# roahmlab/armour

Measured on NVIDIA B200. Metric: planning iters/s (eval_g + eval_jac_g pairs on built reach sets; Kinova 7-DOF, 128 steps, 10 obstacles), higher is better.
Workload: dtype f64

## Files before the change

### armour_b200/_lib.py

```python
from __future__ import annotations

import ctypes as C
import os

_HERE = os.path.dirname(os.path.abspath(__file__))
LIB_PATH = os.environ.get("ARMOUR_B200_LIB") or os.path.join(_HERE, "libarmour_b200.so")
NF = 7

OK, ERR_ARG, ERR_CUDA, ERR_OBSTACLES, ERR_CAPACITY, ERR_STATE, ERR_NOMEM = 0, -1, -2, -3, -4, -5, -6


class ArmourError(RuntimeError):
    def __init__(self, code, msg):
        super().__init__(f"armour_b200 error {code}: {msg}")
        self.code = code


class Config(C.Structure):
    _fields_ = [
        ("struct_size", C.c_int), ("device", C.c_int), ("robot_model", C.c_int), ("num_time_steps", C.c_int),
        ("max_obstacles", C.c_int), ("max_problems", C.c_int), ("cap_link_monomials", C.c_int),
        ("cap_torque_monomials", C.c_int), ("cap_work_monomials", C.c_int), ("simplify_threshold", C.c_double),
        ("k_range", C.c_double * NF), ("mass_uncertainty", C.c_double), ("inertia_uncertainty", C.c_double),
    ]


dp = C.POINTER(C.c_double)
ip = C.POINTER(C.c_int)
up = C.POINTER(C.c_ulonglong)


class ReachsetTables(C.Structure):
    _fields_ = [
        ("cap_link", C.c_int), ("cap_u", C.c_int), ("link_n", ip), ("link_center", dp), ("link_key", up),
        ("link_coeff", dp), ("u_n", ip), ("u_center", dp), ("u_key", up), ("u_coeff", dp), ("u_radius", dp),
        ("torque_radius", dp), ("link_gens", dp),
    ]


SIGNATURES = {
    "armour_config_default": (C.c_int, [C.POINTER(Config)]),
    "armour_ctx_create": (C.c_int, [C.POINTER(Config), C.POINTER(C.c_void_p)]),
    "armour_ctx_destroy": (C.c_int, [C.c_void_p]),
    "armour_ctx_reserve": (C.c_int, [C.c_void_p, C.c_int, C.c_int]),
    "armour_ctx_set_stream": (C.c_int, [C.c_void_p, C.c_void_p]),
    "armour_ctx_synchronize": (C.c_int, [C.c_void_p]),
    "armour_status_string": (C.c_char_p, [C.c_int]),
    "armour_last_error": (C.c_char_p, [C.c_void_p]),
    "armour_abi_version": (C.c_int, []),
    "armour_kernel_launches": (C.c_longlong, [C.c_void_p]),
    "armour_num_joints": (C.c_int, [C.c_void_p]),
    "armour_num_time_steps": (C.c_int, [C.c_void_p]),
    "armour_num_constraints": (C.c_int, [C.c_void_p, C.c_int]),
    "armour_reachsets_build": (C.c_int, [C.c_void_p, dp, dp, dp, dp, C.c_int]),
    "armour_get_torque_radius": (C.c_int, [C.c_void_p, dp]),
    "armour_get_link_independent_generators": (C.c_int, [C.c_void_p, dp]),
    "armour_get_bounds": (C.c_int, [C.c_void_p, dp, dp]),
    "armour_eval_g": (C.c_int, [C.c_void_p, dp, dp]),
    "armour_eval_jac_g": (C.c_int, [C.c_void_p, dp, dp]),
    "armour_eval_g_jac": (C.c_int, [C.c_void_p, dp, dp, dp]),
    "armour_get_link_sliced_center": (C.c_int, [C.c_void_p, dp]),
    "armour_verdict": (C.c_int, [C.c_void_p, dp, ip, ip]),
    "armour_cost": (C.c_int, [C.c_void_p, dp, dp, dp, dp]),
    "armour_batch_reachsets_build": (C.c_int, [C.c_void_p, C.c_int, dp, dp, dp, dp, C.c_int]),
    "armour_batch_eval": (C.c_int, [C.c_void_p, C.c_int, dp, dp, dp]),
    "armour_batch_eval_device": (C.c_int, [C.c_void_p, C.c_int, C.c_void_p, C.c_void_p, C.c_void_p]),
    "armour_batch_reachsets_build_device": (C.c_int, [C.c_void_p, C.c_int, C.c_void_p, C.c_void_p, C.c_void_p,
                                                      C.c_void_p, C.c_int]),
    "armour_batch_verdict_device": (C.c_int, [C.c_void_p, C.c_int, C.c_void_p, C.c_void_p, C.c_void_p]),
    "armour_batch_get_torque_radius": (C.c_int, [C.c_void_p, C.c_int, dp]),
    "armour_batch_get_link_independent_generators": (C.c_int, [C.c_void_p, C.c_int, dp]),
    "armour_batch_get_bounds": (C.c_int, [C.c_void_p, C.c_int, dp, dp]),
    "armour_batch_get_build_status": (C.c_int, [C.c_void_p, C.c_int, ip]),
    "armour_batch_get_monomial_counts": (C.c_int, [C.c_void_p, C.c_int, ip, ip]),
    "armour_batch_get_candidate_counts": (C.c_int, [C.c_void_p, C.c_int, C.c_void_p]),
    "armour_chunk_intervals": (C.c_int, []),
    "armour_jacobian_nnz": (C.c_longlong, [C.c_void_p, C.c_int]),
    "armour_jacobian_structure": (C.c_int, [C.c_void_p, C.c_int, ip, ip]),
    "armour_eval_jac_g_structured": (C.c_int, [C.c_void_p, dp, dp]),
    "armour_batch_eval_structured": (C.c_int, [C.c_void_p, C.c_int, dp, dp, dp]),
    "armour_batch_eval_structured_device": (C.c_int, [C.c_void_p, C.c_int, C.c_void_p, C.c_void_p, C.c_void_p]),
    "armour_measure_fp64_peak": (C.c_int, [C.c_void_p, dp]),
    "armour_solver_options_default": (None, [C.c_void_p]),
    "armour_batch_solve_device": (C.c_int, [C.c_void_p, C.c_int, C.c_void_p, C.c_void_p, C.c_void_p, C.c_void_p,
                                            C.c_void_p, C.c_void_p]),
    "armour_batch_solve": (C.c_int, [C.c_void_p, C.c_int, dp, C.c_void_p, dp, ip, ip, ip]),
    "armour_export_reachsets": (C.c_int, [C.c_void_p, C.c_int, C.POINTER(ReachsetTables)]),
    "armour_import_reachsets": (C.c_int, [C.c_void_p, C.c_int, C.c_int, C.POINTER(ReachsetTables), dp, dp, dp, dp,
                                          C.c_int]),
}


class ControllerGains(C.Structure):
    _fields_ = [("Kr", dp), ("alpha", C.c_double), ("V_max", C.c_double), ("r_norm_threshold", C.c_double),
                ("apply_friction", C.c_int)]


_gp = C.POINTER(ControllerGains)
SIGNATURES.update({
    "armour_controller_create": (C.c_int, [C.c_char_p, C.c_double, C.c_int, C.POINTER(C.c_void_p)]),
    "armour_controller_create_error": (C.c_char_p, []),
    "armour_controller_destroy": (None, [C.c_void_p]),
    "armour_controller_num_joints": (C.c_int, [C.c_void_p]),
    "armour_controller_last_error": (C.c_char_p, [C.c_void_p]),
    "armour_controller_kernel_launches": (C.c_longlong, [C.c_void_p]),
    "armour_controller_set_stream": (C.c_int, [C.c_void_p, C.c_void_p]),
    "armour_controller_synchronize": (C.c_int, [C.c_void_p]),
    "armour_controller_get_interval_model": (C.c_int, [C.c_void_p, dp]),
    "armour_controller_rnea": (C.c_int, [C.c_void_p, C.c_int, dp, dp, dp, dp, C.c_int, C.c_int, dp, dp, dp]),
    "armour_controller_rnea_device": (C.c_int, [C.c_void_p, C.c_int] + [C.c_void_p] * 5 + [C.c_int, C.c_int] + [C.c_void_p] * 3),
    "armour_controller_update": (C.c_int, [C.c_void_p, C.c_int, _gp, dp, dp, dp, dp, dp, dp, dp, dp, ip]),
    "armour_controller_update_device": (C.c_int, [C.c_void_p, C.c_int, _gp] + [C.c_void_p] * 10),
})

SIGNATURES.update({
    "armour_armtd_ctx_create": (C.c_int, [C.POINTER(Config), C.POINTER(C.c_void_p)]),
    "armour_armtd_build": (C.c_int, [C.c_void_p, dp, dp, dp, dp, dp, C.c_int]),
    "armour_armtd_num_constraints": (C.c_int, [C.c_void_p]),
    "armour_armtd_eval": (C.c_int, [C.c_void_p, dp, dp, dp]),
    "armour_armtd_get_bounds": (C.c_int, [C.c_void_p, dp, dp]),
    "armour_armtd_verdict": (C.c_int, [C.c_void_p, dp, ip, ip]),
    "armour_armtd_cost": (C.c_int, [C.c_void_p, dp, dp, dp, dp]),
    "armour_armtd_get_link_sliced_center": (C.c_int, [C.c_void_p, dp]),
    "armour_armtd_get_link_independent_generators": (C.c_int, [C.c_void_p, dp]),
    "armour_armtd_batch_ctx_create": (C.c_int, [C.POINTER(Config), C.POINTER(C.c_void_p)]),
    "armour_armtd_batch_build": (C.c_int, [C.c_void_p, C.c_int, dp, dp, dp, dp, dp, C.c_int]),
    "armour_armtd_batch_build_device": (C.c_int, [C.c_void_p, C.c_int] + [C.c_void_p] * 5 + [C.c_int, C.c_void_p]),
    "armour_armtd_batch_eval": (C.c_int, [C.c_void_p, C.c_int, dp, dp, dp]),
    "armour_armtd_batch_eval_device": (C.c_int, [C.c_void_p, C.c_int, C.c_void_p, C.c_void_p, C.c_void_p]),
    "armour_armtd_batch_verdict_device": (C.c_int, [C.c_void_p, C.c_int, C.c_void_p, C.c_void_p, C.c_void_p]),
    "armour_armtd_batch_cost": (C.c_int, [C.c_void_p, C.c_int, dp, dp, dp, dp]),
    "armour_armtd_batch_get_link_independent_generators": (C.c_int, [C.c_void_p, C.c_int, dp]),
    "armour_armtd_batch_solve": (C.c_int, [C.c_void_p, C.c_int, dp, C.c_void_p, dp, ip, ip, ip]),
    "armour_armtd_batch_solve_device": (C.c_int, [C.c_void_p, C.c_int] + [C.c_void_p] * 6),
})


class SolverOptions(C.Structure):
    _fields_ = [("max_iter", C.c_int), ("tol", C.c_double), ("torque_tol", C.c_double), ("collision_tol", C.c_double),
                ("qp_sweeps", C.c_int), ("qp_update_budget", C.c_int)]


class RolloutOptions(C.Structure):
    _fields_ = [("struct_size", C.c_int), ("max_replans", C.c_int), ("lookahead", C.c_double), ("goal_radius", C.c_double),
                ("audit_samples", C.c_int), ("solver", SolverOptions)]


class RolloutOut(C.Structure):
    _fields_ = [("outcome", ip), ("replans", ip), ("infeasible", ip), ("final_state", dp), ("min_clearance", dp),
                ("log_state", dp), ("log_q_des", dp), ("log_k", dp), ("log_int", ip), ("log_clearance", dp)]


ROLLOUT_BUDGET, ROLLOUT_ARRIVED, ROLLOUT_COLLISION, ROLLOUT_LIMIT = 0, 1, 2, 3

SIGNATURES.update({
    "armour_rollout_options_default": (None, [C.POINTER(RolloutOptions)]),
    "armour_batch_rollout_device": (C.c_int, [C.c_void_p, C.c_int, C.c_void_p, C.c_void_p, C.c_void_p, C.c_int,
                                              C.POINTER(RolloutOptions), C.POINTER(RolloutOut)]),
    "armour_batch_rollout": (C.c_int, [C.c_void_p, C.c_int, dp, dp, dp, C.c_int, C.POINTER(RolloutOptions),
                                       C.POINTER(RolloutOut)]),
    "armour_batch_clearance_device": (C.c_int, [C.c_void_p, C.c_int] + [C.c_void_p] * 3 + [C.c_int, C.c_void_p, C.c_void_p]),
    "armour_batch_clearance": (C.c_int, [C.c_void_p, C.c_int, dp, ip, dp, C.c_int, dp, ip]),
})


_LIB = None


def load():
    global _LIB
    if _LIB is None:
        if not os.path.exists(LIB_PATH):
            raise ImportError(
                f"{LIB_PATH} is missing: build the CUDA extension first (python -c 'import __graft_entry__ as g; "
                "g.build()' or make -C armour_b200/csrc). armour_b200 has no CPU fallback.")
        lib = C.CDLL(LIB_PATH)
        for name, (res, args) in SIGNATURES.items():
            fn = getattr(lib, name)
            fn.restype = res
            fn.argtypes = args
        _LIB = lib
    return _LIB
```

### armour_b200/csrc/armour_capi.cu

```cuda
#include <cuda_runtime.h>

#include <algorithm>
#include <cmath>
#include <cstdio>
#include <cstdlib>
#include <cstring>
#include <mutex>
#include <new>
#include <string>
#include <vector>

#include "../../include/armour_b200.h"
#include "bezier.cuh"
#include "device_constants.cuh"
#ifdef K1_PROFILE
constexpr int K1_PROF_SITES = 512;
__device__ long long g_k1prof[128 * K1_PROF_SITES * 2];
__device__ int g_k1spill[8];
#endif
#ifndef K1LAT_NT
#define K1LAT_NT 128
#endif
#ifndef K1LAT_CTAS
#define K1LAT_CTAS 1
#endif
#ifndef K1LAT_GROUPS
#define K1LAT_GROUPS 3
#endif
#ifndef K1LAT_MG
#define K1LAT_MG 1
#endif
#ifndef K1LAT_TAB_16THS
#define K1LAT_TAB_16THS 11
#endif
#define K1_TAB_16THS K1LAT_TAB_16THS
#ifndef K1LAT_DYN_CAP
#define K1LAT_DYN_CAP -1
#endif
#define K1_DYN_CAP K1LAT_DYN_CAP
#define K1_NS k1lat
#define K1_NT K1LAT_NT
#define K1_CTAS K1LAT_CTAS
#define K1_GROUPS K1LAT_GROUPS
#define K1_MG K1LAT_MG
#include "k1_reachsets.cuh"
#undef K1_NS
#undef K1_NT
#undef K1_CTAS
#undef K1_GROUPS
#undef K1_MG
#undef K1_TAB_16THS
#define K1_MG 0
#ifndef K1THR_NT
#define K1THR_NT 64
#endif
#ifndef K1THR_GROUPS
#define K1THR_GROUPS 8
#endif
#ifndef K1THR_CTAS
#define K1THR_CTAS 2
#endif
#ifndef K1THR_TAB_EIGHTHS
#define K1THR_TAB_EIGHTHS 4
#endif
#ifndef K1THR_DYN_CAP
#define K1THR_DYN_CAP 0
#endif
#ifndef K1THR_JRS_GLOBAL
#define K1THR_JRS_GLOBAL 1
#endif
#undef K1_JRS_GLOBAL
#define K1_JRS_GLOBAL K1THR_JRS_GLOBAL
#undef K1_DYN_CAP
#define K1_DYN_CAP K1THR_DYN_CAP
#undef K1_TAB_EIGHTHS
#define K1_TAB_EIGHTHS K1THR_TAB_EIGHTHS
#define K1_TAB_16THS (2 * K1THR_TAB_EIGHTHS)
#define K1_NS k1thr
#define K1_NT K1THR_NT
#define K1_CTAS K1THR_CTAS
#define K1_GROUPS K1THR_GROUPS
#include "k1_reachsets.cuh"
#undef K1_NS
#undef K1_NT
#undef K1_CTAS
#undef K1_GROUPS
#include "k3_constraints.cuh"
#include "k4_solver.cuh"
#include "armtd.cuh"
#include "rollout.cuh"
#include "layout.h"

using namespace armour;

struct armour_ctx {
    armour_config cfg;
    RobotConstants rc;
    cudaStream_t stream = nullptr;
    cudaStream_t own_stream = nullptr;
    Batch B;
    int built_nprob = 0;
    size_t hp_capacity = 0;
    int hp_nprob = 0;
    int* d_unit_flag = nullptr;
    size_t obs_capacity = 0;
    double* d_in = nullptr;
    double* d_obs = nullptr;
    double* d_k = nullptr;
    double* d_g = nullptr;
    double* d_jac = nullptr;
    size_t g_capacity = 0, jac_capacity = 0;
    double* d_jnz = nullptr;
    size_t jnz_capacity = 0;
    int* d_verdict = nullptr;
    double* d_solver = nullptr;
    int* d_solver_i = nullptr;
    double* d_solver_io = nullptr;
    size_t solver_doubles = 0, solver_ints = 0;
    k1lat::K1Scratch k1_lat;
    k1thr::K1Scratch k1_thr;
    bool k1_thr_ready = false;
    long long launches = 0;
    std::string last_error;
    std::vector<double> h_torque_radius;
    bool h_torque_valid = false;
    std::vector<double> h_q0, h_qd0, h_qdd0;
    bool armtd = false;
    double* d_jrs = nullptr;
    double* d_armtd_in = nullptr;
    double* d_krange = nullptr;
    double* d_zero = nullptr;
    double* d_cs = nullptr;
    double* d_jrs_raw = nullptr;
    double* d_ga = nullptr;
    double* d_ja = nullptr;
    size_t ga_capacity = 0, ja_capacity = 0;
    std::vector<double> h_krange;
    double* d_roll = nullptr;
    int* d_roll_i = nullptr;
    size_t roll_doubles = 0, roll_ints = 0;
    char* d_stage = nullptr;
    size_t stage_bytes = 0;
};

namespace {

__global__ void __launch_bounds__(256) k_fp64_peak(double* out, int iters, double a) {
    double x[8];
#pragma unroll
    for (int i = 0; i < 8; i++) x[i] = double(threadIdx.x + i);
    for (int it = 0; it < iters; it++) {
#pragma unroll
        for (int i = 0; i < 8; i++) x[i] = __fma_rn(x[i], a, 0.5);
    }
    double s = 0;
#pragma unroll
    for (int i = 0; i < 8; i++) s += x[i];
    if (s == 12345.678) out[0] = s;
}

int fail(armour_ctx* c, int code, const std::string& msg) {
    if (c) c->last_error = msg;
    return code;
}
#define CU(expr)                                                                                     \
    do {                                                                                             \
        cudaError_t e__ = (expr);                                                                    \
        if (e__ != cudaSuccess)                                                                      \
            return fail(ctx, ARMOUR_ERR_CUDA, std::string(#expr) + ": " + cudaGetErrorString(e__)); \
    } while (0)

template <class T>
cudaError_t dalloc(T** p, size_t n) {
    return cudaMalloc(reinterpret_cast<void**>(p), std::max<size_t>(n, 1) * sizeof(T));
}

int ensure_eval_buffers(armour_ctx* ctx, int nprob, bool need_g, bool need_jac) {
    const size_t m = size_t(ctx->B.m());
    if (need_g && ctx->g_capacity < nprob * m) {
        if (ctx->d_g) cudaFree(ctx->d_g);
        ctx->d_g = nullptr;
        CU(dalloc(&ctx->d_g, nprob * m));
        ctx->g_capacity = nprob * m;
    }
    if (need_jac && ctx->jac_capacity < nprob * m * NF) {
        if (ctx->d_jac) cudaFree(ctx->d_jac);
        ctx->d_jac = nullptr;
        CU(dalloc(&ctx->d_jac, nprob * m * NF));
        ctx->jac_capacity = nprob * m * NF;
    }
    return ARMOUR_OK;
}

int ensure_obstacle_buffers(armour_ctx* ctx, int nprob, int nobs) {
    const size_t need_obs = size_t(nprob) * nobs * 12;
    if (ctx->obs_capacity < need_obs) {
        if (ctx->d_obs) cudaFree(ctx->d_obs);
        ctx->d_obs = nullptr;
        CU(dalloc(&ctx->d_obs, need_obs));
        ctx->obs_capacity = need_obs;
    }
    Batch& B = ctx->B;
    B.O = nobs;
    B.nprob = nprob;
    const size_t need_hp = size_t(nprob) * (B.T / TB) * B.hp_chunk();
    if (ctx->hp_capacity < need_hp || ctx->hp_nprob < nprob) {
        if (B.hp_cand) cudaFree(B.hp_cand);
        if (B.hp_cnt) cudaFree(B.hp_cnt);
        if (B.hp_slow) cudaFree(B.hp_slow);
        B.hp_cand = nullptr;
        B.hp_cnt = nullptr;
        B.hp_slow = nullptr;
        ctx->hp_capacity = 0;
        ctx->hp_nprob = 0;
        ctx->built_nprob = 0;
        const size_t np = std::max(nprob, ctx->hp_nprob);
        CU(dalloc(&B.hp_cand, need_hp));
        CU(dalloc(&B.hp_cnt, need_hp / (HP_CAP * 4)));
        CU(dalloc(&B.hp_slow, np));
        CU(cudaMemsetAsync(B.hp_slow, 0, np * sizeof(int), ctx->stream));
        ctx->hp_capacity = need_hp;
        ctx->hp_nprob = nprob;
    }
    B.obstacles = ctx->d_obs;
    return ARMOUR_OK;
}

int launch_build(armour_ctx* ctx, const Batch& B, int* nl, bool* latency) {
    const long long nunits = (long long)B.nprob * B.T;
    const bool thr = ctx->cfg.max_problems > 1 && nunits > 2LL * ctx->k1_lat.grid;
    *latency = !thr;
    if (thr) {
        if (!ctx->k1_thr_ready) {
            CU(k1thr::k1_scratch_create(&ctx->k1_thr, ctx->cfg, ctx->rc, ctx->stream));
            ctx->k1_thr_ready = true;
        }
        CU(k1thr::launch_reachsets(B, ctx->k1_thr, ctx->stream, nl));
    } else {
        CU(k1lat::launch_reachsets(B, ctx->k1_lat, ctx->stream, nl, ctx->d_unit_flag));
    }
    return ARMOUR_OK;
}

std::mutex g_const_mutex;
struct ConstOwner {
    bool valid = false;
    RobotConstants rc;
};
ConstOwner g_const_owner[64];

int ensure_constants(armour_ctx* ctx) {
    const int dev = ctx->cfg.device;
    if (dev < 0 || dev >= 64) return fail(ctx, ARMOUR_ERR_ARG, "device ordinal");
    std::lock_guard<std::mutex> lock(g_const_mutex);
    ConstOwner& o = g_const_owner[dev];
    if (o.valid && std::memcmp(&o.rc, &ctx->rc, sizeof(RobotConstants)) == 0) return ARMOUR_OK;
    CU(cudaDeviceSynchronize());
    CU(upload_constants(ctx->rc, ctx->stream));
    o.rc = ctx->rc;
    o.valid = true;
    return ARMOUR_OK;
}

int check_batch(armour_ctx* ctx, int nprob, int nobs) {
    if (!ctx) return ARMOUR_ERR_ARG;
    if (nprob < 1 || nprob > ctx->cfg.max_problems)
        return fail(ctx, ARMOUR_ERR_STATE, "nprob outside [1, max_problems]");
    if (nobs < 0) return fail(ctx, ARMOUR_ERR_ARG, "negative obstacle count");
    if (nobs > ctx->cfg.max_obstacles)
        return fail(ctx, ARMOUR_ERR_OBSTACLES, "number of obstacles larger than max_obstacles");
    return ARMOUR_OK;
}

int fetch_torque_radius(armour_ctx* ctx) {
    if (ctx->h_torque_valid) return ARMOUR_OK;
    const size_t n = size_t(ctx->built_nprob) * NF * ctx->B.T;
    ctx->h_torque_radius.resize(n);
    CU(cudaMemcpyAsync(ctx->h_torque_radius.data(), ctx->B.torque_radius, n * sizeof(double), cudaMemcpyDeviceToHost,
                       ctx->stream));
    CU(cudaStreamSynchronize(ctx->stream));
    ctx->h_torque_valid = true;
    return ARMOUR_OK;
}

}

extern "C" {

int armour_abi_version(void) { return ARMOUR_ABI_VERSION; }

const char* armour_status_string(int s) {
    switch (s) {
        case ARMOUR_OK: return "ok";
        case ARMOUR_ERR_ARG: return "invalid argument";
        case ARMOUR_ERR_CUDA: return "CUDA error";
        case ARMOUR_ERR_OBSTACLES: return "too many obstacles";
        case ARMOUR_ERR_CAPACITY: return "monomial table capacity exceeded";
        case ARMOUR_ERR_STATE: return "invalid call order or batch size";
        case ARMOUR_ERR_NOMEM: return "out of memory";
        default: return "unknown status";
    }
}

int armour_config_default(armour_config* cfg) {
    if (!cfg) return ARMOUR_ERR_ARG;
    std::memset(cfg, 0, sizeof(*cfg));
    cfg->struct_size = int(sizeof(armour_config));
    cfg->device = 0;
    cfg->robot_model = 0;
    cfg->num_time_steps = 128;
    cfg->max_obstacles = 40;
    cfg->max_problems = 1;
    cfg->cap_link_monomials = 32;
    cfg->cap_torque_monomials = 64;
    cfg->cap_work_monomials = 768;
    cfg->simplify_threshold = 5e-4;
    for (int i = 0; i < NF; i++) cfg->k_range[i] = M_PI / 48;
    cfg->mass_uncertainty = -1;
    cfg->inertia_uncertainty = -1;
    return ARMOUR_OK;
}

int armour_ctx_create(const armour_config* cfg, armour_ctx** out) {
    if (!cfg || !out) return ARMOUR_ERR_ARG;
    *out = nullptr;
    if (cfg->struct_size != int(sizeof(armour_config))) return ARMOUR_ERR_ARG;
    if (cfg->num_time_steps < TB || cfg->num_time_steps > 128 || cfg->num_time_steps % TB != 0) return ARMOUR_ERR_ARG;
    if (cfg->max_problems < 1 || cfg->max_obstacles < 0) return ARMOUR_ERR_ARG;
    if (cfg->robot_model < 0 || cfg->robot_model > 1) return ARMOUR_ERR_ARG;
    if (cfg->cap_link_monomials < 1 || cfg->cap_torque_monomials < 1 || cfg->cap_work_monomials < 64)
        return ARMOUR_ERR_ARG;
    if (cfg->cap_link_monomials % 8 != 0 || cfg->cap_torque_monomials % 8 != 0) return ARMOUR_ERR_ARG;
    if (cfg->max_problems > 65535) return ARMOUR_ERR_ARG;
    int ndev = 0;
    if (cudaGetDeviceCount(&ndev) != cudaSuccess || ndev == 0 || cfg->device >= ndev) return ARMOUR_ERR_CUDA;
    armour_ctx* ctx = new (std::nothrow) armour_ctx();
    if (!ctx) return ARMOUR_ERR_NOMEM;
    ctx->cfg = *cfg;
    ctx->rc = make_robot_constants(cfg->robot_model);
    ctx->rc.num_time_steps = cfg->num_time_steps;
    ctx->rc.simplify_threshold = cfg->simplify_threshold;
    for (int i = 0; i < NF; i++) ctx->rc.k_range[i] = cfg->k_range[i];
    if (cfg->mass_uncertainty >= 0) ctx->rc.mass_uncertainty = cfg->mass_uncertainty;
    if (cfg->inertia_uncertainty >= 0) ctx->rc.inertia_uncertainty = cfg->inertia_uncertainty;

    auto bail = [&](const char* what, cudaError_t e) {
        std::fprintf(stderr, "armour_ctx_create: %s: %s\n", what, cudaGetErrorString(e));
        armour_ctx_destroy(ctx);
        return ARMOUR_ERR_CUDA;
    };
    cudaError_t e;
    if ((e = cudaSetDevice(cfg->device)) != cudaSuccess) return bail("cudaSetDevice", e);
    if ((e = cudaStreamCreateWithFlags(&ctx->own_stream, cudaStreamNonBlocking)) != cudaSuccess)
        return bail("cudaStreamCreate", e);
    ctx->stream = ctx->own_stream;
    if (ensure_constants(ctx) != ARMOUR_OK) return bail("upload_constants", cudaGetLastError());

    Batch& B = ctx->B;
    std::memset(&B, 0, sizeof(B));
    B.T = cfg->num_time_steps;
    B.NJ = ctx->rc.num_joints;
    B.capL = cfg->cap_link_monomials;
    B.capU = cfg->cap_torque_monomials;
    const size_t P = size_t(cfg->max_problems), T = size_t(B.T), NJ = size_t(B.NJ);
#define ALLOC(ptr, n) \
    if ((e = dalloc(&ptr, (n))) != cudaSuccess) return bail(#ptr, e)
    ALLOC(ctx->d_in, 3 * P * NF);
    ALLOC(B.link_n, P * T * NJ);
    ALLOC(B.link_c, P * T * NJ * 3);
    ALLOC(B.link_key, P * T * NJ * B.capL);
    ALLOC(B.link_g, P * T * NJ * B.capL * 3);
    ALLOC(B.u_n, P * T * NF);
    ALLOC(B.u_c, P * T * NF);
    ALLOC(B.u_r, P * T * NF);
    ALLOC(B.u_key, P * T * NF * B.capU);
    ALLOC(B.u_g, P * T * NF * B.capU);
    ALLOC(B.torque_radius, P * NF * T);
    ALLOC(B.link_gens, P * T * NJ * 18);
    ALLOC(B.link_r, P * T * NJ * 3);
    ALLOC(B.link_sliced, P * T * NJ * 3);
    ALLOC(B.status, P);
    ALLOC(ctx->d_unit_flag, P * T);
    ALLOC(ctx->d_k, P * NF);
    ALLOC(ctx->d_verdict, 2 * P);
#undef ALLOC
    B.q0 = ctx->d_in;
    B.qd0 = ctx->d_in + P * NF;
    B.qdd0 = ctx->d_in + 2 * P * NF;
    if ((e = cudaMemsetAsync(B.status, 0, P * sizeof(int), ctx->stream)) != cudaSuccess) return bail("memset", e);
    if ((e = cudaMemsetAsync(ctx->d_unit_flag, 0, P * T * sizeof(int), ctx->stream)) != cudaSuccess) return bail("memset", e);
    if ((e = cudaMemsetAsync(B.link_n, 0, P * T * NJ * sizeof(int), ctx->stream)) != cudaSuccess) return bail("memset", e);
    if ((e = cudaMemsetAsync(B.u_n, 0, P * T * NF * sizeof(int), ctx->stream)) != cudaSuccess) return bail("memset", e);
    if ((e = k1lat::k1_scratch_create(&ctx->k1_lat, ctx->cfg, ctx->rc, ctx->stream)) != cudaSuccess) return bail("k1 scratch", e);
    if ((long long)cfg->max_problems * B.T > 2LL * ctx->k1_lat.grid) {
        if ((e = k1thr::k1_scratch_create(&ctx->k1_thr, ctx->cfg, ctx->rc, ctx->stream)) != cudaSuccess) return bail("k1 throughput scratch", e);
        ctx->k1_thr_ready = true;
        cudaFuncAttributes fa2;
        if ((e = cudaFuncGetAttributes(&fa2, k1thr::k_reachsets)) != cudaSuccess) return bail("load k_reachsets (throughput)", e);
    }
    {
        cudaFuncAttributes fa;
        if ((e = cudaFuncGetAttributes(&fa, k1lat::k_reachsets)) != cudaSuccess) return bail("load k_reachsets", e);
        if ((e = cudaFuncGetAttributes(&fa, k_hyperplanes)) != cudaSuccess) return bail("load k_hyperplanes", e);
        if ((e = cudaFuncGetAttributes(&fa, k_constraints)) != cudaSuccess) return bail("load k_constraints", e);
        if ((e = cudaFuncSetAttribute(k_constraints, cudaFuncAttributeMaxDynamicSharedMemorySize,
                                      TB * (MAXJ * K3_LTAB_BYTES + NF * K3_UTAB_BYTES) + K3_CAND_ARENA)) != cudaSuccess)
            return bail("k_constraints shared memory", e);
        if ((e = cudaFuncGetAttributes(&fa, k_constraints_slow)) != cudaSuccess) return bail("load k_constraints_slow", e);
        if ((e = cudaFuncGetAttributes(&fa, k_verdict)) != cudaSuccess) return bail("load k_verdict", e);
    }
    if ((e = cudaStreamSynchronize(ctx->stream)) != cudaSuccess) return bail("sync", e);
    *out = ctx;
    return ARMOUR_OK;
}

int armour_ctx_destroy(armour_ctx* ctx) {
    if (!ctx) return ARMOUR_OK;
    cudaSetDevice(ctx->cfg.device);
    Batch& B = ctx->B;
    void* ptrs[] = {ctx->d_roll, ctx->d_roll_i, ctx->d_stage, ctx->d_solver, ctx->d_solver_i, ctx->d_solver_io, ctx->d_unit_flag, ctx->d_jnz, ctx->d_jrs, ctx->d_armtd_in, ctx->d_ga, ctx->d_ja,
                    ctx->d_in, ctx->d_obs, ctx->d_k, ctx->d_g, ctx->d_jac, ctx->d_verdict, B.link_n, B.link_c,
                    B.link_key, B.link_g, B.u_n, B.u_c, B.u_r, B.u_key, B.u_g, B.torque_radius, B.link_gens, B.link_r, B.hp_cand, B.hp_cnt, B.hp_slow,
                    B.link_sliced, B.status};
    for (void* p : ptrs)
        if (p) cudaFree(p);
    k1lat::k1_scratch_destroy(&ctx->k1_lat);
    k1thr::k1_scratch_destroy(&ctx->k1_thr);
    if (ctx->own_stream) cudaStreamDestroy(ctx->own_stream);
    delete ctx;
    return ARMOUR_OK;
}

int armour_ctx_set_stream(armour_ctx* ctx, void* s) {
    if (!ctx) return ARMOUR_ERR_ARG;
    ctx->stream = s ? static_cast<cudaStream_t>(s) : ctx->own_stream;
    return ARMOUR_OK;
}
int armour_ctx_synchronize(armour_ctx* ctx) {
    if (!ctx) return ARMOUR_ERR_ARG;
    CU(cudaStreamSynchronize(ctx->stream));
    return ARMOUR_OK;
}
const char* armour_last_error(const armour_ctx* ctx) { return ctx ? ctx->last_error.c_str() : "null context"; }
long long armour_kernel_launches(const armour_ctx* ctx) { return ctx ? ctx->launches : 0; }
int armour_num_joints(const armour_ctx* ctx) { return ctx ? ctx->B.NJ : ARMOUR_ERR_ARG; }
int armour_num_time_steps(const armour_ctx* ctx) { return ctx ? ctx->B.T : ARMOUR_ERR_ARG; }
int armour_num_constraints(const armour_ctx* ctx, int nobs) {
    if (!ctx || nobs < 0) return ARMOUR_ERR_ARG;
    return NF * ctx->B.T + ctx->B.NJ * ctx->B.T * nobs + 4 * NF;
}

int armour_ctx_reserve(armour_ctx* ctx, int nprob, int nobs) {
    int rc = check_batch(ctx, nprob, nobs);
    if (rc) return rc;
    CU(cudaSetDevice(ctx->cfg.device));
    { int rc_c = ensure_constants(ctx); if (rc_c) return rc_c; }
    const int O = ctx->B.O, np = ctx->B.nprob;
    rc = ensure_obstacle_buffers(ctx, nprob, nobs);
    ctx->B.O = O;
    ctx->B.nprob = np;
    if (rc) return rc;
    ctx->B.O = nobs;
    rc = ensure_eval_buffers(ctx, nprob, true, true);
    ctx->B.O = O;
    return rc;
}

int armour_batch_reachsets_build_device(armour_ctx* ctx, int nprob, const double* d_q0, const double* d_qd0,
                                        const double* d_qdd0, const double* d_obstacles, int nobs) {
    int rc = check_batch(ctx, nprob, nobs);
    if (rc) return rc;
    if (!d_q0 || !d_qd0 || !d_qdd0 || (nobs > 0 && !d_obstacles)) return fail(ctx, ARMOUR_ERR_ARG, "null input");
    CU(cudaSetDevice(ctx->cfg.device));
    { int rc_c = ensure_constants(ctx); if (rc_c) return rc_c; }
    rc = ensure_obstacle_buffers(ctx, nprob, nobs);
    if (rc) return rc;
    const size_t P = size_t(ctx->cfg.max_problems);
    ctx->B.epoch++;
    int nl = 0;
    bool latency = false;
    if (nobs > 0) {
        Batch Bb = ctx->B;
        Bb.q0 = d_q0;
        Bb.qd0 = d_qd0;
        Bb.qdd0 = d_qdd0;
        Bb.obstacles = d_obstacles;
        { int rc2 = launch_build(ctx, Bb, &nl, &latency); if (rc2) return rc2; }
        HpStage stage{ctx->d_in, ctx->d_in + P * NF, ctx->d_in + 2 * P * NF, ctx->d_obs};
        CU(launch_hyperplanes(Bb, ctx->stream, latency ? ctx->d_unit_flag : nullptr, stage));
        nl++;
    } else {
        const size_t nb = size_t(nprob) * NF * sizeof(double);
        CU(cudaMemcpyAsync(ctx->d_in, d_q0, nb, cudaMemcpyDeviceToDevice, ctx->stream));
        CU(cudaMemcpyAsync(ctx->d_in + P * NF, d_qd0, nb, cudaMemcpyDeviceToDevice, ctx->stream));
        CU(cudaMemcpyAsync(ctx->d_in + 2 * P * NF, d_qdd0, nb, cudaMemcpyDeviceToDevice, ctx->stream));
        { int rc2 = launch_build(ctx, ctx->B, &nl, &latency); if (rc2) return rc2; }
    }
    ctx->launches += nl;
    ctx->built_nprob = nprob;
    ctx->h_torque_valid = false;
    ctx->h_q0.clear();
    return ARMOUR_OK;
}

int armour_batch_reachsets_build(armour_ctx* ctx, int nprob, const double* q0, const double* qd0, const double* qdd0,
                                 const double* obstacles, int nobs) {
    int rc = check_batch(ctx, nprob, nobs);
    if (rc) return rc;
    if (!q0 || !qd0 || !qdd0 || (nobs > 0 && !obstacles)) return fail(ctx, ARMOUR_ERR_ARG, "null input");
    CU(cudaSetDevice(ctx->cfg.device));
    { int rc_c = ensure_constants(ctx); if (rc_c) return rc_c; }
    rc = ensure_obstacle_buffers(ctx, nprob, nobs);
    if (rc) return rc;
    const size_t P = size_t(ctx->cfg.max_problems);
    const size_t nb = size_t(nprob) * NF * sizeof(double);
    CU(cudaMemcpyAsync(ctx->d_in, q0, nb, cudaMemcpyHostToDevice, ctx->stream));
    CU(cudaMemcpyAsync(ctx->d_in + P * NF, qd0, nb, cudaMemcpyHostToDevice, ctx->stream));
    CU(cudaMemcpyAsync(ctx->d_in + 2 * P * NF, qdd0, nb, cudaMemcpyHostToDevice, ctx->stream));
    if (nobs > 0)
        CU(cudaMemcpyAsync(ctx->d_obs, obstacles, size_t(nprob) * nobs * 12 * sizeof(double), cudaMemcpyHostToDevice,
                           ctx->stream));
    ctx->B.epoch++;
    int nl = 0;
    bool latency = false;
    { int rc2 = launch_build(ctx, ctx->B, &nl, &latency); if (rc2) return rc2; }
    ctx->launches += nl;
    CU(launch_hyperplanes(ctx->B, ctx->stream, (latency && nobs > 0) ? ctx->d_unit_flag : nullptr));
    ctx->launches += (nobs > 0);
    ctx->built_nprob = nprob;
    ctx->h_torque_valid = false;
    ctx->h_q0.assign(q0, q0 + size_t(nprob) * NF);
    ctx->h_qd0.assign(qd0, qd0 + size_t(nprob) * NF);
    ctx->h_qdd0.assign(qdd0, qdd0 + size_t(nprob) * NF);
    std::vector<int> st(nprob);
    CU(cudaMemcpyAsync(st.data(), ctx->B.status, nprob * sizeof(int), cudaMemcpyDeviceToHost, ctx->stream));
    CU(cudaStreamSynchronize(ctx->stream));
    for (int p = 0; p < nprob; p++)
        if ((st[p] >> 3) == ctx->B.epoch && (st[p] & 7) != 0) {
            int site[3] = {0, 0, 0};
            const int* dstats = latency ? ctx->k1_lat.stats : ctx->k1_thr.stats;
            std::string where;
            if (dstats && cudaMemcpy(site, dstats + 4, sizeof(site), cudaMemcpyDeviceToHost) == cudaSuccess && site[2] == ctx->B.epoch) {
                const int line = site[0] >> 3;
                where = "; first failing check: code " + std::to_string(site[0] & 7) + " at " +
                        (line >= 10000 ? "k1_reachsets.cuh:" + std::to_string(line - 10000) : "k1_pz.cuh:" + std::to_string(line)) +
                        ", problem " + std::to_string(site[1] / ctx->B.T) + " interval " + std::to_string(site[1] % ctx->B.T);
            }
            return fail(ctx, ARMOUR_ERR_CAPACITY,
                        "reach-set build overflowed a monomial table (problem " + std::to_string(p) + ", code " +
                            std::to_string(st[p] & 7) + ")" + where);
        }
    return ARMOUR_OK;
}

int armour_reachsets_build(armour_ctx* ctx, const double* q0, const double* qd0, const double* qdd0,
                           const double* obstacles, int nobs) {
    return armour_batch_reachsets_build(ctx, 1, q0, qd0, qdd0, obstacles, nobs);
}

int armour_batch_get_build_status(armour_ctx* ctx, int nprob, int* out) {
    if (!ctx || !out || nprob < 1 || nprob > ctx->built_nprob) return ARMOUR_ERR_ARG;
    CU(cudaMemcpyAsync(out, ctx->B.status, nprob * sizeof(int), cudaMemcpyDeviceToHost, ctx->stream));
    CU(cudaStreamSynchronize(ctx->stream));
    for (int p = 0; p < nprob; p++)
        out[p] = ((out[p] >> 3) == ctx->B.epoch && (out[p] & 7) != 0) ? ARMOUR_ERR_CAPACITY : ARMOUR_OK;
    return ARMOUR_OK;
}

int armour_batch_get_monomial_counts(armour_ctx* ctx, int nprob, int* link_n, int* u_n) {
    if (!ctx || nprob < 1 || nprob > ctx->built_nprob) return ARMOUR_ERR_ARG;
    const size_t T = ctx->B.T, NJ = ctx->B.NJ;
    if (link_n)
        CU(cudaMemcpyAsync(link_n, ctx->B.link_n, nprob * T * NJ * sizeof(int), cudaMemcpyDeviceToHost, ctx->stream));
    if (u_n) CU(cudaMemcpyAsync(u_n, ctx->B.u_n, nprob * T * NF * sizeof(int), cudaMemcpyDeviceToHost, ctx->stream));
    CU(cudaStreamSynchronize(ctx->stream));
    return ARMOUR_OK;
}

int armour_batch_get_candidate_counts(armour_ctx* ctx, int nprob, unsigned char* out) {
    if (!ctx || !out || nprob < 1 || nprob > ctx->built_nprob) return ARMOUR_ERR_ARG;
    const size_t rows = size_t(ctx->B.NJ) * ctx->B.T * ctx->B.O;
    if (rows) CU(cudaMemcpyAsync(out, ctx->B.hp_cnt, nprob * rows, cudaMemcpyDeviceToHost, ctx->stream));
    CU(cudaStreamSynchronize(ctx->stream));
    return ARMOUR_OK;
}

int armour_chunk_intervals(void) { return TB; }

#ifdef K1_PROFILE
extern "C" int armour_debug_k1_profile(long long* out, int reset) {
    cudaDeviceSynchronize();
    if (out) {
        int sp[8];
        if (cudaMemcpyFromSymbol(sp, g_k1spill, sizeof(sp)) == cudaSuccess)
            std::printf("k1 profile: %d of %d arena blocks in global memory, %d scratch pools in global memory, %d cross products on "
                        "the table path (largest term count %d)\n", sp[0], sp[1], sp[2], sp[3], sp[4]);
    }
    if (out && cudaMemcpyFromSymbol(out, g_k1prof, sizeof(long long) * 128 * K1_PROF_SITES * 2) != cudaSuccess) return ARMOUR_ERR_CUDA;
    if (reset) {
        void* p = nullptr;
        if (cudaGetSymbolAddress(&p, g_k1prof) != cudaSuccess) return ARMOUR_ERR_CUDA;
        if (cudaMemset(p, 0, sizeof(long long) * 128 * K1_PROF_SITES * 2) != cudaSuccess) return ARMOUR_ERR_CUDA;
    }
    return ARMOUR_OK;
}
#endif

int armour_measure_fp64_peak(armour_ctx* ctx, double* tflops) {
    if (!ctx || !tflops) return ARMOUR_ERR_ARG;
    CU(cudaSetDevice(ctx->cfg.device));
    { int rc_c = ensure_constants(ctx); if (rc_c) return rc_c; }
    int sms = 0;
    CU(cudaDeviceGetAttribute(&sms, cudaDevAttrMultiProcessorCount, ctx->cfg.device));
    double* d_out = nullptr;
    CU(dalloc(&d_out, 1));
    cudaEvent_t e0, e1;
    CU(cudaEventCreate(&e0));
    CU(cudaEventCreate(&e1));
    const int iters = 4096, grid = sms * 8, block = 256;
    double best = 0.0;
    for (int rep = 0; rep < 4; rep++) {
        CU(cudaEventRecord(e0, ctx->stream));
        k_fp64_peak<<<grid, block, 0, ctx->stream>>>(d_out, iters, 1.0000001);
        CU(cudaEventRecord(e1, ctx->stream));
        CU(cudaEventSynchronize(e1));
        float ms = 0;
        CU(cudaEventElapsedTime(&ms, e0, e1));
        const double fl = 2.0 * 8 * double(iters) * double(grid) * block;
        if (rep > 0) best = std::max(best, fl / (ms * 1e-3) / 1e12);
    }
    ctx->launches += 4;
    cudaEventDestroy(e0);
    cudaEventDestroy(e1);
    cudaFree(d_out);
    *tflops = best;
    return ARMOUR_OK;
}

int armour_batch_eval_device(armour_ctx* ctx, int nprob, const double* d_k, double* d_g, double* d_values) {
    if (!ctx || !d_k) return ARMOUR_ERR_ARG;
    if (nprob < 1 || nprob > ctx->built_nprob) return fail(ctx, ARMOUR_ERR_STATE, "evaluate before build");
    CU(cudaSetDevice(ctx->cfg.device));
    { int rc_c = ensure_constants(ctx); if (rc_c) return rc_c; }
    Batch B = ctx->B;
    B.nprob = nprob;
    CU(launch_constraints(B, d_k, d_g, d_values, ctx->stream));
    ctx->launches += 1 + (B.O > 0);
    return ARMOUR_OK;
}

int armour_batch_eval(armour_ctx* ctx, int nprob, const double* k, double* g, double* values) {
    if (!ctx || !k) return ARMOUR_ERR_ARG;
    if (nprob < 1 || nprob > ctx->built_nprob) return fail(ctx, ARMOUR_ERR_STATE, "evaluate before build");
    CU(cudaSetDevice(ctx->cfg.device));
    { int rc_c = ensure_constants(ctx); if (rc_c) return rc_c; }
    int rc = ensure_eval_buffers(ctx, nprob, g != nullptr, values != nullptr);
    if (rc) return rc;
    const size_t m = size_t(ctx->B.m());
    CU(cudaMemcpyAsync(ctx->d_k, k, size_t(nprob) * NF * sizeof(double), cudaMemcpyHostToDevice, ctx->stream));
    rc = armour_batch_eval_device(ctx, nprob, ctx->d_k, g ? ctx->d_g : nullptr, values ? ctx->d_jac : nullptr);
    if (rc) return rc;
    if (g) CU(cudaMemcpyAsync(g, ctx->d_g, nprob * m * sizeof(double), cudaMemcpyDeviceToHost, ctx->stream));
    if (values)
        CU(cudaMemcpyAsync(values, ctx->d_jac, nprob * m * NF * sizeof(double), cudaMemcpyDeviceToHost, ctx->stream));
    CU(cudaStreamSynchronize(ctx->stream));
    return ARMOUR_OK;
}

long long armour_jacobian_nnz(const armour_ctx* ctx, int nobs) {
    if (!ctx || nobs < 0) return ARMOUR_ERR_ARG;
    return jac_nnz(ctx->B.T, ctx->B.NJ, nobs);
}

int armour_jacobian_structure(const armour_ctx* ctx, int nobs, int* iRow, int* jCol) {
    if (!ctx || nobs < 0 || !iRow || !jCol) return ARMOUR_ERR_ARG;
    const int T = ctx->B.T, NJ = ctx->B.NJ;
    size_t n = 0;
    for (int r = 0; r < NF * T; r++)
        for (int c = 0; c < NF; c++, n++) {
            iRow[n] = r;
            jCol[n] = c;
        }
    for (int l = 0; l < NJ; l++)
        for (int r = 0; r < T * nobs; r++)
            for (int c = 0; c < jac_link_width(l); c++, n++) {
                iRow[n] = NF * T + l * T * nobs + r;
                jCol[n] = c;
            }
    for (int r = 0; r < 4 * NF; r++, n++) {
        iRow[n] = NF * T + NJ * T * nobs + r;
        jCol[n] = r % NF;
    }
    return ARMOUR_OK;
}

int armour_batch_eval_structured_device(armour_ctx* ctx, int nprob, const double* d_k, double* d_g, double* d_values_nnz) {
    if (!ctx || !d_k || !d_values_nnz) return ARMOUR_ERR_ARG;
    if (nprob < 1 || nprob > ctx->built_nprob) return fail(ctx, ARMOUR_ERR_STATE, "evaluate before build");
    CU(cudaSetDevice(ctx->cfg.device));
    int rc = ensure_eval_buffers(ctx, nprob, false, true);
    if (rc) return rc;
    rc = armour_batch_eval_device(ctx, nprob, d_k, d_g, ctx->d_jac);
    if (rc) return rc;
    Batch B = ctx->B;
    B.nprob = nprob;
    CU(launch_pack_jacobian(B, ctx->d_jac, d_values_nnz, ctx->stream));
    ctx->launches += 1;
    return ARMOUR_OK;
}

int armour_batch_eval_structured(armour_ctx* ctx, int nprob, const double* k, double* g, double* values_nnz) {
    if (!ctx || !k || !values_nnz) return ARMOUR_ERR_ARG;
    if (nprob < 1 || nprob > ctx->built_nprob) return fail(ctx, ARMOUR_ERR_STATE, "evaluate before build");
    CU(cudaSetDevice(ctx->cfg.device));
    int rc = ensure_eval_buffers(ctx, nprob, g != nullptr, true);
    if (rc) return rc;
    const size_t m = size_t(ctx->B.m());
    const size_t nnz = size_t(jac_nnz(ctx->B.T, ctx->B.NJ, ctx->B.O));
    if (ctx->jnz_capacity < nprob * nnz) {
        if (ctx->d_jnz) cudaFree(ctx->d_jnz);
        ctx->d_jnz = nullptr;
        ctx->jnz_capacity = 0;
        CU(dalloc(&ctx->d_jnz, nprob * nnz));
        ctx->jnz_capacity = nprob * nnz;
    }
    CU(cudaMemcpyAsync(ctx->d_k, k, size_t(nprob) * NF * sizeof(double), cudaMemcpyHostToDevice, ctx->stream));
    rc = armour_batch_eval_structured_device(ctx, nprob, ctx->d_k, g ? ctx->d_g : nullptr, ctx->d_jnz);
    if (rc) return rc;
    if (g) CU(cudaMemcpyAsync(g, ctx->d_g, nprob * m * sizeof(double), cudaMemcpyDeviceToHost, ctx->stream));
    CU(cudaMemcpyAsync(values_nnz, ctx->d_jnz, nprob * nnz * sizeof(double), cudaMemcpyDeviceToHost, ctx->stream));
    CU(cudaStreamSynchronize(ctx->stream));
    return ARMOUR_OK;
}

int armour_eval_jac_g_structured(armour_ctx* ctx, const double* k, double* values_nnz) {
    return armour_batch_eval_structured(ctx, 1, k, nullptr, values_nnz);
}

int armour_eval_g(armour_ctx* ctx, const double* k, double* g) { return armour_batch_eval(ctx, 1, k, g, nullptr); }
int armour_eval_jac_g(armour_ctx* ctx, const double* k, double* values) {
    return armour_batch_eval(ctx, 1, k, nullptr, values);
}
int armour_eval_g_jac(armour_ctx* ctx, const double* k, double* g, double* values) {
    return armour_batch_eval(ctx, 1, k, g, values);
}

int armour_batch_verdict_device(armour_ctx* ctx, int nprob, const double* d_g, int* d_feasible, int* d_first) {
    if (!ctx || !d_g || !d_feasible || !d_first) return ARMOUR_ERR_ARG;
    if (nprob < 1 || nprob > ctx->built_nprob) return fail(ctx, ARMOUR_ERR_STATE, "verdict before build");
    CU(cudaSetDevice(ctx->cfg.device));
    { int rc_c = ensure_constants(ctx); if (rc_c) return rc_c; }
    Batch B = ctx->B;
    B.nprob = nprob;
    CU(launch_verdict(B, d_g, d_feasible, d_first, ctx->stream));
    ctx->launches += 1;
    return ARMOUR_OK;
}

void armour_solver_options_default(armour_solver_options* opt) {
    if (!opt) return;
    opt->max_iter = 60;
    opt->tol = 1e-4;
    opt->torque_tol = 1e-2;
    opt->collision_tol = 1e-4;
    opt->qp_sweeps = 200;
    opt->qp_update_budget = 16384;
}

}

namespace {

template <class Nlp, class Eval, class Verdict>
int run_solver(armour_ctx* ctx, int nprob, const double* d_q_des, const armour_solver_options& opt, const Nlp& nlp, int m_rows,
               double* g_x, double* jac_x, const Eval& eval, int n_eval, const Verdict& verdict, double* d_k_opt, int* d_feasible,
               int* d_first, int* d_iters) {
    if (opt.max_iter < 1 || !(opt.tol > 0) || opt.qp_sweeps < 1) return fail(ctx, ARMOUR_ERR_ARG, "solver options");
    Batch B = ctx->B;
    B.nprob = nprob;
    const size_t m = size_t(m_rows);
    const size_t P = size_t(nprob);
    const size_t need_d = P * (3 * NF + 4) + P * m + P * SOLVER_ROWCAP * SOLVER_ROWW;
    const size_t need_i = 8 * P + 1;
    if (ctx->solver_doubles < need_d) {
        if (ctx->d_solver) cudaFree(ctx->d_solver);
        ctx->d_solver = nullptr;
        ctx->solver_doubles = 0;
        CU(dalloc(&ctx->d_solver, need_d));
        ctx->solver_doubles = need_d;
    }
    if (ctx->solver_ints < need_i) {
        if (ctx->d_solver_i) cudaFree(ctx->d_solver_i);
        ctx->d_solver_i = nullptr;
        ctx->solver_ints = 0;
        CU(dalloc(&ctx->d_solver_i, need_i));
        ctx->solver_ints = need_i;
    }
    SolverState S;
    double* w = ctx->d_solver;
    S.x = w; w += P * NF;
    S.xt = w; w += P * NF;
    S.best = w; w += P * NF;
    S.f = w; w += P;
    S.viol = w; w += P;
    S.fbest = w; w += P;
    S.delta = w; w += P;
    double* d_gt = w; w += P * m;
    S.rows = w;
    S.have_best = ctx->d_solver_i;
    S.status = S.have_best + P;
    S.iters = S.status + P;
    S.evals = S.iters + P;
    S.dbg = S.evals + P;
    int* d_running = S.dbg + 3 * P;
    int* d_list = d_running + 1;
    S.q_des = d_q_des;
    S.tol = opt.tol;
    S.torque_tol = opt.torque_tol;
    S.collision_tol = opt.collision_tol;
    S.max_iter = opt.max_iter;
    S.qp_sweeps = opt.qp_sweeps;
    S.qp_update_budget = opt.qp_update_budget;
    cudaStream_t st = ctx->stream;
    const size_t step_smem = solver_step_smem(m_rows);
    if (step_smem > 200 * 1024) return fail(ctx, ARMOUR_ERR_ARG, "too many constraint rows for the batched solver");
    if (step_smem > 40 * 1024)
        CU(cudaFuncSetAttribute(k_solver_step<Nlp>, cudaFuncAttributeMaxDynamicSharedMemorySize, int(step_smem)));
    CU(cudaMemsetAsync(S.x, 0, size_t(nprob) * NF * sizeof(double), st));
    CU(cudaMemsetAsync(S.xt, 0, size_t(nprob) * NF * sizeof(double), st));
    { int rc = eval(B, S.x, g_x, nullptr); if (rc) return rc; }
    k_solver_start<<<nprob, SOLVER_THREADS, 0, st>>>(B, nlp, S, g_x);
    CU(cudaGetLastError());
    ctx->launches += 1 + n_eval;
    static const int compact_every = [] {
        const char* v = std::getenv("ARMOUR_SOLVER_COMPACT_EVERY");
        const int n = v ? std::atoi(v) : 0;
        return n >= 1 ? n : 4;
    }();
    Batch Ba = B;
    int nactive = nprob;
    for (int it = 0; it < opt.max_iter && nactive > 0; it++) {
        Ba.nprob = nactive;
        { int rc = eval(Ba, S.x, g_x, jac_x); if (rc) return rc; }
        k_solver_step<<<nactive, SOLVER_THREADS, step_smem, st>>>(Ba, nlp, S, g_x, jac_x, it);
        { int rc = eval(Ba, S.xt, d_gt, nullptr); if (rc) return rc; }
        k_solver_accept<<<nactive, SOLVER_THREADS, 0, st>>>(Ba, nlp, S, d_gt, it == opt.max_iter - 1 ? 1 : 0);
        CU(cudaGetLastError());
        ctx->launches += 2 + 2 * n_eval;
        if ((it + 1) % compact_every == 0 && it + 1 < opt.max_iter) {
            CU(cudaMemsetAsync(d_running, 0, sizeof(int), st));
            k_solver_compact<<<(nprob + 255) / 256, 256, 0, st>>>(S, nprob, d_running, d_list);
            CU(cudaMemcpyAsync(&nactive, d_running, sizeof(int), cudaMemcpyDeviceToHost, st));
            CU(cudaStreamSynchronize(st));
            ctx->launches += 1;
            Ba.plist = d_list;
        }
    }
    k_solver_final<<<(nprob + 255) / 256, 256, 0, st>>>(S, nprob, d_k_opt, nullptr);
    { int rc = eval(B, d_k_opt, g_x, nullptr); if (rc) return rc; }
    { int rc = verdict(g_x, d_feasible, d_first); if (rc) return rc; }
    if (d_iters) CU(cudaMemcpyAsync(d_iters, S.iters, size_t(nprob) * sizeof(int), cudaMemcpyDeviceToDevice, st));
    if (std::getenv("ARMOUR_SOLVER_DEBUG")) {
        std::vector<int> dbg(size_t(nprob) * 3);
        CU(cudaMemcpyAsync(dbg.data(), S.dbg, dbg.size() * sizeof(int), cudaMemcpyDeviceToHost, st));
        CU(cudaStreamSynchronize(st));
        long long r = 0, sw = 0, mv = 0;
        int rmax = 0, mvmax = 0;
        for (int p = 0; p < nprob; p++) {
            r += dbg[p * 3];
            sw += dbg[p * 3 + 1];
            mv += dbg[p * 3 + 2];
            rmax = std::max(rmax, dbg[p * 3]);
            mvmax = std::max(mvmax, dbg[p * 3 + 2]);
        }
        std::printf("solver debug: last step per problem: rows mean %.0f max %d, active-set iterations mean %.1f, dropped rows mean %.1f max %d\n",
                    double(r) / nprob, rmax, double(sw) / nprob, double(mv) / nprob, mvmax);
    }
    ctx->launches += 2 + n_eval;
    CU(cudaGetLastError());
    return ARMOUR_OK;
}

using SolveDeviceFn = int (*)(armour_ctx*, int, const double*, const armour_solver_options*, double*, int*, int*, int*);
int solve_from_host(armour_ctx* ctx, int nprob, const double* q_des, const armour_solver_options* opt, double* k_opt, int* feasible,
                    int* first_violation, int* iterations, SolveDeviceFn solve_device) {
    CU(cudaSetDevice(ctx->cfg.device));
    { int rc_c = ensure_constants(ctx); if (rc_c) return rc_c; }
    if (!ctx->d_solver_io) CU(dalloc(&ctx->d_solver_io, size_t(ctx->cfg.max_problems) * (2 * NF + 2)));
    const size_t P = size_t(ctx->cfg.max_problems);
    double* d_q = ctx->d_solver_io;
// ... 205 lines not shown
    for (int i = 0; i < 13; i++) {
        off[i] = total;
        total += (sz[i] + 255) / 256 * 256;
    }
    rc = ensure_buffer(ctx, &ctx->d_stage, &ctx->stage_bytes, total);
    if (rc) return rc;
    char* base = ctx->d_stage;
    auto at = [&](int i) -> void* { return sz[i] ? base + off[i] : nullptr; };
    cudaStream_t st = ctx->stream;
    CU(cudaMemcpyAsync(at(0), start, sz[0], cudaMemcpyHostToDevice, st));
    CU(cudaMemcpyAsync(at(1), goal, sz[1], cudaMemcpyHostToDevice, st));
    if (nobs > 0) CU(cudaMemcpyAsync(at(2), obstacles, sz[2], cudaMemcpyHostToDevice, st));
    armour_rollout_out d_out;
    d_out.outcome = static_cast<int*>(at(3));
    d_out.replans = static_cast<int*>(at(4));
    d_out.infeasible = static_cast<int*>(at(5));
    d_out.final_state = static_cast<double*>(at(6));
    d_out.min_clearance = static_cast<double*>(at(7));
    d_out.log_state = static_cast<double*>(at(8));
    d_out.log_q_des = static_cast<double*>(at(9));
    d_out.log_k = static_cast<double*>(at(10));
    d_out.log_int = static_cast<int*>(at(11));
    d_out.log_clearance = static_cast<double*>(at(12));
    rc = rollout_run(ctx, nworlds, static_cast<const double*>(at(0)), static_cast<const double*>(at(1)),
                     nobs > 0 ? static_cast<const double*>(at(2)) : nullptr, nobs, *opt, d_out);
    if (rc) return rc;
    void* host[13] = {nullptr, nullptr, nullptr, out->outcome, out->replans, out->infeasible, out->final_state, out->min_clearance,
                      out->log_state, out->log_q_des, out->log_k, out->log_int, out->log_clearance};
    for (int i = 3; i < 13; i++)
        if (sz[i]) CU(cudaMemcpyAsync(host[i], at(i), sz[i], cudaMemcpyDeviceToHost, st));
    CU(cudaStreamSynchronize(st));
    return ARMOUR_OK;
}

int armour_batch_clearance_device(armour_ctx* ctx, int nconf, const double* d_q, const int* d_world, const double* d_obstacles,
                                  int nobs, double* d_clearance, int* d_which) {
    int rc = check_clearance(ctx, nconf, nobs);
    if (rc) return rc;
    if (!d_q || !d_clearance || (nobs > 0 && !d_obstacles)) return fail(ctx, ARMOUR_ERR_ARG, "null input");
    CU(cudaSetDevice(ctx->cfg.device));
    { int rc_c = ensure_constants(ctx); if (rc_c) return rc_c; }
    k_clearance<<<nconf, CLEAR_THREADS, 0, ctx->stream>>>(d_q, 1, d_world, d_obstacles, nobs, d_clearance, d_which);
    CU(cudaGetLastError());
    ctx->launches += 1;
    return ARMOUR_OK;
}

int armour_batch_clearance(armour_ctx* ctx, int nconf, const double* q, const int* world, const double* obstacles, int nobs,
                           double* clearance, int* which) {
    int rc = check_clearance(ctx, nconf, nobs);
    if (rc) return rc;
    if (!q || !clearance || (nobs > 0 && !obstacles)) return fail(ctx, ARMOUR_ERR_ARG, "null input");
    int nsets = 1;
    if (world)
        for (int i = 0; i < nconf; i++) {
            if (world[i] < 0) return fail(ctx, ARMOUR_ERR_ARG, "negative obstacle-set index");
            nsets = std::max(nsets, world[i] + 1);
        }
    CU(cudaSetDevice(ctx->cfg.device));
    const size_t nq = size_t(nconf) * NF * 8, nw = world ? size_t(nconf) * 4 : 0, nb = size_t(nsets) * nobs * 12 * 8,
                 nc = size_t(nconf) * 8, nh = which ? size_t(nconf) * 4 : 0;
    const size_t oq = 0, ow = oq + (nq + 255) / 256 * 256, ob = ow + (nw + 255) / 256 * 256, oc = ob + (nb + 255) / 256 * 256,
                 oh = oc + (nc + 255) / 256 * 256;
    rc = ensure_buffer(ctx, &ctx->d_stage, &ctx->stage_bytes, oh + nh);
    if (rc) return rc;
    char* base = ctx->d_stage;
    cudaStream_t st = ctx->stream;
    CU(cudaMemcpyAsync(base + oq, q, nq, cudaMemcpyHostToDevice, st));
    if (world) CU(cudaMemcpyAsync(base + ow, world, nw, cudaMemcpyHostToDevice, st));
    if (nobs > 0) CU(cudaMemcpyAsync(base + ob, obstacles, nb, cudaMemcpyHostToDevice, st));
    rc = armour_batch_clearance_device(ctx, nconf, reinterpret_cast<const double*>(base + oq),
                                       world ? reinterpret_cast<const int*>(base + ow) : nullptr,
                                       nobs > 0 ? reinterpret_cast<const double*>(base + ob) : nullptr, nobs,
                                       reinterpret_cast<double*>(base + oc), which ? reinterpret_cast<int*>(base + oh) : nullptr);
    if (rc) return rc;
    CU(cudaMemcpyAsync(clearance, base + oc, nc, cudaMemcpyDeviceToHost, st));
    if (which) CU(cudaMemcpyAsync(which, base + oh, nh, cudaMemcpyDeviceToHost, st));
    CU(cudaStreamSynchronize(st));
    return ARMOUR_OK;
}

int armour_batch_get_torque_radius(armour_ctx* ctx, int nprob, double* out) {
    if (!ctx || !out || nprob < 1 || nprob > ctx->built_nprob) return ARMOUR_ERR_ARG;
    int rc = fetch_torque_radius(ctx);
    if (rc) return rc;
    std::memcpy(out, ctx->h_torque_radius.data(), size_t(nprob) * NF * ctx->B.T * sizeof(double));
    return ARMOUR_OK;
}
int armour_get_torque_radius(armour_ctx* ctx, double* out) { return armour_batch_get_torque_radius(ctx, 1, out); }

int armour_batch_get_link_independent_generators(armour_ctx* ctx, int nprob, double* out) {
    if (!ctx || !out || nprob < 1 || nprob > ctx->built_nprob) return ARMOUR_ERR_ARG;
    CU(cudaMemcpyAsync(out, ctx->B.link_gens, size_t(nprob) * ctx->B.T * ctx->B.NJ * 18 * sizeof(double),
                       cudaMemcpyDeviceToHost, ctx->stream));
    CU(cudaStreamSynchronize(ctx->stream));
    return ARMOUR_OK;
}
int armour_get_link_independent_generators(armour_ctx* ctx, double* out) {
    return armour_batch_get_link_independent_generators(ctx, 1, out);
}

int armour_get_link_sliced_center(armour_ctx* ctx, double* out) {
    if (!ctx || !out || ctx->built_nprob < 1) return ARMOUR_ERR_ARG;
    CU(cudaMemcpyAsync(out, ctx->B.link_sliced, size_t(ctx->B.T) * ctx->B.NJ * 3 * sizeof(double),
                       cudaMemcpyDeviceToHost, ctx->stream));
    CU(cudaStreamSynchronize(ctx->stream));
    return ARMOUR_OK;
}

int armour_batch_get_bounds(armour_ctx* ctx, int nprob, double* g_l, double* g_u) {
    if (!ctx || !g_l || !g_u || nprob < 1 || nprob > ctx->built_nprob) return ARMOUR_ERR_ARG;
    int rc = fetch_torque_radius(ctx);
    if (rc) return rc;
    const RobotConstants& R = ctx->rc;
    const int T = ctx->B.T, NJ = ctx->B.NJ, O = ctx->B.O, m = ctx->B.m();
    for (int p = 0; p < nprob; p++) {
        double* gl = g_l + size_t(p) * m;
        double* gu = g_u + size_t(p) * m;
        const double* tr = ctx->h_torque_radius.data() + size_t(p) * NF * T;
        for (int t = 0; t < T; t++)
            for (int j = 0; j < NF; j++) {
                gl[t * NF + j] = -R.torque_limits[j] + tr[j * T + t];
                gu[t * NF + j] = R.torque_limits[j] - tr[j * T + t];
            }
        int off = NF * T;
        for (int i = off; i < off + T * NJ * O; i++) {
            gl[i] = -1e19;
            gu[i] = 0;
        }
        off += T * NJ * O;
        for (int rep = 0; rep < 2; rep++, off += NF)
            for (int i = 0; i < NF; i++) {
                gl[off + i] = R.state_limits_lb[i] + R.qe;
                gu[off + i] = R.state_limits_ub[i] - R.qe;
            }
        for (int rep = 0; rep < 2; rep++, off += NF)
            for (int i = 0; i < NF; i++) {
                gl[off + i] = -R.speed_limits[i] + R.qde;
                gu[off + i] = R.speed_limits[i] - R.qde;
            }
    }
    return ARMOUR_OK;
}
int armour_get_bounds(armour_ctx* ctx, double* g_l, double* g_u) { return armour_batch_get_bounds(ctx, 1, g_l, g_u); }

int armour_verdict(armour_ctx* ctx, const double* g, int* feasible, int* first_violation) {
    if (!ctx || !g || !feasible || ctx->built_nprob < 1) return ARMOUR_ERR_ARG;
    int rc = fetch_torque_radius(ctx);
    if (rc) return rc;
    const RobotConstants& R = ctx->rc;
    const int T = ctx->B.T, NJ = ctx->B.NJ, O = ctx->B.O;
    const double* tr = ctx->h_torque_radius.data();
    auto done = [&](int ok, int row) {
        *feasible = ok;
        if (first_violation) *first_violation = row;
        return ARMOUR_OK;
    };
    for (int t = 0; t < T; t++)
        for (int j = 0; j < NF; j++) {
            const double v = g[t * NF + j];
            if (v < -R.torque_limits[j] + tr[j * T + t] - R.torque_violation_threshold ||
                v > R.torque_limits[j] - tr[j * T + t] + R.torque_violation_threshold)
                return done(0, t * NF + j);
        }
    int off = NF * T;
    for (int i = 0; i < NJ * T * O; i++)
        if (g[off + i] > R.collision_violation_threshold) return done(0, off + i);
    off += NJ * T * O;
    for (int rep = 0; rep < 2; rep++, off += NF)
        for (int i = 0; i < NF; i++)
            if (g[off + i] < R.state_limits_lb[i] + R.qe || g[off + i] > R.state_limits_ub[i] - R.qe)
                return done(0, off + i);
    for (int rep = 0; rep < 2; rep++, off += NF)
        for (int i = 0; i < NF; i++)
            if (g[off + i] < -R.speed_limits[i] + R.qde || g[off + i] > R.speed_limits[i] - R.qde)
                return done(0, off + i);
    return done(1, -1);
}

int armour_cost(armour_ctx* ctx, const double* q_des, const double* k, double* obj, double* grad) {
    if (!ctx || !q_des || !k || ctx->built_nprob < 1 || ctx->h_q0.empty()) return ARMOUR_ERR_ARG;
    const RobotConstants& R = ctx->rc;
    auto wrap = [](double a) {
        while (a < -M_PI) a += 2 * M_PI;
        while (a > M_PI) a -= 2 * M_PI;
        return a;
    };
    const double tp = R.t_plan, D = R.duration;
    double qp[NF];
    for (int i = 0; i < NF; i++)
        qp[i] = bez_q(ctx->h_q0[i], ctx->h_qd0[i] * D, ctx->h_qdd0[i] * D * D, R.k_range[i] * k[i], tp);
    if (obj) {
        double v = pw2(wrap(q_des[0] - qp[0])) + pw2(wrap(q_des[2] - qp[2])) + pw2(wrap(q_des[4] - qp[4])) +
                   pw2(wrap(q_des[6] - qp[6])) + pw2(q_des[1] - qp[1]) + pw2(q_des[3] - qp[3]) + pw2(q_des[5] - qp[5]);
        *obj = v * R.cost_scale;
    }
    if (grad) {
        for (int i = 0; i < NF; i++) {
            const double dk = pw3(tp) * (6 * pw2(tp) - 15 * tp + 10) * R.k_range[i];
            grad[i] = (i % 2 == 0) ? (2 * wrap(qp[i] - q_des[i]) * dk) : (2 * (qp[i] - q_des[i]) * dk);
            grad[i] *= R.cost_scale;
        }
    }
    return ARMOUR_OK;
}

int armour_export_reachsets(armour_ctx* ctx, int prob, armour_reachset_tables* out) {
    if (!ctx || !out || prob < 0 || prob >= ctx->built_nprob) return ARMOUR_ERR_ARG;
    const Batch& B = ctx->B;
    const size_t T = B.T, NJ = B.NJ;
    if (out->cap_link < B.capL || out->cap_u < B.capU) return fail(ctx, ARMOUR_ERR_ARG, "export caps too small");
    std::vector<uint16_t> lk(T * NJ * B.capL), uk(T * NF * B.capU);
    std::vector<double> lg(T * NJ * B.capL * 3), ug(T * NF * B.capU);
    cudaStream_t st = ctx->stream;
#define D2H(dst, src, n) CU(cudaMemcpyAsync(dst, src, (n), cudaMemcpyDeviceToHost, st))
    D2H(out->link_n, B.link_n + prob * T * NJ, T * NJ * sizeof(int));
    D2H(out->link_center, B.link_c + prob * T * NJ * 3, T * NJ * 3 * sizeof(double));
    D2H(lk.data(), B.link_key + prob * T * NJ * B.capL, lk.size() * sizeof(uint16_t));
    D2H(lg.data(), B.link_g + prob * T * NJ * B.capL * 3, lg.size() * sizeof(double));
    D2H(out->u_n, B.u_n + prob * T * NF, T * NF * sizeof(int));
    D2H(out->u_center, B.u_c + prob * T * NF, T * NF * sizeof(double));
    D2H(uk.data(), B.u_key + prob * T * NF * B.capU, uk.size() * sizeof(uint16_t));
    D2H(ug.data(), B.u_g + prob * T * NF * B.capU, ug.size() * sizeof(double));
    if (out->u_radius) D2H(out->u_radius, B.u_r + prob * T * NF, T * NF * sizeof(double));
    if (out->torque_radius) D2H(out->torque_radius, B.torque_radius + prob * NF * T, NF * T * sizeof(double));
    if (out->link_gens) D2H(out->link_gens, B.link_gens + prob * T * NJ * 18, T * NJ * 18 * sizeof(double));
#undef D2H
    CU(cudaStreamSynchronize(st));
    for (size_t i = 0; i < T * NJ; i++)
        for (int mI = 0; mI < out->cap_link; mI++) {
            const bool valid = mI < out->link_n[i] && mI < B.capL;
            out->link_key[i * out->cap_link + mI] = valid ? lk[i * B.capL + mI] : 0;
            for (int e = 0; e < 3; e++)
                out->link_coeff[(i * out->cap_link + mI) * 3 + e] = valid ? lg[(i * B.capL + mI) * 3 + e] : 0.0;
        }
    for (size_t i = 0; i < T * NF; i++)
        for (int mI = 0; mI < out->cap_u; mI++) {
            const bool valid = mI < out->u_n[i] && mI < B.capU;
            out->u_key[i * out->cap_u + mI] = valid ? uk[i * B.capU + mI] : 0;
            out->u_coeff[i * out->cap_u + mI] = valid ? ug[i * B.capU + mI] : 0.0;
        }
    return ARMOUR_OK;
}

int armour_import_reachsets(armour_ctx* ctx, int prob, int nprob_total, const armour_reachset_tables* in,
                            const double* q0, const double* qd0, const double* qdd0, const double* obstacles, int nobs) {
    int rc = check_batch(ctx, nprob_total, nobs);
    if (rc) return rc;
    if (!in || !in->u_radius || !in->torque_radius || !in->link_gens || !q0 || !qd0 || !qdd0 || prob < 0 ||
        prob >= nprob_total)
        return ARMOUR_ERR_ARG;
    CU(cudaSetDevice(ctx->cfg.device));
    { int rc_c = ensure_constants(ctx); if (rc_c) return rc_c; }
    if (prob == 0 || ctx->B.O != nobs || ctx->B.nprob != nprob_total) {
        rc = ensure_obstacle_buffers(ctx, nprob_total, nobs);
        if (rc) return rc;
    }
    if (prob == 0) ctx->B.epoch++;
    const Batch& B = ctx->B;
    const size_t T = B.T, NJ = B.NJ, P = size_t(ctx->cfg.max_problems);
    std::vector<uint16_t> lk(T * NJ * B.capL, 0), uk(T * NF * B.capU, 0);
    std::vector<double> lg(T * NJ * B.capL * 3, 0.0), ug(T * NF * B.capU, 0.0);
    for (size_t i = 0; i < T * NJ; i++) {
        if (in->link_n[i] > B.capL) return fail(ctx, ARMOUR_ERR_CAPACITY, "imported link table exceeds cap_link_monomials");
        for (int mI = 0; mI < in->link_n[i]; mI++) {
            lk[i * B.capL + mI] = uint16_t(in->link_key[i * in->cap_link + mI]);
            for (int e = 0; e < 3; e++) lg[(i * B.capL + mI) * 3 + e] = in->link_coeff[(i * in->cap_link + mI) * 3 + e];
        }
    }
    for (size_t i = 0; i < T * NF; i++) {
        if (in->u_n[i] > B.capU) return fail(ctx, ARMOUR_ERR_CAPACITY, "imported torque table exceeds cap_torque_monomials");
        for (int mI = 0; mI < in->u_n[i]; mI++) {
            uk[i * B.capU + mI] = uint16_t(in->u_key[i * in->cap_u + mI]);
            ug[i * B.capU + mI] = in->u_coeff[i * in->cap_u + mI];
        }
    }
    cudaStream_t st = ctx->stream;
#define H2D(dst, src, n) CU(cudaMemcpyAsync(dst, src, (n), cudaMemcpyHostToDevice, st))
    H2D(B.link_n + prob * T * NJ, in->link_n, T * NJ * sizeof(int));
    H2D(B.link_c + prob * T * NJ * 3, in->link_center, T * NJ * 3 * sizeof(double));
    H2D(B.link_key + prob * T * NJ * B.capL, lk.data(), lk.size() * sizeof(uint16_t));
    H2D(B.link_g + prob * T * NJ * B.capL * 3, lg.data(), lg.size() * sizeof(double));
    H2D(B.u_n + prob * T * NF, in->u_n, T * NF * sizeof(int));
    H2D(B.u_c + prob * T * NF, in->u_center, T * NF * sizeof(double));
    H2D(B.u_key + prob * T * NF * B.capU, uk.data(), uk.size() * sizeof(uint16_t));
    H2D(B.u_g + prob * T * NF * B.capU, ug.data(), ug.size() * sizeof(double));
    H2D(B.torque_radius + prob * NF * T, in->torque_radius, NF * T * sizeof(double));
    H2D(B.link_gens + prob * T * NJ * 18, in->link_gens, T * NJ * 18 * sizeof(double));
    std::vector<double> lr(T * NJ * 3);
    for (size_t i = 0; i < T * NJ; i++)
        for (int e = 0; e < 3; e++) lr[i * 3 + e] = in->link_gens[i * 18 + e + (3 + e) * 3];
    H2D(B.link_r + prob * T * NJ * 3, lr.data(), lr.size() * sizeof(double));
    H2D(B.u_r + prob * T * NF, in->u_radius, T * NF * sizeof(double));
    H2D(ctx->d_in + prob * NF, q0, NF * sizeof(double));
    H2D(ctx->d_in + P * NF + prob * NF, qd0, NF * sizeof(double));
    H2D(ctx->d_in + 2 * P * NF + prob * NF, qdd0, NF * sizeof(double));
    if (nobs > 0) H2D(ctx->d_obs + size_t(prob) * nobs * 12, obstacles, size_t(nobs) * 12 * sizeof(double));
#undef H2D
    CU(cudaStreamSynchronize(st));
    if (prob == nprob_total - 1) {
        if (nobs > 0) CU(cudaMemsetAsync(ctx->B.hp_slow, 0, size_t(nprob_total) * sizeof(int), ctx->stream));
        CU(launch_hyperplanes(ctx->B, ctx->stream));
        ctx->launches += (nobs > 0);
        ctx->built_nprob = nprob_total;
        ctx->h_torque_valid = false;
    }
    if (prob == 0) {
        ctx->h_q0.assign(q0, q0 + NF);
        ctx->h_qd0.assign(qd0, qd0 + NF);
        ctx->h_qdd0.assign(qdd0, qdd0 + NF);
    }
    return ARMOUR_OK;
}


}

namespace {

int armtd_ctx_create(const armour_config* cfg_in, bool batch, armour_ctx** out) {
    if (!out) return ARMOUR_ERR_ARG;
    armour_config cfg;
    if (cfg_in) {
        cfg = *cfg_in;
    } else {
        int rc = armour_config_default(&cfg);
        if (rc) return rc;
    }
    cfg.num_time_steps = ARMTD_T_PADDED;
    if (!batch) cfg.max_problems = 1;
    cfg.robot_model = 0;
    armour_ctx* ctx = nullptr;
    int rc = armour_ctx_create(&cfg, &ctx);
    if (rc) return rc;
    const size_t P = size_t(ctx->cfg.max_problems);
    if (dalloc(&ctx->d_jrs, P * ARMTD_T_PADDED * NF * 6) != cudaSuccess ||
        dalloc(&ctx->d_armtd_in, P * NF * 4 + P * 6 * NF * ARMTD_T) != cudaSuccess ||
        cudaMemsetAsync(ctx->d_armtd_in, 0, P * NF * 2 * sizeof(double), ctx->stream) != cudaSuccess ||
        cudaStreamSynchronize(ctx->stream) != cudaSuccess) {
        armour_ctx_destroy(ctx);
        return ARMOUR_ERR_NOMEM;
    }
    ctx->d_krange = ctx->d_armtd_in;
    ctx->d_zero = ctx->d_krange + P * NF;
    ctx->d_cs = ctx->d_zero + P * NF;
    ctx->d_jrs_raw = ctx->d_cs + P * NF * 2;
    ctx->armtd = true;
    ctx->B.jrs_ext = ctx->d_jrs;
    *out = ctx;
    return ARMOUR_OK;
}

int check_armtd_batch(armour_ctx* ctx, int nprob, int nobs) {
    if (!ctx) return ARMOUR_ERR_ARG;
    if (!ctx->armtd) return fail(ctx, ARMOUR_ERR_STATE, "not an ARMTD context (armour_armtd_ctx_create / armour_armtd_batch_ctx_create)");
    return check_batch(ctx, nprob, nobs);
}

int check_armtd_built(armour_ctx* ctx, int nprob, const char* what) {
    if (!ctx->armtd) return fail(ctx, ARMOUR_ERR_STATE, "not an ARMTD context (armour_armtd_ctx_create / armour_armtd_batch_ctx_create)");
    if (nprob < 1 || nprob > ctx->built_nprob) return fail(ctx, ARMOUR_ERR_STATE, std::string(what) + " before armour_armtd_build");
    return ARMOUR_OK;
}

int ensure_armtd_buffers(armour_ctx* ctx, int nprob, bool need_jac) {
    const size_t ma = size_t(nprob) * armtd_m(ctx->B.NJ, ctx->B.O);
    if (ctx->ga_capacity < ma) {
        if (ctx->d_ga) cudaFree(ctx->d_ga);
        ctx->d_ga = nullptr;
        ctx->ga_capacity = 0;
        CU(dalloc(&ctx->d_ga, ma));
        ctx->ga_capacity = ma;
    }
    if (need_jac && ctx->ja_capacity < ma * NF) {
        if (ctx->d_ja) cudaFree(ctx->d_ja);
        ctx->d_ja = nullptr;
        ctx->ja_capacity = 0;
        CU(dalloc(&ctx->d_ja, ma * NF));
        ctx->ja_capacity = ma * NF;
    }
    return ARMOUR_OK;
}

int armtd_eval_launch(armour_ctx* ctx, const Batch& Bb, const double* d_k, double* d_g, double* d_jac) {
    CU(launch_constraints(Bb, d_k, ctx->d_g, d_jac ? ctx->d_jac : nullptr, ctx->stream));
    CU(launch_armtd_assemble(Bb, ctx->d_krange, d_k, ctx->d_g, ctx->d_jac, d_g, d_jac, ctx->stream));
    return ARMOUR_OK;
}

int fetch_armtd_inputs(armour_ctx* ctx) {
    const size_t n = size_t(ctx->built_nprob) * NF, P = size_t(ctx->cfg.max_problems);
    if (ctx->h_q0.size() >= n && ctx->h_qd0.size() >= n && ctx->h_krange.size() >= n) return ARMOUR_OK;
    ctx->h_q0.resize(n);
    ctx->h_qd0.resize(n);
    ctx->h_qdd0.assign(n, 0.0);
    ctx->h_krange.resize(n);
    CU(cudaMemcpyAsync(ctx->h_q0.data(), ctx->d_in, n * sizeof(double), cudaMemcpyDeviceToHost, ctx->stream));
    CU(cudaMemcpyAsync(ctx->h_qd0.data(), ctx->d_in + P * NF, n * sizeof(double), cudaMemcpyDeviceToHost, ctx->stream));
    CU(cudaMemcpyAsync(ctx->h_krange.data(), ctx->d_krange, n * sizeof(double), cudaMemcpyDeviceToHost, ctx->stream));
    CU(cudaStreamSynchronize(ctx->stream));
    return ARMOUR_OK;
}

}

extern "C" {

int armour_armtd_ctx_create(const armour_config* cfg, armour_ctx** out) { return armtd_ctx_create(cfg, false, out); }
int armour_armtd_batch_ctx_create(const armour_config* cfg, armour_ctx** out) { return armtd_ctx_create(cfg, true, out); }

int armour_armtd_num_constraints(const armour_ctx* ctx) {
    if (!ctx || !ctx->armtd) return ARMOUR_ERR_ARG;
    return armtd_m(ctx->B.NJ, ctx->B.O);
}

int armour_armtd_batch_build_device(armour_ctx* ctx, int nprob, const double* d_q0, const double* d_qd0, const double* d_jrs,
                                    const double* d_k_range, const double* d_obstacles, int nobs, const double* d_sincos) {
    int rc = check_armtd_batch(ctx, nprob, nobs);
    if (rc) return rc;
    if (!d_q0 || !d_qd0 || !d_jrs || !d_k_range || (nobs > 0 && !d_obstacles)) return fail(ctx, ARMOUR_ERR_ARG, "null input");
    CU(cudaSetDevice(ctx->cfg.device));
    { int rc_c = ensure_constants(ctx); if (rc_c) return rc_c; }
    const int n = nprob * ARMTD_T_PADDED * NF;
    k_armtd_jrs<<<(n + 255) / 256, 256, 0, ctx->stream>>>(nprob, d_q0, d_sincos, d_jrs, ctx->d_jrs);
    CU(cudaGetLastError());
    ctx->launches++;
    CU(cudaMemcpyAsync(ctx->d_krange, d_k_range, size_t(nprob) * NF * sizeof(double), cudaMemcpyDeviceToDevice, ctx->stream));
    ctx->h_krange.clear();
    return armour_batch_reachsets_build_device(ctx, nprob, d_q0, d_qd0, ctx->d_zero, d_obstacles, nobs);
}

int armour_armtd_batch_build(armour_ctx* ctx, int nprob, const double* q0, const double* qd0, const double* jrs,
                             const double* k_range, const double* obstacles, int nobs) {
    int rc = check_armtd_batch(ctx, nprob, nobs);
    if (rc) return rc;
    if (!q0 || !qd0 || !jrs || !k_range || (nobs > 0 && !obstacles)) return fail(ctx, ARMOUR_ERR_ARG, "null input");
    CU(cudaSetDevice(ctx->cfg.device));
    { int rc_c = ensure_constants(ctx); if (rc_c) return rc_c; }
    const size_t n = size_t(nprob) * NF;
    std::vector<double> cs(2 * n);
    for (size_t x = 0; x < n; x++) {
        cs[2 * x] = std::cos(q0[x]);
        cs[2 * x + 1] = std::sin(q0[x]);
    }
    cudaStream_t st = ctx->stream;
    CU(cudaMemcpyAsync(ctx->d_cs, cs.data(), cs.size() * sizeof(double), cudaMemcpyHostToDevice, st));
    CU(cudaMemcpyAsync(ctx->d_jrs_raw, jrs, n * 6 * ARMTD_T * sizeof(double), cudaMemcpyHostToDevice, st));
    CU(cudaMemcpyAsync(ctx->d_krange, k_range, n * sizeof(double), cudaMemcpyHostToDevice, st));
    const int nt = nprob * ARMTD_T_PADDED * NF;
    k_armtd_jrs<<<(nt + 255) / 256, 256, 0, st>>>(nprob, nullptr, ctx->d_cs, ctx->d_jrs_raw, ctx->d_jrs);
    CU(cudaGetLastError());
    ctx->launches++;
    ctx->h_krange.assign(k_range, k_range + n);
    const std::vector<double> zero(n, 0.0);
    rc = armour_batch_reachsets_build(ctx, nprob, q0, qd0, zero.data(), obstacles, nobs);
    if (rc != ARMOUR_OK && rc != ARMOUR_ERR_CAPACITY) cudaStreamSynchronize(st);
    return rc;
}

int armour_armtd_build(armour_ctx* ctx, const double* q0, const double* qd0, const double* jrs, const double* k_range,
                       const double* obstacles, int nobs) {
    if (!ctx || !q0 || !qd0 || !jrs || !k_range) return ARMOUR_ERR_ARG;
    return armour_armtd_batch_build(ctx, 1, q0, qd0, jrs, k_range, obstacles, nobs);
}

int armour_armtd_batch_eval_device(armour_ctx* ctx, int nprob, const double* d_k, double* d_g, double* d_values) {
    if (!ctx || !d_k || (!d_g && !d_values)) return ARMOUR_ERR_ARG;
    int rc = check_armtd_built(ctx, nprob, "evaluate");
    if (rc) return rc;
    CU(cudaSetDevice(ctx->cfg.device));
    { int rc_c = ensure_constants(ctx); if (rc_c) return rc_c; }
    rc = ensure_eval_buffers(ctx, nprob, true, d_values != nullptr);
    if (rc) return rc;
    Batch B = ctx->B;
    B.nprob = nprob;
    rc = armtd_eval_launch(ctx, B, d_k, d_g, d_values);
    ctx->launches += 2 + (B.O > 0);
    return rc;
}

int armour_armtd_batch_eval(armour_ctx* ctx, int nprob, const double* k, double* g, double* values) {
    if (!ctx || !k || (!g && !values)) return ARMOUR_ERR_ARG;
    int rc = check_armtd_built(ctx, nprob, "evaluate");
    if (rc) return rc;
    CU(cudaSetDevice(ctx->cfg.device));
    rc = ensure_armtd_buffers(ctx, nprob, values != nullptr);
    if (rc) return rc;
    const size_t ma = size_t(nprob) * armtd_m(ctx->B.NJ, ctx->B.O);
    cudaStream_t st = ctx->stream;
    CU(cudaMemcpyAsync(ctx->d_k, k, size_t(nprob) * NF * sizeof(double), cudaMemcpyHostToDevice, st));
    rc = armour_armtd_batch_eval_device(ctx, nprob, ctx->d_k, g ? ctx->d_ga : nullptr, values ? ctx->d_ja : nullptr);
    if (rc) return rc;
    if (g) CU(cudaMemcpyAsync(g, ctx->d_ga, ma * sizeof(double), cudaMemcpyDeviceToHost, st));
    if (values) CU(cudaMemcpyAsync(values, ctx->d_ja, ma * NF * sizeof(double), cudaMemcpyDeviceToHost, st));
    CU(cudaStreamSynchronize(st));
    return ARMOUR_OK;
}

int armour_armtd_eval(armour_ctx* ctx, const double* k, double* g, double* values) {
    return armour_armtd_batch_eval(ctx, 1, k, g, values);
}

int armour_armtd_get_bounds(armour_ctx* ctx, double* g_l, double* g_u) {
    if (!ctx || !g_l || !g_u || !ctx->armtd || ctx->built_nprob < 1) return ARMOUR_ERR_ARG;
    const RobotConstants& R = ctx->rc;
    int off = ctx->B.NJ * ARMTD_T * ctx->B.O;
    for (int i = 0; i < off; i++) {
        g_l[i] = -1e19;
        g_u[i] = 0;
    }
    for (int rep = 0; rep < 2; rep++, off += NF)
        for (int i = 0; i < NF; i++) {
            g_l[off + i] = R.state_limits_lb[i] + R.qe;
            g_u[off + i] = R.state_limits_ub[i] - R.qe;
        }
    for (int rep = 0; rep < 2; rep++, off += NF)
        for (int i = 0; i < NF; i++) {
            g_l[off + i] = -R.speed_limits[i] + R.qde;
            g_u[off + i] = R.speed_limits[i] - R.qde;
        }
    return ARMOUR_OK;
}

int armour_armtd_batch_verdict_device(armour_ctx* ctx, int nprob, const double* d_g, int* d_feasible, int* d_first) {
    if (!ctx || !d_g || !d_feasible || !d_first) return ARMOUR_ERR_ARG;
    int rc = check_armtd_built(ctx, nprob, "verdict");
    if (rc) return rc;
    CU(cudaSetDevice(ctx->cfg.device));
    { int rc_c = ensure_constants(ctx); if (rc_c) return rc_c; }
    k_armtd_verdict<<<nprob, 256, 0, ctx->stream>>>(ctx->B.NJ, ctx->B.O, d_g, d_feasible, d_first);
    CU(cudaGetLastError());
    ctx->launches++;
    return ARMOUR_OK;
}

int armour_armtd_verdict(armour_ctx* ctx, const double* g, int* feasible, int* first_violation) {
    if (!ctx || !g || !feasible || !ctx->armtd || ctx->built_nprob < 1) return ARMOUR_ERR_ARG;
    CU(cudaSetDevice(ctx->cfg.device));
    int rc = ensure_armtd_buffers(ctx, 1, false);
    if (rc) return rc;
    cudaStream_t st = ctx->stream;
    CU(cudaMemcpyAsync(ctx->d_ga, g, size_t(armtd_m(ctx->B.NJ, ctx->B.O)) * sizeof(double), cudaMemcpyHostToDevice, st));
    rc = armour_armtd_batch_verdict_device(ctx, 1, ctx->d_ga, ctx->d_verdict, ctx->d_verdict + 1);
    if (rc) return rc;
    int v[2];
    CU(cudaMemcpyAsync(v, ctx->d_verdict, sizeof(v), cudaMemcpyDeviceToHost, st));
    CU(cudaStreamSynchronize(st));
    *feasible = v[0];
    if (first_violation) *first_violation = v[1];
    return ARMOUR_OK;
}

int armour_armtd_batch_cost(armour_ctx* ctx, int nprob, const double* q_des, const double* k, double* obj, double* grad) {
    if (!ctx || !q_des || !k || !ctx->armtd || nprob < 1 || nprob > ctx->built_nprob) return ARMOUR_ERR_ARG;
    int rc = fetch_armtd_inputs(ctx);
    if (rc) return rc;
    for (int p = 0; p < nprob; p++) {
        const size_t o = size_t(p) * NF;
        const double f = armtd_cost(ctx->h_q0.data() + o, ctx->h_qd0.data() + o, ctx->h_krange.data() + o, q_des + o, k + o,
                                    ctx->rc.cost_scale, grad ? grad + o : nullptr);
        if (obj) obj[p] = f;
    }
    return ARMOUR_OK;
}

int armour_armtd_cost(armour_ctx* ctx, const double* q_des, const double* k, double* obj, double* grad) {
    return armour_armtd_batch_cost(ctx, 1, q_des, k, obj, grad);
}

int armour_armtd_batch_solve_device(armour_ctx* ctx, int nprob, const double* d_q_des, const armour_solver_options* opt_in,
                                    double* d_k_opt, int* d_feasible, int* d_first, int* d_iters) {
    if (!ctx || !d_q_des || !d_k_opt || !d_feasible || !d_first) return ARMOUR_ERR_ARG;
    int rc = check_armtd_built(ctx, nprob, "solve");
    if (rc) return rc;
    armour_solver_options opt;
    armour_solver_options_default(&opt);
    opt.tol = 1e-7;
    if (opt_in) opt = *opt_in;
    if (opt.max_iter < 1 || !(opt.tol > 0) || opt.qp_sweeps < 1) return fail(ctx, ARMOUR_ERR_ARG, "solver options");
    CU(cudaSetDevice(ctx->cfg.device));
    { int rc_c = ensure_constants(ctx); if (rc_c) return rc_c; }
    rc = ensure_eval_buffers(ctx, nprob, true, true);
    if (rc) return rc;
    rc = ensure_armtd_buffers(ctx, nprob, true);
    if (rc) return rc;
    auto eval = [ctx](const Batch& Bb, const double* x, double* g, double* jac) { return armtd_eval_launch(ctx, Bb, x, g, jac); };
    auto verdict = [ctx, nprob](const double* g, int* feasible, int* first) {
        k_armtd_verdict<<<nprob, 256, 0, ctx->stream>>>(ctx->B.NJ, ctx->B.O, g, feasible, first);
        CU(cudaGetLastError());
        return int(ARMOUR_OK);
    };
    return run_solver(ctx, nprob, d_q_des, opt, ArmtdNlp{ctx->d_krange}, armtd_m(ctx->B.NJ, ctx->B.O), ctx->d_ga, ctx->d_ja, eval,
                      2 + (ctx->B.O > 0), verdict, d_k_opt, d_feasible, d_first, d_iters);
}

int armour_armtd_batch_solve(armour_ctx* ctx, int nprob, const double* q_des, const armour_solver_options* opt, double* k_opt,
                             int* feasible, int* first_violation, int* iterations) {
    if (!ctx || !q_des || !k_opt || !feasible) return ARMOUR_ERR_ARG;
    int rc = check_armtd_built(ctx, nprob, "solve");
    if (rc) return rc;
    return solve_from_host(ctx, nprob, q_des, opt, k_opt, feasible, first_violation, iterations, armour_armtd_batch_solve_device);
}

int armour_armtd_get_link_sliced_center(armour_ctx* ctx, double* out) {
    if (!ctx || !out || !ctx->armtd || ctx->built_nprob < 1) return ARMOUR_ERR_ARG;
    CU(cudaMemcpyAsync(out, ctx->B.link_sliced, size_t(ARMTD_T) * ctx->B.NJ * 3 * sizeof(double), cudaMemcpyDeviceToHost, ctx->stream));
// ... 17 lines not shown
```

### armour_b200/csrc/k3_constraints.cuh

```cuda
#pragma once
#include <cuda_runtime.h>

#include "bezier.cuh"
#include "device_constants.cuh"
#include "layout.h"

namespace armour {

#ifndef K3_CH
#define K3_CH 2
#endif
#ifndef K3_CQ
#define K3_CQ 2
#endif
#ifndef K3_MINB
#define K3_MINB 4
#endif

template <class F>
__device__ __forceinline__ void for_each_plane(const double (&G)[9][3], const double (&oc)[3], F f) {
    int i = 0;
#pragma unroll
    for (int a = 0; a < 8; a++) {
#pragma unroll
        for (int b = a + 1; b < 9; b++) {
            const double cx = G[a][1] * G[b][2] - G[a][2] * G[b][1];
            const double cy = G[a][2] * G[b][0] - G[a][0] * G[b][2];
            const double cz = G[a][0] * G[b][1] - G[a][1] * G[b][0];
            const double nrm = sqrt(cx * cx + cy * cy + cz * cz);
            double C0 = 0, C1 = 0, C2 = 0;
            if (nrm > 0) {
                C0 = cx / nrm;
                C1 = cy / nrm;
                C2 = cz / nrm;
            }
            const double d = C0 * oc[0] + C1 * oc[1] + C2 * oc[2];
            double delta = 0.0;
#pragma unroll
            for (int gI = 0; gI < 9; gI++) delta += fabs(C0 * G[gI][0] + C1 * G[gI][1] + C2 * G[gI][2]);
            const bool nz = sqrt(C0 * C0 + C1 * C1 + C2 * C2) > 0;
            f(i, C0, C1, C2, d, delta, nz);
            i++;
        }
    }
}

__device__ __forceinline__ void load_row_generators(const double* __restrict__ ob, const double* __restrict__ LG,
                                                    double (&G)[9][3], double (&oc)[3]) {
#pragma unroll
    for (int e = 0; e < 3; e++) {
        oc[e] = ob[e];
#pragma unroll
        for (int gI = 0; gI < 3; gI++) G[gI][e] = ob[(gI + 1) * 3 + e];
#pragma unroll
        for (int gI = 0; gI < 6; gI++) G[gI + 3][e] = LG[e + gI * 3];
    }
}

constexpr int HP_ROWS = 8;
constexpr int HP_STAGE = 24;
constexpr int HP_THREADS = HP_ROWS * NCOMB;
struct HpStage {
    double* q0;
    double* qd0;
    double* qdd0;
    double* obstacles;
};
__global__ void __launch_bounds__(HP_THREADS) k_hyperplanes(Batch B, const int* __restrict__ unit_flag, HpStage stage) {
    const int p = blockIdx.y;
    if (stage.q0 && blockIdx.x == 0) {
        for (int i = threadIdx.x; i < NF; i += HP_THREADS) {
            stage.q0[size_t(p) * NF + i] = B.q0[size_t(p) * NF + i];
            stage.qd0[size_t(p) * NF + i] = B.qd0[size_t(p) * NF + i];
            stage.qdd0[size_t(p) * NF + i] = B.qdd0[size_t(p) * NF + i];
        }
        for (int i = threadIdx.x; i < B.O * 12; i += HP_THREADS)
            stage.obstacles[size_t(p) * B.O * 12 + i] = B.obstacles[size_t(p) * B.O * 12 + i];
    }
    if (unit_flag) {
        if (threadIdx.x == 0) {
            const int per = B.NJ * TB * B.O, total = per * (B.T / TB);
            int r0 = blockIdx.x * HP_ROWS, r1 = r0 + HP_ROWS - 1;
            if (r1 >= total) r1 = total - 1;
            int t_seen = -1;
            for (int r = r0; r <= r1; r++) {
                const int t = (r / per) * TB + ((r % per) / B.O) % TB;
                if (t == t_seen) continue;
                t_seen = t;
                const int* f = unit_flag + size_t(p) * B.T + t;
                int v;
                for (;;) {
                    asm volatile("ld.acquire.gpu.global.s32 %0, [%1];" : "=r"(v) : "l"(f) : "memory");
                    if (v == B.epoch) break;
                    __nanosleep(200);
                }
            }
        }
        __syncthreads();
    }
    const int NJ = B.NJ, O = B.O, T = B.T;
    const int per_pair = NJ * TB * O;
    const int rows_total = per_pair * (T / TB);
    const int lr = threadIdx.x / NCOMB, pi = threadIdx.x % NCOMB;
    const int r = blockIdx.x * HP_ROWS + lr;
    __shared__ double s_G[HP_ROWS][9][3], s_oc[HP_ROWS][3], s_c[HP_ROWS][3];
    __shared__ double s_A[HP_ROWS][NCOMB][3], s_b[HP_ROWS][2 * NCOMB], s_up[HP_ROWS][2 * NCOMB], s_lo[HP_ROWS][NCOMB];
    __shared__ double s_lomax[HP_ROWS];
    __shared__ double s_vc[HP_ROWS][2 * NCOMB];
    __shared__ double s_gm[HP_ROWS][HP_STAGE][3];
    __shared__ int s_best[HP_ROWS];
    __shared__ unsigned char s_flag[HP_ROWS][2 * NCOMB], s_list[HP_ROWS][2 * NCOMB];
    __shared__ int s_nlist[HP_ROWS];
    const bool live = r < rows_total;
    int tb = 0, x = 0;
    size_t idx = 0;
    if (live) {
        tb = r / per_pair;
        x = r - tb * per_pair;
        const int o = x % O, ltt = x / O, tt = ltt % TB, l = ltt / TB;
        idx = (size_t(p) * T + size_t(tb) * TB + tt) * NJ + l;
        if (pi < 27) {
            const int gI = pi / 3, e = pi % 3;
            s_G[lr][gI][e] = (gI < 3) ? B.obstacles[(size_t(p) * O + o) * 12 + (gI + 1) * 3 + e] : B.link_gens[idx * 18 + e + (gI - 3) * 3];
        } else if (pi < 30) {
            s_oc[lr][pi - 27] = B.obstacles[(size_t(p) * O + o) * 12 + (pi - 27)];
        } else if (pi < 33) {
            s_c[lr][pi - 30] = B.link_c[idx * 3 + (pi - 30)];
        } else if (pi == 33) {
            s_nlist[lr] = 0;
        }
        const int n = B.link_n[idx];
        const int ns = n < HP_STAGE ? n : HP_STAGE;
        for (int q = pi; q < ns * 3; q += NCOMB) s_gm[lr][q / 3][q % 3] = B.link_g[idx * B.capL * 3 + q];
    }
    __syncthreads();
    bool nz = false;
    if (live) {
        const int a = c_combA[pi], b = c_combB[pi];
        const double(*G)[3] = s_G[lr];
        const double cx = G[a][1] * G[b][2] - G[a][2] * G[b][1];
        const double cy = G[a][2] * G[b][0] - G[a][0] * G[b][2];
        const double cz = G[a][0] * G[b][1] - G[a][1] * G[b][0];
        const double nrm = sqrt(cx * cx + cy * cy + cz * cz);
        double C0 = 0, C1 = 0, C2 = 0;
        if (nrm > 0) {
            C0 = cx / nrm;
            C1 = cy / nrm;
            C2 = cz / nrm;
        }
        const double d = C0 * s_oc[lr][0] + C1 * s_oc[lr][1] + C2 * s_oc[lr][2];
        double delta = 0.0;
#pragma unroll 1
        for (int gI = 0; gI < 9; gI++) delta += fabs(C0 * G[gI][0] + C1 * G[gI][1] + C2 * G[gI][2]);
        nz = sqrt(C0 * C0 + C1 * C1 + C2 * C2) > 0;
        const double dot = C0 * s_c[lr][0] + C1 * s_c[lr][1] + C2 * s_c[lr][2];
        const double vpos = dot - (d + delta);
        const double vneg = -dot - (-d + delta);
        const int n = B.link_n[idx];
        const int ns = n < HP_STAGE ? n : HP_STAGE;
        const double* __restrict__ lg = B.link_g + idx * B.capL * 3;
        double rr = 0.0;
#pragma unroll 1
        for (int mI = 0; mI < ns; mI++) rr += fabs(C0 * s_gm[lr][mI][0] + C1 * s_gm[lr][mI][1] + C2 * s_gm[lr][mI][2]);
#pragma unroll 1
        for (int mI = ns; mI < n; mI++) rr += fabs(C0 * lg[mI * 3 + 0] + C1 * lg[mI * 3 + 1] + C2 * lg[mI * 3 + 2]);
        const double rho = rr * HP_RHO_SCALE + (1e-10 + 1e-12 * (fabs(dot) + fabs(d) + delta));
        s_A[lr][pi][0] = C0;
        s_A[lr][pi][1] = C1;
        s_A[lr][pi][2] = C2;
        s_b[lr][2 * pi] = d + delta;
        s_b[lr][2 * pi + 1] = -d + delta;
        s_up[lr][2 * pi] = nz ? vpos + rho : -1e300;
        s_up[lr][2 * pi + 1] = nz ? vneg + rho : -1e300;
        s_lo[lr][pi] = nz ? fmax(vpos, vneg) - rho : -1e300;
        s_vc[lr][2 * pi] = vpos;
        s_vc[lr][2 * pi + 1] = vneg;
    }
    __syncthreads();
    if (live && pi == 0) {
        double lo_max = -100000000;
        int best = -1;
#pragma unroll 1
        for (int i = 0; i < NCOMB; i++) {
            if (s_lo[lr][i] > lo_max) {
                lo_max = s_lo[lr][i];
                best = 2 * i + (s_vc[lr][2 * i + 1] > s_vc[lr][2 * i] ? 1 : 0);
            }
        }
        s_lomax[lr] = lo_max;
        s_best[lr] = best;
    }
    __syncthreads();
    bool drop[2] = {false, false};
    if (live && nz && s_best[lr] >= 0) {
        const int jb = s_best[lr];
        const double sj = (jb & 1) ? -1.0 : 1.0;
        const double J0 = sj * s_A[lr][jb >> 1][0], J1 = sj * s_A[lr][jb >> 1][1], J2 = sj * s_A[lr][jb >> 1][2];
        const double vj = s_vc[lr][jb];
        const int n = B.link_n[idx];
        const int ns = n < HP_STAGE ? n : HP_STAGE;
        const double* __restrict__ lg = B.link_g + idx * B.capL * 3;
#pragma unroll 1
        for (int sgn = 0; sgn < 2; sgn++) {
            const int sI = 2 * pi + sgn;
            if (sI == jb || !(s_up[lr][sI] >= s_lomax[lr])) continue;
            const double sg = sgn ? -1.0 : 1.0;
            const double D0 = J0 - sg * s_A[lr][pi][0], D1 = J1 - sg * s_A[lr][pi][1], D2 = J2 - sg * s_A[lr][pi][2];
            double rd = 0.0;
#pragma unroll 1
            for (int mI = 0; mI < ns; mI++) rd += fabs(D0 * s_gm[lr][mI][0] + D1 * s_gm[lr][mI][1] + D2 * s_gm[lr][mI][2]);
#pragma unroll 1
            for (int mI = ns; mI < n; mI++) rd += fabs(D0 * lg[mI * 3 + 0] + D1 * lg[mI * 3 + 1] + D2 * lg[mI * 3 + 2]);
            const double vi = s_vc[lr][sI];
            const double margin = rd * HP_RHO_SCALE + (1e-10 + 1e-12 * (fabs(vi) + fabs(vj) + fabs(s_b[lr][sI]) + fabs(s_b[lr][jb])));
            drop[sgn] = (vj - vi) > margin;
        }
    }
    __syncthreads();
    if (live) {
        if (drop[0]) s_up[lr][2 * pi] = -1e300;
        if (drop[1]) s_up[lr][2 * pi + 1] = -1e300;
    }
    __syncthreads();
    if (live) {
        const double lo_max = s_lomax[lr];
#pragma unroll 1
        for (int sgn = 0; sgn < 2; sgn++) {
            const int sI = 2 * pi + sgn;
            if (nz && s_up[lr][sI] >= lo_max) s_list[lr][atomicAdd(&s_nlist[lr], 1)] = (unsigned char)sI;
        }
    }
    __syncthreads();
    bool keep[2] = {false, false};
    if (live) {
        const double lo_max = s_lomax[lr];
        const int nl = s_nlist[lr];
#pragma unroll 1
        for (int sgn = 0; sgn < 2; sgn++) {
            const int sI = 2 * pi + sgn;
            bool k = nz && s_up[lr][sI] >= lo_max;
            if (k) {
                const double sg = sgn ? -1.0 : 1.0;
                const double A0 = sg * s_A[lr][pi][0], A1 = sg * s_A[lr][pi][1], A2 = sg * s_A[lr][pi][2], bb = s_b[lr][sI];
#pragma unroll 1
                for (int c = 0; c < nl && k; c++) {
                    const int q = s_list[lr][c];
                    if (q >= sI) continue;
                    const double sq = (q & 1) ? -1.0 : 1.0;
                    const int qi = q >> 1;
                    if (sq * s_A[lr][qi][0] == A0 && sq * s_A[lr][qi][1] == A1 && sq * s_A[lr][qi][2] == A2 && s_b[lr][q] <= bb)
                        k = false;
                }
            }
            keep[sgn] = k;
            s_flag[lr][sI] = k ? 1 : 0;
        }
    }
    __syncthreads();
    if (live) {
        const size_t chunk = size_t(p) * (T / TB) + tb;
        double* row = B.hp_cand + chunk * B.hp_chunk() + size_t(x) * 4;
        const size_t cstride = size_t(per_pair) * 4;
        const int nl = s_nlist[lr];
        if (keep[0] || keep[1] || pi == 0) {
            int count = 0, before[2] = {0, 0};
#pragma unroll 1
            for (int c = 0; c < nl; c++) {
                const int q = s_list[lr][c];
                if (s_flag[lr][q]) {
                    count++;
                    before[0] += (q < 2 * pi);
                    before[1] += (q < 2 * pi + 1);
                }
            }
            if (count <= HP_CAP) {
#pragma unroll 1
                for (int sgn = 0; sgn < 2; sgn++) {
                    if (keep[sgn]) {
                        const double sg = sgn ? -1.0 : 1.0;
                        double* e = row + size_t(before[sgn]) * cstride;
                        e[0] = sg * s_A[lr][pi][0];
                        e[1] = sg * s_A[lr][pi][1];
                        e[2] = sg * s_A[lr][pi][2];
                        e[3] = s_b[lr][2 * pi + sgn];
                    }
                }
            }
            if (pi == 0) B.hp_cnt[chunk * per_pair + x] = (count > HP_CAP) ? (unsigned char)HP_OVERFLOW : (unsigned char)count;
            if (pi == 0 && count > HP_CAP) atomicAdd(&B.hp_slow[p], 1);
        }
    }
}

__device__ __noinline__ void row_from_generators(const double* __restrict__ ob, const double* __restrict__ LG,
                                                 double c0, double c1, double c2, double* max_out, double* A0o,
                                                 double* A1o, double* A2o) {
    double G[9][3], oc[3];
    load_row_generators(ob, LG, G, oc);
    double max_elt = -100000000, A0 = 0, A1 = 0, A2 = 0;
    for_each_plane(G, oc, [&](int, double a0, double a1, double a2, double d, double dl, bool nz) {
        if (!nz) return;
        const double dot = a0 * c0 + a1 * c1 + a2 * c2;
        const double pos = dot - (d + dl);
        const double neg = -dot - (-d + dl);
        if (pos > max_elt) {
            max_elt = pos;
            A0 = -a0; A1 = -a1; A2 = -a2;
        }
        if (neg > max_elt) {
            max_elt = neg;
            A0 = a0; A1 = a1; A2 = a2;
        }
    });
    *max_out = max_elt;
    *A0o = A0;
    *A1o = A1;
    *A2o = A2;
}

__device__ __forceinline__ void slice_component(const uint16_t* __restrict__ keys, const double* __restrict__ coef,
                                                int n, int kstride, int cstride, const double2 (*kpd)[4], double& value,
                                                double (&grad)[NF]) {
    constexpr int CH = K3_CH;
    for (int m0 = 0; m0 < n; m0 += CH) {
        unsigned kk[CH];
        double cc[CH];
#pragma unroll
        for (int i = 0; i < CH; i++) {
            const bool on = m0 + i < n;
            kk[i] = on ? keys[(m0 + i) * kstride] : 0u;
            cc[i] = on ? coef[(m0 + i) * cstride] : 0.0;
        }
#pragma unroll 1
        for (int i = 0; i < CH; i++) {
            if (m0 + i >= n) break;
            const unsigned key = kk[0];
            double val = cc[0];
#pragma unroll
            for (int q = 0; q + 1 < CH; q++) {
                kk[q] = kk[q + 1];
                cc[q] = cc[q + 1];
            }
            double D[NF];
#pragma unroll
            for (int j = 0; j < NF; j++) {
                const double2 fd = kpd[j][(key >> (2 * j)) & 3];
                D[j] = val * fd.y;
#pragma unroll
                for (int v = 0; v < j; v++) D[v] *= fd.x;
                val *= fd.x;
            }
            value += val;
#pragma unroll
            for (int v = 0; v < NF; v++) grad[v] += D[v];
        }
    }
}

__device__ __forceinline__ unsigned smem_u32(const void* p) { return (unsigned)__cvta_generic_to_shared(p); }
__device__ __forceinline__ void mbar_init(unsigned long long* bar, unsigned count) {
    asm volatile("mbarrier.init.shared::cta.b64 [%0], %1;" ::"r"(smem_u32(bar)), "r"(count) : "memory");
}
__device__ __forceinline__ void mbar_arrive_expect_tx(unsigned long long* bar, unsigned bytes) {
    asm volatile("mbarrier.arrive.expect_tx.shared::cta.b64 _, [%0], %1;" ::"r"(smem_u32(bar)), "r"(bytes) : "memory");
}
__device__ __forceinline__ void bulk_g2s(void* dst, const void* src, unsigned bytes, unsigned long long* bar) {
    asm volatile("cp.async.bulk.shared::cluster.global.mbarrier::complete_tx::bytes [%0], [%1], %2, [%3];" ::"r"(smem_u32(dst)),
                 "l"(src), "r"(bytes), "r"(smem_u32(bar))
                 : "memory");
}
__device__ __forceinline__ void mbar_wait(unsigned long long* bar, unsigned parity) {
    unsigned ok;
    do {
        asm volatile("{\n\t.reg .pred p;\n\tmbarrier.try_wait.parity.shared::cta.b64 p, [%1], %2;\n\tselp.u32 %0, 1, 0, p;\n\t}"
                     : "=r"(ok)
                     : "r"(smem_u32(bar)), "r"(parity)
                     : "memory");
    } while (!ok);
}
#ifndef K3_STAGE_CAND
#define K3_STAGE_CAND 0
#endif
constexpr int K3_CAND_ARENA = 36864;
#ifndef K3_STAGE_TABLES
#define K3_STAGE_TABLES 0
#endif
#ifndef K3_DIRECT_J
#define K3_DIRECT_J 1
#endif
constexpr int K3_LSLOT = 12;
constexpr int K3_USLOT = 32;
constexpr int K3_LTAB_BYTES = 32 + K3_LSLOT * 24;
constexpr int K3_UTAB_BYTES = K3_USLOT * 2 + K3_USLOT * 8;
__device__ __forceinline__ void cp_async16(void* dst, const void* src) {
    asm volatile("cp.async.ca.shared.global [%0], [%1], 16;" ::"r"((unsigned)__cvta_generic_to_shared(dst)), "l"(src) : "memory");
}
#ifndef K3_SKIP_ZERO_DK
#define K3_SKIP_ZERO_DK 0
#endif
#ifndef K3_STREAM_STORES
#define K3_STREAM_STORES 0
#endif
#if K3_STREAM_STORES
#define K3_ST2(p, a, b) __stcs(reinterpret_cast<double2*>(p), make_double2(a, b))
#define K3_ST1(p, a) __stcs(p, a)
#else
#define K3_ST2(p, a, b) (*reinterpret_cast<double2*>(p) = make_double2(a, b))
#define K3_ST1(p, a) (*(p) = (a))
#endif
#ifndef K3_LD_NOALLOC
#define K3_LD_NOALLOC 0
#endif
#ifndef K3_LD256
#define K3_LD256 1
#endif
#ifndef K3_POWER_TABLES
#define K3_POWER_TABLES 1
#endif
constexpr int PT_LO = 64, PT_LO_STRIDE = 4;
constexpr int PT_HI = 256, PT_HI_STRIDE = 6;
__device__ __forceinline__ void power_and_slope(double k, int d, double& f, double& fp) {
    f = d == 0 ? 1.0 : d == 1 ? k : d == 2 ? k * k : k * k * k;
    fp = d == 0 ? 0.0 : d == 1 ? 1.0 : d == 2 ? 2.0 * k : 3.0 * (k * k);
}
template <int NV>
__device__ __forceinline__ void power_table_entry(const double* __restrict__ k, int v0, int e, double* out) {
    double f[NV], fp[NV];
#pragma unroll
    for (int i = 0; i < NV; i++) power_and_slope(k[v0 + i], (e >> (2 * i)) & 3, f[i], fp[i]);
    double M = f[0];
#pragma unroll
    for (int i = 1; i < NV; i++) M *= f[i];
    out[0] = M;
#pragma unroll
    for (int i = 0; i < NV; i++) {
        double G = fp[i];
#pragma unroll
        for (int u = 0; u < NV; u++)
            if (u != i) G *= f[u];
        out[1 + i] = G;
    }
}
__device__ __forceinline__ void slice_component_pt(const uint16_t* __restrict__ keys, const double* __restrict__ coef, int n,
                                                   int kstride, int cstride, const double* __restrict__ pt_lo,
                                                   const double* __restrict__ pt_hi, double& value, double (&grad)[NF]) {
    constexpr int CH = K3_CH;
    for (int m0 = 0; m0 < n; m0 += CH) {
        unsigned kk[CH];
        double cc[CH];
#pragma unroll
        for (int i = 0; i < CH; i++) {
            const bool on = m0 + i < n;
            kk[i] = on ? keys[(m0 + i) * kstride] : 0u;
            cc[i] = on ? coef[(m0 + i) * cstride] : 0.0;
        }
#pragma unroll
        for (int i = 0; i < CH; i++) {
            const double2* L = reinterpret_cast<const double2*>(pt_lo + (kk[i] & (PT_LO - 1)) * PT_LO_STRIDE);
            const double2* H = reinterpret_cast<const double2*>(pt_hi + ((kk[i] >> 6) & (PT_HI - 1)) * PT_HI_STRIDE);
            const double2 l0 = L[0], l1 = L[1], h0 = H[0], h1 = H[1], h2 = H[2];
            const double cl = cc[i] * l0.x, ch = cc[i] * h0.x;
            value = fma(cl, h0.x, value);
            grad[0] = fma(ch, l0.y, grad[0]);
            grad[1] = fma(ch, l1.x, grad[1]);
            grad[2] = fma(ch, l1.y, grad[2]);
            grad[3] = fma(cl, h0.y, grad[3]);
            grad[4] = fma(cl, h1.x, grad[4]);
            grad[5] = fma(cl, h1.y, grad[5]);
            grad[6] = fma(cl, h2.x, grad[6]);
        }
    }
}
constexpr int K3_LINK_THREADS = ((TB * 3 * MAXJ + 31) / 32) * 32;
#ifndef K3_TORQUE_LANES_N
#define K3_TORQUE_LANES_N 2
#endif
constexpr int K3_TORQUE_LANES = K3_TORQUE_LANES_N;
constexpr int K3_THREADS = K3_LINK_THREADS + ((TB * NF * K3_TORQUE_LANES + 31) / 32) * 32;
constexpr int K3_CNT_SMEM = 2048;
constexpr int K3_WARPS = K3_THREADS / 32;
constexpr int K3_TORQUE_T0 = K3_LINK_THREADS;
static_assert(TB * 3 * MAXJ <= K3_LINK_THREADS && K3_TORQUE_T0 + TB * NF * K3_TORQUE_LANES <= K3_THREADS,
              "thread map of the slice phase");

#if K3_POWER_TABLES
#define K3_SLICE slice_component_pt
#define K3_SLICE_TABLES pt_lo, pt_hi
#else
#define K3_SLICE slice_component
#define K3_SLICE_TABLES kpd
#endif
__global__ void __launch_bounds__(K3_THREADS, K3_MINB)
k_constraints(Batch B, const double* __restrict__ kin, double* __restrict__ g, double* __restrict__ jac) {
    const int tb = blockIdx.x, p = B.plist ? B.plist[blockIdx.y] : int(blockIdx.y);
    const int NJ = B.NJ, O = B.O, T = B.T;
    const int m = B.m();
    const int tid = threadIdx.x, lane = tid & 31, warp = tid >> 5;
#if K3_POWER_TABLES
    __shared__ __align__(16) double pt_lo[PT_LO * PT_LO_STRIDE];
    __shared__ __align__(16) double pt_hi[PT_HI * PT_HI_STRIDE];
#else
    __shared__ double2 kpd[NF][4];
#endif
    __shared__ __align__(4) unsigned char s_cnt[K3_CNT_SMEM];
    __shared__ double s_lc[TB][MAXJ][3];
    __shared__ double s_dlc[TB][MAXJ][NF][3];
#if !K3_DIRECT_J
    __shared__ double s_stage[K3_WARPS][32 * NF];
#endif
    __shared__ double s_tj[TB * NF * NF];
    extern __shared__ __align__(16) unsigned char k3_tab[];
    __shared__ unsigned long long s_bar;
    __shared__ int s_in_domain;
    __shared__ int s_next;

    if (B.failed(p) != 0) {
        double* gp0 = g ? g + size_t(p) * m : nullptr;
        double* jp0 = jac ? jac + size_t(p) * m * NF : nullptr;
        for (int i = tid; i < TB * NF; i += K3_THREADS) {
            if (gp0) gp0[size_t(tb) * TB * NF + i] = 1e300;
            if (jp0)
                for (int v = 0; v < NF; v++) jp0[(size_t(tb) * TB * NF + i) * NF + v] = 0.0;
        }
        for (int x = tid; x < NJ * TB * O; x += K3_THREADS) {
            const int o = x % O, ltt = x / O, tt = ltt % TB, l = ltt / TB;
            const size_t r = size_t(NF) * T + (size_t(l) * T + tb * TB + tt) * O + o;
            if (gp0) gp0[r] = 1e300;
            if (jp0)
                for (int v = 0; v < NF; v++) jp0[r * NF + v] = 0.0;
        }
        if (tb == 0 && tid < 4 * NF) {
            const size_t r = size_t(NF) * T + size_t(NJ) * T * O + tid;
            if (gp0) gp0[r] = 0.0;
            if (jp0)
                for (int v = 0; v < NF; v++) jp0[r * NF + v] = 0.0;
        }
        return;
    }
#if K3_STAGE_CAND
    const int rows_all = NJ * TB * O;
    const int rows_staged = rows_all < K3_CAND_ARENA / 64 ? rows_all : K3_CAND_ARENA / 64;
    double* const s_rec = reinterpret_cast<double*>(k3_tab + (K3_STAGE_TABLES ? TB * (NJ * K3_LTAB_BYTES + NF * K3_UTAB_BYTES) : 0));
    if (tid == 0) {
        mbar_init(&s_bar, 1);
        asm volatile("fence.mbarrier_init.release.cluster;" ::: "memory");
        const double* src = B.hp_cand + (size_t(p) * (T / TB) + tb) * B.hp_chunk();
        const unsigned bytes = unsigned(rows_staged) * 32u;
        mbar_arrive_expect_tx(&s_bar, rows_staged > 0 ? 2 * bytes : 0);
        if (rows_staged > 0) {
            bulk_g2s(s_rec, src, bytes, &s_bar);
            bulk_g2s(s_rec + size_t(rows_staged) * 4, src + size_t(rows_all) * 4, bytes, &s_bar);
        }
    }
#endif
#ifndef K3_PREFETCH_L2
#define K3_PREFETCH_L2 0
#endif
#if K3_PREFETCH_L2
    {
        const char* c0p = reinterpret_cast<const char*>(B.hp_cand + (size_t(p) * (T / TB) + tb) * B.hp_chunk());
        const int lines = (NJ * TB * O * 32 * 2 + 127) / 128;
        for (int i = tid; i < lines; i += K3_THREADS) asm volatile("prefetch.global.L2 [%0];" ::"l"(c0p + size_t(i) * 128));
    }
#endif
    if (tid == 32) {
        bool in = true;
        for (int j = 0; j < NF; j++) in = in && (fabs(kin[size_t(p) * NF + j]) <= K_DOMAIN);
        s_in_domain = in ? 1 : 0;
        s_next = 0;
    }
#if K3_POWER_TABLES
    for (int q = tid; q < PT_HI + PT_LO; q += K3_THREADS) {
        if (q < PT_HI) {
            power_table_entry<4>(kin + size_t(p) * NF, 3, q, pt_hi + q * PT_HI_STRIDE);
            pt_hi[q * PT_HI_STRIDE + 5] = 0.0;
        } else {
            power_table_entry<3>(kin + size_t(p) * NF, 0, q - PT_HI, pt_lo + (q - PT_HI) * PT_LO_STRIDE);
        }
    }
#else
    if (tid < NF) {
        const double k = kin[size_t(p) * NF + tid];
        kpd[tid][0] = make_double2(1.0, 0.0);
        kpd[tid][1] = make_double2(k, 1.0);
        kpd[tid][2] = make_double2(k * k, 2.0 * k);
        kpd[tid][3] = make_double2(k * k * k, 3.0 * (k * k));
    }
#endif
    const int per_pair = NJ * TB * O;
    const size_t chunk = size_t(p) * (T / TB) + tb;
    const bool cnt_in_smem = per_pair <= K3_CNT_SMEM;
    __syncthreads();

    double* gp = g ? g + size_t(p) * m : nullptr;
    double* jp = jac ? jac + size_t(p) * m * NF : nullptr;

    if (tid < K3_LINK_THREADS) {
        constexpr int CW = (K3_CNT_SMEM / 4 + K3_LINK_THREADS - 1) / K3_LINK_THREADS;
        unsigned cw[CW];
        if (cnt_in_smem) {
            const unsigned* src = reinterpret_cast<const unsigned*>(B.hp_cnt + chunk * per_pair);
#pragma unroll
            for (int q = 0; q < CW; q++) cw[q] = (tid + q * K3_LINK_THREADS < per_pair / 4) ? __ldg(src + tid + q * K3_LINK_THREADS) : 0u;
        }
        const bool slicer = tid < TB * NJ * 3;
        const int e = tid % 3;
        const int l = (tid / 3) % NJ;
        const int tt = slicer ? tid / (3 * NJ) : 0;
        const size_t idx = (size_t(p) * T + tb * TB + tt) * NJ + l;
        const int n = slicer ? B.link_n[idx] : 0;
#if K3_STAGE_TABLES
        unsigned char* slot = k3_tab + (tt * NJ + l) * K3_LTAB_BYTES;
        const int ns = n < K3_LSLOT ? n : K3_LSLOT;
        if (slicer) {
            const char* ksrc = reinterpret_cast<const char*>(B.link_key + idx * B.capL);
            const char* csrc = reinterpret_cast<const char*>(B.link_g + idx * B.capL * 3);
            const int kc = (ns * 2 + 15) >> 4, cc = (ns * 24 + 15) >> 4;
            if (e == 0)
                for (int c = 0; c < kc; c++) cp_async16(slot + 16 * c, ksrc + 16 * c);
            for (int c = e; c < cc; c += 3) cp_async16(slot + 32 + 16 * c, csrc + 16 * c);
        }
        asm volatile("cp.async.commit_group;" ::: "memory");
        asm volatile("cp.async.wait_group 0;" ::: "memory");
        __syncwarp();
        asm volatile("bar.sync 4, %0;" ::"n"(K3_LINK_THREADS) : "memory");
#endif
        if (slicer) {
            double value = B.link_c[idx * 3 + e];
            double grad[NF] = {0, 0, 0, 0, 0, 0, 0};
#if K3_STAGE_TABLES
            K3_SLICE(reinterpret_cast<const uint16_t*>(slot), reinterpret_cast<const double*>(slot + 32) + e, ns, 1, 3, K3_SLICE_TABLES,
                            value, grad);
            if (n > ns)
                K3_SLICE(B.link_key + idx * B.capL + ns, B.link_g + (idx * B.capL + ns) * 3 + e, n - ns, 1, 3, K3_SLICE_TABLES, value, grad);
#else
            K3_SLICE(B.link_key + idx * B.capL, B.link_g + idx * B.capL * 3 + e, n, 1, 3, K3_SLICE_TABLES, value, grad);
#endif
            const double r = B.link_r[idx * 3 + e];
            const double c = ((value - r) + (value + r)) * 0.5;
            s_lc[tt][l][e] = c;
            if (p == 0) B.link_sliced[((size_t(tb) * TB + tt) * NJ + l) * 3 + e] = c;
#pragma unroll
            for (int v = 0; v < NF; v++) s_dlc[tt][l][v][e] = grad[v];
        }
        if (cnt_in_smem) {
#pragma unroll
            for (int q = 0; q < CW; q++)
                if (tid + q * K3_LINK_THREADS < per_pair / 4) reinterpret_cast<unsigned*>(s_cnt)[tid + q * K3_LINK_THREADS] = cw[q];
        }
        asm volatile("bar.sync 1, %0;" ::"n"(K3_LINK_THREADS) : "memory");
        asm volatile("bar.arrive 2, %0;" ::"n"(K3_THREADS) : "memory");
    } else {
        const int tq = tid - K3_TORQUE_T0;
        const int i = tq / K3_TORQUE_LANES, part = tq % K3_TORQUE_LANES;
        double value = 0.0;
        double grad[NF] = {0, 0, 0, 0, 0, 0, 0};
        const bool on = i < TB * NF;
        const size_t idx = (size_t(p) * T + tb * TB) * NF + (on ? i : 0);
        if (on) {
            const int n = B.u_n[idx];
#if K3_STAGE_TABLES
            unsigned char* slot = k3_tab + TB * NJ * K3_LTAB_BYTES + i * K3_UTAB_BYTES;
            const int ns = n < K3_USLOT ? n : K3_USLOT;
            {
                const char* ksrc = reinterpret_cast<const char*>(B.u_key + idx * B.capU);
                const char* csrc = reinterpret_cast<const char*>(B.u_g + idx * B.capU);
                const int kc = (ns * 2 + 15) >> 4, cc = (ns * 8 + 15) >> 4;
                for (int c = part; c < kc; c += K3_TORQUE_LANES) cp_async16(slot + 16 * c, ksrc + 16 * c);
                for (int c = part; c < cc; c += K3_TORQUE_LANES) cp_async16(slot + K3_USLOT * 2 + 16 * c, csrc + 16 * c);
            }
        }
        asm volatile("cp.async.commit_group;" ::: "memory");
        asm volatile("cp.async.wait_group 0;" ::: "memory");
        __syncwarp();
        asm volatile("bar.sync 5, %0;" ::"n"(K3_THREADS - K3_LINK_THREADS) : "memory");
        if (on) {
            const int n = B.u_n[idx];
            unsigned char* slot = k3_tab + TB * NJ * K3_LTAB_BYTES + i * K3_UTAB_BYTES;
            const int ns = n < K3_USLOT ? n : K3_USLOT;
            const int mine_s = (ns - part + K3_TORQUE_LANES - 1) / K3_TORQUE_LANES;
            K3_SLICE(reinterpret_cast<const uint16_t*>(slot) + part, reinterpret_cast<const double*>(slot + K3_USLOT * 2) + part,
                            mine_s > 0 ? mine_s : 0, K3_TORQUE_LANES, K3_TORQUE_LANES, K3_SLICE_TABLES, value, grad);
            if (n > ns) {
                const int rest = (n - ns - part + K3_TORQUE_LANES - 1) / K3_TORQUE_LANES;
                K3_SLICE(B.u_key + idx * B.capU + ns + part, B.u_g + idx * B.capU + ns + part, rest > 0 ? rest : 0,
                                K3_TORQUE_LANES, K3_TORQUE_LANES, K3_SLICE_TABLES, value, grad);
            }
#else
            const int mine = (n - part + K3_TORQUE_LANES - 1) / K3_TORQUE_LANES;
            K3_SLICE(B.u_key + idx * B.capU + part, B.u_g + idx * B.capU + part, mine > 0 ? mine : 0,
                            K3_TORQUE_LANES, K3_TORQUE_LANES, K3_SLICE_TABLES, value, grad);
#endif
        }
#pragma unroll
        for (int d = 1; d < K3_TORQUE_LANES; d <<= 1) {
            value += __shfl_xor_sync(0xffffffffu, value, d);
#pragma unroll
            for (int v = 0; v < NF; v++) grad[v] += __shfl_xor_sync(0xffffffffu, grad[v], d);
        }
        double* st = s_tj;
        if (on && part == 0) {
            value = B.u_c[idx] + value;
            const double r = B.u_r[idx];
            if (gp) gp[tb * TB * NF + i] = ((value - r) + (value + r)) * 0.5;
#pragma unroll
            for (int v = 0; v < NF; v++) st[i * NF + v] = grad[v];
        }
        asm volatile("bar.sync 3, %0;" ::"n"(K3_THREADS - K3_LINK_THREADS) : "memory");
        if (jp) {
            double* dst = jp + size_t(tb) * TB * NF * NF;
            for (int q = tq; q < TB * NF * NF; q += K3_THREADS - K3_TORQUE_T0) dst[q] = st[q];
        }
        asm volatile("bar.sync 3, %0;" ::"n"(K3_THREADS - K3_LINK_THREADS) : "memory");
        asm volatile("bar.sync 2, %0;" ::"n"(K3_THREADS) : "memory");
    }

    const double* cand = B.hp_cand + chunk * B.hp_chunk();
    const unsigned char* cnt = B.hp_cnt + chunk * per_pair;
    const size_t cstride2 = size_t(per_pair) * 2;
    const bool in_domain = s_in_domain != 0;
    const float inv_O = O > 0 ? 1.0f / float(O) : 0.0f;
#if !K3_DIRECT_J
    double* stage = &s_stage[warp][0];
#endif
#if K3_STAGE_CAND
    mbar_wait(&s_bar, 0);
#endif
    for (;;) {
        int x0 = 0;
        if (lane == 0) x0 = atomicAdd(&s_next, 1) * 32;
        x0 = __shfl_sync(0xffffffffu, x0, 0);
        if (x0 >= per_pair) break;
        const int x = x0 + lane;
        bool active = x < per_pair;
        double max_elt = -100000000;
        double A0 = 0, A1 = 0, A2 = 0;
        int l = 0, tt = 0, o = 0;
        if (active) {
            const int ltt = __float2int_rz((float(x) + 0.5f) * inv_O);
            o = x - ltt * O;
            tt = ltt % TB;
            l = ltt / TB;
            const double c0 = s_lc[tt][l][0], c1 = s_lc[tt][l][1], c2 = s_lc[tt][l][2];
            const int n = cnt_in_smem ? s_cnt[x] : cnt[x];
            if (n != HP_OVERFLOW && in_domain) {
                const double2* row = reinterpret_cast<const double2*>(cand) + size_t(x) * 2;
                for (int q0 = 0; q0 < n; q0 += K3_CQ) {
                    double2 u[K3_CQ], w[K3_CQ];
#if K3_STAGE_CAND
                    static_assert(K3_CQ == 2, "the staged levels are the first pass of the scan");
                    if (q0 == 0 && x < rows_staged) {
                        const double2* sr = reinterpret_cast<const double2*>(s_rec) + size_t(x) * 2;
                        u[0] = sr[0];
                        w[0] = sr[1];
                        if (n > 1) {
                            u[1] = sr[size_t(rows_staged) * 2];
                            w[1] = sr[size_t(rows_staged) * 2 + 1];
                        }
                    } else
#endif
#pragma unroll
                    for (int i = 0; i < K3_CQ; i++) {
                        if (q0 + i < n) {
#if K3_LD256
#if K3_LD_NOALLOC
                            asm volatile("ld.global.nc.L1::no_allocate.v4.f64 {%0, %1, %2, %3}, [%4];"
#else
                            asm volatile("ld.global.nc.v4.f64 {%0, %1, %2, %3}, [%4];"
#endif
                                         : "=d"(u[i].x), "=d"(u[i].y), "=d"(w[i].x), "=d"(w[i].y)
                                         : "l"(row + (q0 + i) * cstride2));
#else
                            u[i] = __ldg(row + (q0 + i) * cstride2);
                            w[i] = __ldg(row + (q0 + i) * cstride2 + 1);
#endif
                        }
                    }
#pragma unroll
                    for (int i = 0; i < K3_CQ; i++) {
                        if (q0 + i < n) {
                            const double v = (u[i].x * c0 + u[i].y * c1 + w[i].x * c2) - w[i].y;
                            if (v > max_elt) {
                                max_elt = v;
                                A0 = -u[i].x; A1 = -u[i].y; A2 = -w[i].x;
                            }
                        }
                    }
                }
            } else {
                active = false;
            }
        }
        const long long row_i = active ? (long long)(size_t(NF) * T + (size_t(l) * T + tb * TB + tt) * O + o) : -1;
        if (gp && active) gp[row_i] = -max_elt;
#if K3_DIRECT_J
#if K3_SKIP_ZERO_DK
        const int lmax = __reduce_max_sync(0xffffffffu, active ? l : 0);
#endif
        if (jp && active) {
            double* out = jp + row_i * NF;
            double jv[NF];
#pragma unroll
            for (int v = 0; v < NF; v++) {
#if K3_SKIP_ZERO_DK
                if (v > lmax) {
                    jv[v] = 0.0;
                    continue;
                }
#endif
                const double* dk = s_dlc[tt][l][v];
                jv[v] = A0 * dk[0] + A1 * dk[1] + A2 * dk[2];
            }
            if ((row_i & 1) == 0) {
                K3_ST2(out, jv[0], jv[1]);
                K3_ST2(out + 2, jv[2], jv[3]);
                K3_ST2(out + 4, jv[4], jv[5]);
                K3_ST1(out + 6, jv[6]);
            } else {
                K3_ST1(out, jv[0]);
                K3_ST2(out + 1, jv[1], jv[2]);
                K3_ST2(out + 3, jv[3], jv[4]);
                K3_ST2(out + 5, jv[5], jv[6]);
            }
        }
#else
        if (jp) {
            if (active) {
#pragma unroll
                for (int v = 0; v < NF; v++) {
                    const double* dk = s_dlc[tt][l][v];
                    stage[lane * NF + v] = A0 * dk[0] + A1 * dk[1] + A2 * dk[2];
                }
            }
            __syncwarp();
#pragma unroll
            for (int q = 0; q < NF; q++) {
                const int e = q * 32 + lane;
                const int r = e / NF;
                const long long rr = __shfl_sync(0xffffffffu, row_i, r);
                if (rr >= 0) jp[rr * NF + (e - r * NF)] = stage[e];
            }
            __syncwarp();
        }
#endif
    }

    if (tb == 0 && tid < NF) {
        const int i = tid;
        const double D = c_robot.duration;
        const double q0 = B.q0[size_t(p) * NF + i];
        const double a = B.qd0[size_t(p) * NF + i] * D;
        const double b = B.qdd0[size_t(p) * NF + i] * D * D;
        const double kn = kin[size_t(p) * NF + i];
        const int off = NF * T + NJ * T * O;
        for (int vel = 0; vel < 2; vel++) {
            double mn, mx, dmn, dmx;
            bez_extrema(vel == 1, q0, a, b, c_robot.k_range[i], D, kn, &mn, &mx, &dmn, &dmx);
            const int r0 = off + vel * 2 * NF + i;
            if (gp) {
                gp[r0] = mn;
                gp[r0 + NF] = mx;
            }
            if (jp) {
                for (int j = 0; j < NF; j++) {
                    jp[size_t(r0) * NF + j] = (j == i) ? dmn : 0.0;
                    jp[size_t(r0 + NF) * NF + j] = (j == i) ? dmx : 0.0;
                }
            }
        }
    }
}

#undef K3_SLICE
#undef K3_SLICE_TABLES
constexpr int K3S_PROBLEMS = 16;
__global__ void __launch_bounds__(128)
k_constraints_slow(Batch B, const double* __restrict__ kin, double* __restrict__ g, double* __restrict__ jac) {
    asm volatile("griddepcontrol.launch_dependents;" ::: "memory");
    const int NJ = B.NJ, O = B.O, T = B.T;
    __shared__ int s_list[K3S_PROBLEMS], s_n;
    __shared__ double2 kpd[NF][4];
    if (threadIdx.x == 0) s_n = 0;
    __syncthreads();
    if (threadIdx.x < K3S_PROBLEMS) {
        const int i = blockIdx.x * K3S_PROBLEMS + threadIdx.x;
        if (i < B.nprob && O > 0) {
            const int p = B.plist ? B.plist[i] : i;
            if (B.failed(p) == 0) {
                bool in = true;
                for (int j = 0; j < NF; j++) in = in && (fabs(kin[size_t(p) * NF + j]) <= K_DOMAIN);
                if (!in || B.hp_slow[p] != 0) s_list[atomicAdd(&s_n, 1)] = p;
            }
        }
    }
    __syncthreads();
    const int nlist = s_n;
    for (int li = 0; li < nlist; li++) {
    const int p = s_list[li];
    bool in = true;
    for (int j = 0; j < NF; j++) in = in && (fabs(kin[size_t(p) * NF + j]) <= K_DOMAIN);
    __syncthreads();
    if (threadIdx.x < NF) {
        const double k = kin[size_t(p) * NF + threadIdx.x];
        kpd[threadIdx.x][0] = make_double2(1.0, 0.0);
        kpd[threadIdx.x][1] = make_double2(k, 1.0);
        kpd[threadIdx.x][2] = make_double2(k * k, 2.0 * k);
        kpd[threadIdx.x][3] = make_double2(k * k * k, 3.0 * (k * k));
    }
    __syncthreads();
    const int m = B.m();
    const int per_chunk = NJ * TB * O;
    double* gp = g ? g + size_t(p) * m : nullptr;
    double* jp = jac ? jac + size_t(p) * m * NF : nullptr;
    for (int r = threadIdx.x; r < per_chunk * (T / TB); r += blockDim.x) {
        const int tb = r / per_chunk, x = r - tb * per_chunk;
        const size_t chunk = size_t(p) * (T / TB) + tb;
        if (in && B.hp_cnt[chunk * per_chunk + x] != HP_OVERFLOW) continue;
        const int o = x % O, ltt = x / O, tt = ltt % TB, l = ltt / TB;
        const size_t idx = (size_t(p) * T + tb * TB + tt) * NJ + l;
        double c[3], dk[NF][3];
        const int n = B.link_n[idx];
        for (int e = 0; e < 3; e++) {
            double value = B.link_c[idx * 3 + e];
            double grad[NF] = {0, 0, 0, 0, 0, 0, 0};
            for (int mI = 0; mI < n; mI++) {
                const unsigned key = B.link_key[idx * B.capL + mI];
                double val = B.link_g[(idx * B.capL + mI) * 3 + e];
                double D[NF];
#pragma unroll
                for (int j = 0; j < NF; j++) {
                    const double2 fd = kpd[j][(key >> (2 * j)) & 3];
                    D[j] = val * fd.y;
#pragma unroll
                    for (int v = 0; v < j; v++) D[v] *= fd.x;
                    val *= fd.x;
                }
                value += val;
#pragma unroll
                for (int v = 0; v < NF; v++) grad[v] += D[v];
            }
            const double rr = B.link_r[idx * 3 + e];
            c[e] = ((value - rr) + (value + rr)) * 0.5;
#pragma unroll
            for (int v = 0; v < NF; v++) dk[v][e] = grad[v];
        }
        double r_max, A0, A1, A2;
        row_from_generators(B.obstacles + (size_t(p) * O + o) * 12, B.link_gens + idx * 18, c[0], c[1], c[2], &r_max, &A0, &A1, &A2);
        const size_t row = size_t(NF) * T + (size_t(l) * T + tb * TB + tt) * O + o;
        if (gp) gp[row] = -r_max;
        if (jp)
            for (int v = 0; v < NF; v++) jp[row * NF + v] = A0 * dk[v][0] + A1 * dk[v][1] + A2 * dk[v][2];
    }
    }
}

__host__ __device__ inline int jac_link_width(int l) { return l + 1 < NF ? l + 1 : NF; }
__host__ __device__ inline long long jac_nnz(int T, int NJ, int O) {
    long long w = 0;
    for (int l = 0; l < NJ; l++) w += jac_link_width(l);
    return (long long)NF * NF * T + (long long)T * O * w + 4 * NF;
}
__global__ void __launch_bounds__(256)
k_pack_jacobian(Batch B, const double* __restrict__ jac, double* __restrict__ out, long long nnz) {
    const int p = blockIdx.y;
    const int T = B.T, NJ = B.NJ, O = B.O;
    const long long idx = (long long)blockIdx.x * blockDim.x + threadIdx.x;
    if (idx >= nnz) return;
    const double* jp = jac + size_t(p) * B.m() * NF;
    long long row, col;
    const long long n_t = (long long)NF * NF * T;
    if (idx < n_t) {
        row = idx / NF;
        col = idx % NF;
    } else {
        long long r = idx - n_t;
        int l = 0;
        for (; l < NJ; l++) {
            const long long blk = (long long)T * O * jac_link_width(l);
            if (r < blk) break;
            r -= blk;
        }
        if (l < NJ) {
            const int w = jac_link_width(l);
            row = (long long)NF * T + (long long)l * T * O + r / w;
            col = r % w;
        } else {
            row = (long long)NF * T + (long long)NJ * T * O + r;
            col = r % NF;
        }
    }
    out[size_t(p) * nnz + idx] = jp[row * NF + col];
}
cudaError_t launch_pack_jacobian(const Batch& B, const double* d_jac, double* d_out, cudaStream_t st) {
    if (B.nprob == 0) return cudaSuccess;
    const long long nnz = jac_nnz(B.T, B.NJ, B.O);
    dim3 grid((unsigned)((nnz + 255) / 256), B.nprob);
    k_pack_jacobian<<<grid, 256, 0, st>>>(B, d_jac, d_out, nnz);
    return cudaGetLastError();
}

__global__ void __launch_bounds__(256)
k_verdict(Batch B, const double* __restrict__ g, int* __restrict__ feasible, int* __restrict__ first) {
    const int p = blockIdx.x;
    const int T = B.T, NJ = B.NJ, O = B.O, m = B.m();
    const double* gp = g + size_t(p) * m;
    const double* tr = B.torque_radius + size_t(p) * NF * T;
    int best = m;
    for (int r = threadIdx.x; r < m; r += blockDim.x) {
        const double v = gp[r];
        bool bad;
        if (r < NF * T) {
            const int t = r / NF, j = r % NF;
            const double rad = tr[j * T + t];
            bad = v < -c_robot.torque_limits[j] + rad - c_robot.torque_violation_threshold ||
                  v > c_robot.torque_limits[j] - rad + c_robot.torque_violation_threshold;
        } else if (r < NF * T + NJ * T * O) {
            bad = v > c_robot.collision_violation_threshold;
        } else {
            const int q = r - (NF * T + NJ * T * O);
            const int j = q % NF;
            if (q < 2 * NF)
                bad = v < c_robot.state_limits_lb[j] + c_robot.qe || v > c_robot.state_limits_ub[j] - c_robot.qe;
            else
                bad = v < -c_robot.speed_limits[j] + c_robot.qde || v > c_robot.speed_limits[j] - c_robot.qde;
        }
        if (bad && r < best) best = r;
    }
    __shared__ int s_best;
    if (threadIdx.x == 0) s_best = m;
    __syncthreads();
    atomicMin(&s_best, best);
    __syncthreads();
    if (threadIdx.x == 0) {
        feasible[p] = (s_best == m) ? 1 : 0;
        first[p] = (s_best == m) ? -1 : s_best;
    }
}

cudaError_t launch_hyperplanes(const Batch& B, cudaStream_t st, const int* unit_flag = nullptr, HpStage stage = HpStage{nullptr, nullptr, nullptr, nullptr}) {
    if (B.O == 0 || B.nprob == 0) return cudaSuccess;
    const int rows = B.NJ * B.T * B.O;
    dim3 grid((rows + HP_ROWS - 1) / HP_ROWS, B.nprob);
    if (unit_flag) {
        cudaLaunchConfig_t cfg = {};
        cfg.gridDim = grid;
        cfg.blockDim = dim3(HP_THREADS);
        cfg.dynamicSmemBytes = 0;
        cfg.stream = st;
        cudaLaunchAttribute attr[1];
        attr[0].id = cudaLaunchAttributeProgrammaticStreamSerialization;
        attr[0].val.programmaticStreamSerializationAllowed = 1;
        cfg.attrs = attr;
        cfg.numAttrs = 1;
        return cudaLaunchKernelEx(&cfg, k_hyperplanes, B, unit_flag, stage);
    }
    k_hyperplanes<<<grid, HP_THREADS, 0, st>>>(B, unit_flag, stage);
    return cudaGetLastError();
}
cudaError_t launch_constraints(const Batch& B, const double* d_k, double* d_g, double* d_jac, cudaStream_t st) {
    if (B.nprob == 0) return cudaSuccess;
#ifdef K3_CARVEOUT_KNOB
    {
        static int done = 0;
        if (!done) {
            done = 1;
            const char* v = std::getenv("ARMOUR_K3_CARVEOUT");
            if (v) {
                cudaError_t ec = cudaFuncSetAttribute(k_constraints, cudaFuncAttributePreferredSharedMemoryCarveout, std::atoi(v));
                std::printf("k_constraints carve-out %s %%: %s\n", v, cudaGetErrorString(ec));
            }
        }
    }
#endif
    dim3 grid(B.T / TB, B.nprob);
    const int rows_all = B.NJ * TB * B.O;
    const size_t dyn = (K3_STAGE_TABLES ? size_t(TB) * (B.NJ * K3_LTAB_BYTES + NF * K3_UTAB_BYTES) : 0) +
                       (K3_STAGE_CAND ? size_t(rows_all < K3_CAND_ARENA / 64 ? rows_all : K3_CAND_ARENA / 64) * 64 : 0);
    if (B.O == 0) {
        k_constraints<<<grid, K3_THREADS, dyn, st>>>(B, d_k, d_g, d_jac);
        return cudaGetLastError();
    }
    k_constraints_slow<<<(B.nprob + K3S_PROBLEMS - 1) / K3S_PROBLEMS, 128, 0, st>>>(B, d_k, d_g, d_jac);
    cudaError_t e = cudaGetLastError();
    if (e != cudaSuccess) return e;
    cudaLaunchConfig_t cfg = {};
    cfg.gridDim = grid;
    cfg.blockDim = dim3(K3_THREADS);
    cfg.dynamicSmemBytes = dyn;
    cfg.stream = st;
    cudaLaunchAttribute attr[1];
    attr[0].id = cudaLaunchAttributeProgrammaticStreamSerialization;
    attr[0].val.programmaticStreamSerializationAllowed = 1;
    cfg.attrs = attr;
    cfg.numAttrs = 1;
    return cudaLaunchKernelEx(&cfg, k_constraints, B, d_k, d_g, d_jac);
}
cudaError_t launch_verdict(const Batch& B, const double* d_g, int* d_feasible, int* d_first, cudaStream_t st) {
    if (B.nprob == 0) return cudaSuccess;
    k_verdict<<<B.nprob, 256, 0, st>>>(B, d_g, d_feasible, d_first);
    return cudaGetLastError();
}

}
```

### armour_b200/csrc/layout.h

```cpp
#pragma once
#include <cstdint>

#include "robot_constants.h"

namespace armour {

#ifndef ARMOUR_TB
#define ARMOUR_TB 8
#endif
constexpr int TB = ARMOUR_TB;
constexpr int HP_CAP = 32;
constexpr int HP_OVERFLOW = 255;
constexpr double K_DOMAIN = 1.0 + 1e-6;
constexpr double HP_RHO_SCALE = 1.0 + 3e-5;

struct Batch {
    int nprob;
    int T;
    int NJ;
    int O;
    int capL;
    int capU;
    int epoch;
    const double* q0;
    const double* qd0;
    const double* qdd0;
    const double* obstacles;
    const double* jrs_ext;
    int* link_n;
    double* link_c;
    uint16_t* link_key;
    double* link_g;
    int* u_n;
    double* u_c;
    double* u_r;
    uint16_t* u_key;
    double* u_g;
    double* torque_radius;
    double* link_gens;
    double* link_r;
    double* hp_cand;
    unsigned char* hp_cnt;
    int* hp_slow;
    double* link_sliced;
    int* status;
    const int* plist;

    __host__ __device__ size_t hp_chunk() const { return size_t(HP_CAP) * 4 * NJ * TB * O; }
    __host__ __device__ int m() const { return NF * T + NJ * T * O + 4 * NF; }
    __device__ int failed(int p) const { return (status[p] >> 3) == epoch ? (status[p] & 7) : 0; }
};

}
```

### armour_b200/planner.py

```python
from __future__ import annotations

import ctypes as C

import numpy as np

from . import _lib
from ._lib import NF, ArmourError


def _f64(a):
    return np.ascontiguousarray(a, dtype=np.float64)


def _dp(a):
    return a.ctypes.data_as(_lib.dp)


class ReachSetEngine:
    def __init__(self, max_problems=1, max_obstacles=40, device=0, robot_model=0, num_time_steps=128,
                 simplify_threshold=5e-4, k_range=None, cap_link=32, cap_torque=64, cap_work=768,
                 mass_uncertainty=-1.0, inertia_uncertainty=-1.0):
        self.lib = _lib.load()
        cfg = _lib.Config()
        self.lib.armour_config_default(C.byref(cfg))
        cfg.device = device
        cfg.robot_model = robot_model
        cfg.num_time_steps = num_time_steps
        cfg.max_obstacles = max_obstacles
        cfg.max_problems = max_problems
        cfg.cap_link_monomials = cap_link
        cfg.cap_torque_monomials = cap_torque
        cfg.cap_work_monomials = cap_work
        cfg.simplify_threshold = simplify_threshold
        if k_range is not None:
            for i in range(NF):
                cfg.k_range[i] = float(k_range[i])
        cfg.mass_uncertainty = mass_uncertainty
        cfg.inertia_uncertainty = inertia_uncertainty
        self.cfg = cfg
        self._h = C.c_void_p()
        rc = self.lib.armour_ctx_create(C.byref(cfg), C.byref(self._h))
        if rc != 0:
            self._h = None
            raise ArmourError(rc, "armour_ctx_create failed (" + self.lib.armour_status_string(rc).decode() +
                              "); a CUDA device is required, there is no CPU fallback")
        self.T = self.lib.armour_num_time_steps(self._h)
        self.NJ = self.lib.armour_num_joints(self._h)
        self.nobs = 0
        self.nprob = 0

    def close(self):
        if getattr(self, "_h", None):
            self.lib.armour_ctx_destroy(self._h)
            self._h = None

    def __del__(self):
        try:
            self.close()
        except Exception:
            pass

    def _check(self, rc):
        if rc != 0:
            raise ArmourError(rc, self.lib.armour_status_string(rc).decode() + ": " +
                              self.lib.armour_last_error(self._h).decode())

    def set_stream(self, cuda_stream_handle):
        self._check(self.lib.armour_ctx_set_stream(self._h, C.c_void_p(cuda_stream_handle)))

    def synchronize(self):
        self._check(self.lib.armour_ctx_synchronize(self._h))

    @property
    def kernel_launches(self):
        return int(self.lib.armour_kernel_launches(self._h))

    @property
    def m(self):
        return self.lib.armour_num_constraints(self._h, self.nobs)

    def build(self, q0, qd0, qdd0, obstacles):
        q0, qd0, qdd0 = _f64(q0).reshape(-1, NF), _f64(qd0).reshape(-1, NF), _f64(qdd0).reshape(-1, NF)
        nprob = q0.shape[0]
        obs = _f64(obstacles)
        obs = obs.reshape(nprob, -1, 12) if obs.size else np.zeros((nprob, 0, 12))
        nobs = obs.shape[1]
        self._check(self.lib.armour_batch_reachsets_build(self._h, nprob, _dp(q0), _dp(qd0), _dp(qdd0), _dp(obs), nobs))
        self.nprob, self.nobs = nprob, nobs
        return self

    def build_device(self, nprob, nobs, d_q0, d_qd0, d_qdd0, d_obstacles):
        self._check(self.lib.armour_batch_reachsets_build_device(self._h, nprob, d_q0, d_qd0, d_qdd0, d_obstacles, nobs))
        self.nprob, self.nobs = nprob, nobs

    def build_status(self):
        out = np.zeros(self.nprob, np.int32)
        self._check(self.lib.armour_batch_get_build_status(self._h, self.nprob, out.ctypes.data_as(_lib.ip)))
        return out

    def monomial_counts(self):
        ln = np.zeros((self.nprob, self.T, self.NJ), np.int32)
        un = np.zeros((self.nprob, self.T, NF), np.int32)
        self._check(self.lib.armour_batch_get_monomial_counts(self._h, self.nprob, ln.ctypes.data_as(_lib.ip),
                                                              un.ctypes.data_as(_lib.ip)))
        return ln, un

    def candidate_counts(self):
        C_ = self.lib.armour_chunk_intervals()
        out = np.zeros((self.nprob, self.T // C_, self.NJ, C_, max(self.nobs, 0)), np.uint8)
        if out.size:
            self._check(self.lib.armour_batch_get_candidate_counts(self._h, self.nprob, out.ctypes.data_as(C.c_void_p)))
        return out

    def solve(self, q_des, max_iter=None, tol=None, qp_sweeps=None, qp_update_budget=None):
        q_des = np.ascontiguousarray(np.asarray(q_des, dtype=np.float64).reshape(self.nprob, NF))
        opt = _lib.SolverOptions()
        self.lib.armour_solver_options_default(C.byref(opt))
        if max_iter is not None:
            opt.max_iter = int(max_iter)
        if tol is not None:
            opt.tol = float(tol)
        if qp_sweeps is not None:
            opt.qp_sweeps = int(qp_sweeps)
        if qp_update_budget is not None:
            opt.qp_update_budget = int(qp_update_budget)
        k = np.empty((self.nprob, NF))
        ok = np.zeros(self.nprob, np.int32)
        first = np.zeros(self.nprob, np.int32)
        iters = np.zeros(self.nprob, np.int32)
        self._check(self.lib.armour_batch_solve(self._h, self.nprob, _dp(q_des), C.byref(opt), _dp(k),
                                                ok.ctypes.data_as(_lib.ip), first.ctypes.data_as(_lib.ip),
                                                iters.ctypes.data_as(_lib.ip)))
        return k, ok.astype(bool), first, iters

    def rollout(self, start, goal, obstacles, max_replans=100, goal_radius=0.05, lookahead=0.1, audit_samples=16,
                max_iter=None, tol=None, torque_tol=None, collision_tol=None, qp_sweeps=None):
        start, goal = _f64(start).reshape(-1, NF), _f64(goal).reshape(-1, NF)
        n = start.shape[0]
        obs = _f64(obstacles)
        obs = obs.reshape(n, -1, 12) if obs.size else np.zeros((n, 0, 12))
        opt = _lib.RolloutOptions()
        self.lib.armour_rollout_options_default(C.byref(opt))
        opt.max_replans, opt.goal_radius, opt.lookahead = int(max_replans), float(goal_radius), float(lookahead)
        opt.audit_samples = int(audit_samples)
        for name, v in (("max_iter", max_iter), ("tol", tol), ("torque_tol", torque_tol), ("collision_tol", collision_tol),
                        ("qp_sweeps", qp_sweeps)):
            if v is not None:
                setattr(opt.solver, name, type(getattr(opt.solver, name))(v))
        R = opt.max_replans
        res = dict(outcome=np.zeros(n, np.int32), replans=np.zeros(n, np.int32), infeasible=np.zeros(n, np.int32),
                   final_state=np.zeros((n, 3 * NF)), min_clearance=np.zeros(n), log_state=np.zeros((max(R, 0), n, 3 * NF)),
                   log_q_des=np.zeros((max(R, 0), n, NF)), log_k=np.zeros((max(R, 0), n, NF)),
                   log_int=np.zeros((max(R, 0), n, 4), np.int32), log_clearance=np.zeros((max(R, 0), n)))
        out = _lib.RolloutOut()
        for name, a in res.items():
            setattr(out, name, a.ctypes.data_as(_lib.ip if a.dtype == np.int32 else _lib.dp))
        self._check(self.lib.armour_batch_rollout(self._h, n, _dp(start), _dp(goal), _dp(obs), obs.shape[1], C.byref(opt),
                                                  C.byref(out)))
        self.nprob = 0
        return res

    def clearance(self, q, obstacles, world=None):
        q = _f64(q).reshape(-1, NF)
        n = q.shape[0]
        obs = _f64(obstacles)
        nobs = obs.shape[-2] if obs.size else 0
        obs = obs.reshape(-1, nobs, 12) if obs.size else np.zeros((1, 0, 12))
        w = None if world is None else np.ascontiguousarray(np.asarray(world, dtype=np.int32).reshape(n))
        if w is not None and (w.min() < 0 or w.max() >= obs.shape[0]):
            raise ValueError("world index outside the obstacle sets")
        clr = np.empty(n)
        which = np.empty(n, np.int32)
        self._check(self.lib.armour_batch_clearance(self._h, n, _dp(q), w.ctypes.data_as(_lib.ip) if w is not None else None,
                                                    _dp(obs), nobs, _dp(clr), which.ctypes.data_as(_lib.ip)))
        return clr, which

    def measure_fp64_peak(self):
        v = C.c_double(0)
        self._check(self.lib.armour_measure_fp64_peak(self._h, C.byref(v)))
        return v.value

    def torque_radius(self):
        out = np.empty((self.nprob, NF, self.T))
        self._check(self.lib.armour_batch_get_torque_radius(self._h, self.nprob, _dp(out)))
        return out

    def link_independent_generators(self):
        out = np.empty((self.nprob, self.T, self.NJ, 6, 3))
        self._check(self.lib.armour_batch_get_link_independent_generators(self._h, self.nprob, _dp(out)))
        return out.transpose(0, 1, 2, 4, 3)

    def get_bounds_info(self):
        gl, gu = np.empty((self.nprob, self.m)), np.empty((self.nprob, self.m))
        self._check(self.lib.armour_batch_get_bounds(self._h, self.nprob, _dp(gl), _dp(gu)))
        return gl, gu

    def eval(self, k, want_g=True, want_jac=True):
        k = _f64(k).reshape(-1, NF)
        n = k.shape[0]
        g = np.empty((n, self.m)) if want_g else None
        jac = np.empty((n, self.m, NF)) if want_jac else None
        self._check(self.lib.armour_batch_eval(self._h, n, _dp(k), _dp(g) if want_g else None,
                                               _dp(jac) if want_jac else None))
        return g, jac

    def eval_g(self, k):
        return self.eval(k, True, False)[0]

    def eval_jac_g(self, k):
        return self.eval(k, False, True)[1]

    def eval_into(self, k, g, jac):
        n = k.shape[0]
        self._check(self.lib.armour_batch_eval(self._h, n, _dp(k), _dp(g) if g is not None else None,
                                               _dp(jac) if jac is not None else None))

    @property
    def jacobian_nnz(self):
        return int(self.lib.armour_jacobian_nnz(self._h, self.nobs))

    def jacobian_structure(self):
        n = self.jacobian_nnz
        ir, jc = np.zeros(n, np.int32), np.zeros(n, np.int32)
        self._check(self.lib.armour_jacobian_structure(self._h, self.nobs, ir.ctypes.data_as(_lib.ip), jc.ctypes.data_as(_lib.ip)))
        return ir, jc

    def eval_structured(self, k, want_g=True):
        k = _f64(k).reshape(-1, NF)
        n = k.shape[0]
        g = np.empty((n, self.m)) if want_g else None
        vals = np.empty((n, self.jacobian_nnz))
        self._check(self.lib.armour_batch_eval_structured(self._h, n, _dp(k), _dp(g) if want_g else None, _dp(vals)))
        return g, vals

    def eval_structured_into(self, k, g, vals):
        self._check(self.lib.armour_batch_eval_structured(self._h, k.shape[0], _dp(k), _dp(g) if g is not None else None, _dp(vals)))

    def eval_device(self, nprob, d_k, d_g, d_jac):
        self._check(self.lib.armour_batch_eval_device(self._h, nprob, d_k, d_g or None, d_jac or None))

    def verdict_device(self, nprob, d_g, d_feasible, d_first):
        self._check(self.lib.armour_batch_verdict_device(self._h, nprob, d_g, d_feasible, d_first))

    def finalize_solution(self, g):
        g = _f64(g)
        ok, first = C.c_int(0), C.c_int(-1)
        self._check(self.lib.armour_verdict(self._h, _dp(g), C.byref(ok), C.byref(first)))
        return bool(ok.value), first.value

    def cost(self, q_des, k):
        q_des, k = _f64(q_des), _f64(k)
        obj, grad = C.c_double(0), np.empty(NF)
        self._check(self.lib.armour_cost(self._h, _dp(q_des), _dp(k), C.byref(obj), _dp(grad)))
        return obj.value, grad

    def link_sliced_center(self):
        out = np.empty((self.T, self.NJ, 3))
        self._check(self.lib.armour_get_link_sliced_center(self._h, _dp(out)))
        return out

    def _tables(self, r):
        t = _lib.ReachsetTables()
        t.cap_link, t.cap_u = r["hl"].shape[1], r["hu"].shape[1]
        t.link_n = r["nl"].ctypes.data_as(_lib.ip)
        t.link_center = _dp(r["cl"])
        t.link_key = r["hl"].ctypes.data_as(_lib.up)
        t.link_coeff = _dp(r["gl"])
        t.u_n = r["nu"].ctypes.data_as(_lib.ip)
        t.u_center = _dp(r["cu"])
        t.u_key = r["hu"].ctypes.data_as(_lib.up)
        t.u_coeff = _dp(r["gu"])
        t.u_radius = _dp(r["ru"])
        t.torque_radius = _dp(r["torque_radius"])
        t.link_gens = _dp(r["link_gens"])
        return t

    def import_reachsets(self, prob, nprob_total, tables, q0, qd0, qdd0, obstacles):
        obs = _f64(obstacles).reshape(-1, 12)
        q0, qd0, qdd0 = _f64(q0), _f64(qd0), _f64(qdd0)
        t = self._tables(tables)
        self._check(self.lib.armour_import_reachsets(self._h, prob, nprob_total, C.byref(t), _dp(q0), _dp(qd0),
                                                     _dp(qdd0), _dp(obs), obs.shape[0]))
        self.nobs = obs.shape[0]
        if prob == nprob_total - 1:
            self.nprob = nprob_total

    def export_reachsets(self, prob=0):
        T, NJ = self.T, self.NJ
        cl, cu = self.cfg.cap_link_monomials, self.cfg.cap_torque_monomials
        r = dict(nl=np.zeros(T * NJ, np.int32), cl=np.zeros((T * NJ, 3)), hl=np.zeros((T * NJ, cl), np.uint64),
                 gl=np.zeros((T * NJ, cl, 3)), nu=np.zeros(T * NF, np.int32), cu=np.zeros(T * NF),
                 hu=np.zeros((T * NF, cu), np.uint64), gu=np.zeros((T * NF, cu)), ru=np.zeros(T * NF),
                 torque_radius=np.zeros((NF, T)), link_gens=np.zeros((T, NJ, 18)))
        t = self._tables(r)
        self._check(self.lib.armour_export_reachsets(self._h, prob, C.byref(t)))
        return r
```

### include/armour_b200.h

```cpp
#ifndef ARMOUR_B200_H
#define ARMOUR_B200_H

#ifdef __cplusplus
extern "C" {
#endif

#define ARMOUR_NF 7
#define ARMOUR_ABI_VERSION 1

enum {
    ARMOUR_OK = 0,
    ARMOUR_ERR_ARG = -1,
    ARMOUR_ERR_CUDA = -2,
    ARMOUR_ERR_OBSTACLES = -3,
    ARMOUR_ERR_CAPACITY = -4,
    ARMOUR_ERR_STATE = -5,
    ARMOUR_ERR_NOMEM = -6
};

typedef struct armour_ctx armour_ctx;

typedef struct armour_config {
    int struct_size;
    int device;
    int robot_model;
    int num_time_steps;
    int max_obstacles;
    int max_problems;
    int cap_link_monomials;
    int cap_torque_monomials;
    int cap_work_monomials;
    double simplify_threshold;
    double k_range[ARMOUR_NF];
    double mass_uncertainty;
    double inertia_uncertainty;
} armour_config;

int armour_config_default(armour_config* cfg);
int armour_ctx_create(const armour_config* cfg, armour_ctx** out);
int armour_ctx_destroy(armour_ctx* ctx);
int armour_ctx_reserve(armour_ctx* ctx, int nprob, int nobs);
int armour_ctx_set_stream(armour_ctx* ctx, void* cuda_stream);
int armour_ctx_synchronize(armour_ctx* ctx);
const char* armour_status_string(int status);
const char* armour_last_error(const armour_ctx* ctx);
int armour_abi_version(void);
long long armour_kernel_launches(const armour_ctx* ctx);

int armour_num_joints(const armour_ctx* ctx);
int armour_num_time_steps(const armour_ctx* ctx);
int armour_num_constraints(const armour_ctx* ctx, int nobs);


int armour_reachsets_build(armour_ctx* ctx, const double q0[ARMOUR_NF], const double qd0[ARMOUR_NF],
                           const double qdd0[ARMOUR_NF], const double* obstacles, int nobs);
int armour_get_torque_radius(armour_ctx* ctx, double* out);
int armour_get_link_independent_generators(armour_ctx* ctx, double* out);
int armour_get_bounds(armour_ctx* ctx, double* g_l, double* g_u);
int armour_eval_g(armour_ctx* ctx, const double k[ARMOUR_NF], double* g);
int armour_eval_jac_g(armour_ctx* ctx, const double k[ARMOUR_NF], double* values);
int armour_eval_g_jac(armour_ctx* ctx, const double k[ARMOUR_NF], double* g, double* values);
long long armour_jacobian_nnz(const armour_ctx* ctx, int nobs);
int armour_jacobian_structure(const armour_ctx* ctx, int nobs, int* iRow, int* jCol);
int armour_eval_jac_g_structured(armour_ctx* ctx, const double k[ARMOUR_NF], double* values_nnz);
int armour_get_link_sliced_center(armour_ctx* ctx, double* out);
int armour_verdict(armour_ctx* ctx, const double* g, int* feasible, int* first_violation);
int armour_cost(armour_ctx* ctx, const double q_des[ARMOUR_NF], const double k[ARMOUR_NF], double* obj,
                double grad[ARMOUR_NF]);


int armour_batch_reachsets_build(armour_ctx* ctx, int nprob, const double* q0, const double* qd0, const double* qdd0,
                                 const double* obstacles, int nobs);
int armour_batch_eval(armour_ctx* ctx, int nprob, const double* k, double* g, double* values);
int armour_batch_eval_structured(armour_ctx* ctx, int nprob, const double* k, double* g, double* values_nnz);
int armour_batch_eval_structured_device(armour_ctx* ctx, int nprob, const double* d_k, double* d_g, double* d_values_nnz);
int armour_batch_eval_device(armour_ctx* ctx, int nprob, const double* d_k, double* d_g, double* d_values);
int armour_batch_reachsets_build_device(armour_ctx* ctx, int nprob, const double* d_q0, const double* d_qd0,
                                        const double* d_qdd0, const double* d_obstacles, int nobs);
int armour_batch_verdict_device(armour_ctx* ctx, int nprob, const double* d_g, int* d_feasible, int* d_first);
int armour_batch_get_torque_radius(armour_ctx* ctx, int nprob, double* out );
int armour_batch_get_link_independent_generators(armour_ctx* ctx, int nprob, double* out );
int armour_batch_get_bounds(armour_ctx* ctx, int nprob, double* g_l, double* g_u);
typedef struct armour_solver_options {
    int max_iter;
    double tol;
    double torque_tol;
    double collision_tol;
    int qp_sweeps;
    int qp_update_budget;
} armour_solver_options;
void armour_solver_options_default(armour_solver_options* opt);
int armour_batch_solve_device(armour_ctx* ctx, int nprob, const double* d_q_des, const armour_solver_options* opt,
                              double* d_k_opt, int* d_feasible, int* d_first_violation, int* d_iterations);
int armour_batch_solve(armour_ctx* ctx, int nprob, const double* q_des, const armour_solver_options* opt, double* k_opt,
                       int* feasible, int* first_violation, int* iterations);
int armour_batch_get_build_status(armour_ctx* ctx, int nprob, int* out);
int armour_batch_get_monomial_counts(armour_ctx* ctx, int nprob, int* link_n, int* u_n);
int armour_batch_get_candidate_counts(armour_ctx* ctx, int nprob, unsigned char* out);
int armour_chunk_intervals(void);
int armour_measure_fp64_peak(armour_ctx* ctx, double* tflops);

enum { ARMOUR_ROLLOUT_BUDGET = 0, ARMOUR_ROLLOUT_ARRIVED = 1, ARMOUR_ROLLOUT_COLLISION = 2, ARMOUR_ROLLOUT_LIMIT = 3 };
typedef struct armour_rollout_options {
    int struct_size;
    int max_replans;
    double lookahead;
    double goal_radius;
    int audit_samples;
    armour_solver_options solver;
} armour_rollout_options;
void armour_rollout_options_default(armour_rollout_options* opt);
typedef struct armour_rollout_out {
    int* outcome;
    int* replans;
    int* infeasible;
    double* final_state;
    double* min_clearance;
    double* log_state;
    double* log_q_des;
    double* log_k;
    int* log_int;
    double* log_clearance;
} armour_rollout_out;
int armour_batch_rollout_device(armour_ctx* ctx, int nworlds, const double* d_start, const double* d_goal, const double* d_obstacles,
                                int nobs, const armour_rollout_options* opt, const armour_rollout_out* d_out);
int armour_batch_rollout(armour_ctx* ctx, int nworlds, const double* start, const double* goal, const double* obstacles, int nobs,
                         const armour_rollout_options* opt, const armour_rollout_out* out);
int armour_batch_clearance_device(armour_ctx* ctx, int nconf, const double* d_q, const int* d_world, const double* d_obstacles,
                                  int nobs, double* d_clearance, int* d_which);
int armour_batch_clearance(armour_ctx* ctx, int nconf, const double* q, const int* world, const double* obstacles, int nobs,
                           double* clearance, int* which);


typedef struct armour_reachset_tables {
    int cap_link, cap_u;
    int* link_n;
    double* link_center;
    unsigned long long* link_key;
    double* link_coeff;
    int* u_n;
    double* u_center;
    unsigned long long* u_key;
    double* u_coeff;
    double* u_radius;
    double* torque_radius;
    double* link_gens;
} armour_reachset_tables;

int armour_export_reachsets(armour_ctx* ctx, int prob, armour_reachset_tables* out);
int armour_import_reachsets(armour_ctx* ctx, int prob, int nprob_total, const armour_reachset_tables* in,
                            const double q0[ARMOUR_NF], const double qd0[ARMOUR_NF], const double qdd0[ARMOUR_NF],
                            const double* obstacles, int nobs);

typedef struct armour_controller armour_controller;
typedef struct armour_controller_gains {
    const double* Kr;
    double alpha;
    double V_max;
    double r_norm_threshold;
    int apply_friction;
} armour_controller_gains;
int armour_controller_create(const char* model_file, double model_uncertainty, int device, armour_controller** out);
const char* armour_controller_create_error(void);
void armour_controller_destroy(armour_controller* ctl);
int armour_controller_num_joints(const armour_controller* ctl);
const char* armour_controller_last_error(const armour_controller* ctl);
long long armour_controller_kernel_launches(const armour_controller* ctl);
int armour_controller_set_stream(armour_controller* ctl, void* cuda_stream);
int armour_controller_synchronize(armour_controller* ctl);
int armour_controller_get_interval_model(const armour_controller* ctl, double* out);
int armour_controller_rnea(armour_controller* ctl, int n, const double* q, const double* qd, const double* qda,
                           const double* qdd, int apply_friction, int apply_gravity, double* tau, double* tau_lo,
                           double* tau_hi);
int armour_controller_rnea_device(armour_controller* ctl, int n, const double* d_q, const double* d_qd,
                                  const double* d_qda, const double* d_qdd, const double* d_sincos, int apply_friction,
                                  int apply_gravity, double* d_tau, double* d_tau_lo, double* d_tau_hi);
int armour_controller_update(armour_controller* ctl, int n, const armour_controller_gains* gains, const double* q,
                             const double* qd, const double* q_des, const double* qd_des, const double* qdd_des, double* u,
                             double* u_nominal, double* v, int* status);
int armour_controller_update_device(armour_controller* ctl, int n, const armour_controller_gains* gains, const double* d_q,
                                    const double* d_qd, const double* d_q_des, const double* d_qd_des,
                                    const double* d_qdd_des, const double* d_sincos, double* d_u, double* d_u_nominal,
                                    double* d_v, int* d_status);

int armour_armtd_ctx_create(const armour_config* cfg, armour_ctx** out);
int armour_armtd_build(armour_ctx* ctx, const double q0[ARMOUR_NF], const double qd0[ARMOUR_NF], const double* jrs,
                       const double k_range[ARMOUR_NF], const double* obstacles, int nobs);
int armour_armtd_num_constraints(const armour_ctx* ctx);
int armour_armtd_eval(armour_ctx* ctx, const double k[ARMOUR_NF], double* g, double* values);
int armour_armtd_get_bounds(armour_ctx* ctx, double* g_l, double* g_u);
int armour_armtd_verdict(armour_ctx* ctx, const double* g, int* feasible, int* first_violation);
int armour_armtd_cost(armour_ctx* ctx, const double q_des[ARMOUR_NF], const double k[ARMOUR_NF], double* obj, double* grad);
int armour_armtd_get_link_sliced_center(armour_ctx* ctx, double* out);
int armour_armtd_get_link_independent_generators(armour_ctx* ctx, double* out);

int armour_armtd_batch_ctx_create(const armour_config* cfg, armour_ctx** out);
int armour_armtd_batch_build(armour_ctx* ctx, int nprob, const double* q0, const double* qd0, const double* jrs,
                             const double* k_range, const double* obstacles, int nobs);
int armour_armtd_batch_build_device(armour_ctx* ctx, int nprob, const double* d_q0, const double* d_qd0, const double* d_jrs,
                                    const double* d_k_range, const double* d_obstacles, int nobs, const double* d_sincos);
int armour_armtd_batch_eval(armour_ctx* ctx, int nprob, const double* k, double* g, double* values);
int armour_armtd_batch_eval_device(armour_ctx* ctx, int nprob, const double* d_k, double* d_g, double* d_values);
int armour_armtd_batch_verdict_device(armour_ctx* ctx, int nprob, const double* d_g, int* d_feasible, int* d_first);
int armour_armtd_batch_cost(armour_ctx* ctx, int nprob, const double* q_des, const double* k, double* obj, double* grad);
int armour_armtd_batch_get_link_independent_generators(armour_ctx* ctx, int nprob, double* out);
int armour_armtd_batch_solve(armour_ctx* ctx, int nprob, const double* q_des, const armour_solver_options* opt, double* k_opt,
                             int* feasible, int* first_violation, int* iterations);
int armour_armtd_batch_solve_device(armour_ctx* ctx, int nprob, const double* d_q_des, const armour_solver_options* opt,
                                    double* d_k_opt, int* d_feasible, int* d_first_violation, int* d_iterations);

#ifdef __cplusplus
}
#endif
#endif
```

Measured before the change: 1.994 million.

## Pack per-chunk evaluation image with compacted hyperplane records and tables

Adds a pack kernel after reach-set build that compacts the hyperplane candidate records (prefix sum over counts, stored contiguously per chunk) and copies the link and torque monomial tables, centers and radii into a single per-chunk byte image. The constraint kernel then reads candidates through per-warp group offsets and a shuffle prefix sum instead of strided fixed-capacity rows. It also drops the disabled TMA and shared-memory staging paths. The aim is denser, more contiguous memory reads in the eval loop, at the cost of an extra build-time launch and more bookkeeping per warp.

```diff
diff --git a/armour_b200/_lib.py b/armour_b200/_lib.py
--- a/armour_b200/_lib.py
+++ b/armour_b200/_lib.py
@@ -75,6 +75,8 @@
     "armour_batch_get_monomial_counts": (C.c_int, [C.c_void_p, C.c_int, ip, ip]),
     "armour_batch_get_candidate_counts": (C.c_int, [C.c_void_p, C.c_int, C.c_void_p]),
     "armour_chunk_intervals": (C.c_int, []),
+    "armour_eval_image_layout": (C.c_int, [C.c_void_p, C.POINTER(C.c_longlong)]),
+    "armour_batch_get_eval_images": (C.c_int, [C.c_void_p, C.c_int, C.c_void_p]),
     "armour_jacobian_nnz": (C.c_longlong, [C.c_void_p, C.c_int]),
     "armour_jacobian_structure": (C.c_int, [C.c_void_p, C.c_int, ip, ip]),
     "armour_eval_jac_g_structured": (C.c_int, [C.c_void_p, dp, dp]),
diff --git a/armour_b200/csrc/armour_capi.cu b/armour_b200/csrc/armour_capi.cu
--- a/armour_b200/csrc/armour_capi.cu
+++ b/armour_b200/csrc/armour_capi.cu
@@ -100,7 +100,8 @@
     cudaStream_t own_stream = nullptr;
     Batch B;
     int built_nprob = 0;
-    size_t hp_capacity = 0;
+    size_t img_capacity = 0;
+    size_t cnt_capacity = 0;
     int hp_nprob = 0;
     int* d_unit_flag = nullptr;
     size_t obs_capacity = 0;
@@ -203,23 +204,26 @@
     Batch& B = ctx->B;
     B.O = nobs;
     B.nprob = nprob;
-    const size_t need_hp = size_t(nprob) * (B.T / TB) * B.hp_chunk();
-    if (ctx->hp_capacity < need_hp || ctx->hp_nprob < nprob) {
-        if (B.hp_cand) cudaFree(B.hp_cand);
+    const size_t need_img = size_t(nprob) * (B.T / TB) * B.img_chunk();
+    const size_t need_cnt = size_t(nprob) * B.T * B.NJ * nobs;
+    if (ctx->img_capacity < need_img || ctx->hp_nprob < nprob || ctx->cnt_capacity < need_cnt) {
+        if (B.img) cudaFree(B.img);
         if (B.hp_cnt) cudaFree(B.hp_cnt);
         if (B.hp_slow) cudaFree(B.hp_slow);
-        B.hp_cand = nullptr;
+        B.img = nullptr;
         B.hp_cnt = nullptr;
         B.hp_slow = nullptr;
-        ctx->hp_capacity = 0;
+        ctx->img_capacity = 0;
+        ctx->cnt_capacity = 0;
         ctx->hp_nprob = 0;
         ctx->built_nprob = 0;
         const size_t np = std::max(nprob, ctx->hp_nprob);
-        CU(dalloc(&B.hp_cand, need_hp));
-        CU(dalloc(&B.hp_cnt, need_hp / (HP_CAP * 4)));
+        CU(dalloc(&B.img, need_img));
+        CU(dalloc(&B.hp_cnt, need_cnt));
         CU(dalloc(&B.hp_slow, np));
         CU(cudaMemsetAsync(B.hp_slow, 0, np * sizeof(int), ctx->stream));
-        ctx->hp_capacity = need_hp;
+        ctx->img_capacity = need_img;
+        ctx->cnt_capacity = need_cnt;
         ctx->hp_nprob = nprob;
     }
     B.obstacles = ctx->d_obs;
@@ -403,9 +407,6 @@
         if ((e = cudaFuncGetAttributes(&fa, k1lat::k_reachsets)) != cudaSuccess) return bail("load k_reachsets", e);
         if ((e = cudaFuncGetAttributes(&fa, k_hyperplanes)) != cudaSuccess) return bail("load k_hyperplanes", e);
         if ((e = cudaFuncGetAttributes(&fa, k_constraints)) != cudaSuccess) return bail("load k_constraints", e);
-        if ((e = cudaFuncSetAttribute(k_constraints, cudaFuncAttributeMaxDynamicSharedMemorySize,
-                                      TB * (MAXJ * K3_LTAB_BYTES + NF * K3_UTAB_BYTES) + K3_CAND_ARENA)) != cudaSuccess)
-            return bail("k_constraints shared memory", e);
         if ((e = cudaFuncGetAttributes(&fa, k_constraints_slow)) != cudaSuccess) return bail("load k_constraints_slow", e);
         if ((e = cudaFuncGetAttributes(&fa, k_verdict)) != cudaSuccess) return bail("load k_verdict", e);
     }
@@ -420,7 +421,7 @@
     Batch& B = ctx->B;
     void* ptrs[] = {ctx->d_roll, ctx->d_roll_i, ctx->d_stage, ctx->d_solver, ctx->d_solver_i, ctx->d_solver_io, ctx->d_unit_flag, ctx->d_jnz, ctx->d_jrs, ctx->d_armtd_in, ctx->d_ga, ctx->d_ja,
                     ctx->d_in, ctx->d_obs, ctx->d_k, ctx->d_g, ctx->d_jac, ctx->d_verdict, B.link_n, B.link_c,
-                    B.link_key, B.link_g, B.u_n, B.u_c, B.u_r, B.u_key, B.u_g, B.torque_radius, B.link_gens, B.link_r, B.hp_cand, B.hp_cnt, B.hp_slow,
+                    B.link_key, B.link_g, B.u_n, B.u_c, B.u_r, B.u_key, B.u_g, B.torque_radius, B.link_gens, B.link_r, B.img, B.hp_cnt, B.hp_slow,
                     B.link_sliced, B.status};
     for (void* p : ptrs)
         if (p) cudaFree(p);
@@ -496,6 +497,8 @@
         CU(cudaMemcpyAsync(ctx->d_in + 2 * P * NF, d_qdd0, nb, cudaMemcpyDeviceToDevice, ctx->stream));
         { int rc2 = launch_build(ctx, ctx->B, &nl, &latency); if (rc2) return rc2; }
     }
+    CU(launch_pack_image(ctx->B, ctx->stream));
+    nl++;
     ctx->launches += nl;
     ctx->built_nprob = nprob;
     ctx->h_torque_valid = false;
@@ -527,6 +530,8 @@
     ctx->launches += nl;
     CU(launch_hyperplanes(ctx->B, ctx->stream, (latency && nobs > 0) ? ctx->d_unit_flag : nullptr));
     ctx->launches += (nobs > 0);
+    CU(launch_pack_image(ctx->B, ctx->stream));
+    ctx->launches++;
     ctx->built_nprob = nprob;
     ctx->h_torque_valid = false;
     ctx->h_q0.assign(q0, q0 + size_t(nprob) * NF);
@@ -586,6 +591,21 @@
 }
 
 int armour_chunk_intervals(void) { return TB; }
+
+int armour_eval_image_layout(armour_ctx* ctx, long long* layout) {
+    if (!ctx || !layout) return ARMOUR_ERR_ARG;
+    const Batch& B = ctx->B;
+    const size_t v[10] = {B.img_chunk(), 0, B.img_ut(), B.img_lc(), B.img_lr(), B.img_uc(), B.img_ur(), B.img_grp(), B.img_cnt(), B.img_hdr()};
+    for (int i = 0; i < 10; i++) layout[i] = (long long)v[i];
+    return ARMOUR_OK;
+}
+
+int armour_batch_get_eval_images(armour_ctx* ctx, int nprob, void* out) {
+    if (!ctx || !out || nprob < 1 || nprob > ctx->built_nprob) return ARMOUR_ERR_ARG;
+    CU(cudaMemcpyAsync(out, ctx->B.img, size_t(nprob) * (ctx->B.T / TB) * ctx->B.img_chunk(), cudaMemcpyDeviceToHost, ctx->stream));
+    CU(cudaStreamSynchronize(ctx->stream));
+    return ARMOUR_OK;
+}
 
 #ifdef K1_PROFILE
 extern "C" int armour_debug_k1_profile(long long* out, int reset) {
@@ -1397,6 +1417,8 @@
         if (nobs > 0) CU(cudaMemsetAsync(ctx->B.hp_slow, 0, size_t(nprob_total) * sizeof(int), ctx->stream));
         CU(launch_hyperplanes(ctx->B, ctx->stream));
         ctx->launches += (nobs > 0);
+        CU(launch_pack_image(ctx->B, ctx->stream));
+        ctx->launches++;
         ctx->built_nprob = nprob_total;
         ctx->h_torque_valid = false;
     }
diff --git a/armour_b200/csrc/k3_constraints.cuh b/armour_b200/csrc/k3_constraints.cuh
--- a/armour_b200/csrc/k3_constraints.cuh
+++ b/armour_b200/csrc/k3_constraints.cuh
@@ -259,8 +259,8 @@
     __syncthreads();
     if (live) {
         const size_t chunk = size_t(p) * (T / TB) + tb;
-        double* row = B.hp_cand + chunk * B.hp_chunk() + size_t(x) * 4;
-        const size_t cstride = size_t(per_pair) * 4;
+        double* row = reinterpret_cast<double*>(B.img + chunk * B.img_chunk() + B.img_hdr()) + size_t(x) * HP_CAP * 4;
+        const size_t cstride = 4;
         const int nl = s_nlist[lr];
         if (keep[0] || keep[1] || pi == 0) {
             int count = 0, before[2] = {0, 0};
@@ -290,6 +290,125 @@
             if (pi == 0 && count > HP_CAP) atomicAdd(&B.hp_slow[p], 1);
         }
     }
+}
+
+constexpr int PK_THREADS = 256;
+constexpr int PK_TILE = 1024;
+constexpr int PK_ROWS_PER_THREAD = PK_TILE / PK_THREADS;
+__global__ void __launch_bounds__(PK_THREADS) k_pack_image(Batch B) {
+    const int tb = blockIdx.x, p = blockIdx.y, tid = threadIdx.x;
+    if (B.failed(p) != 0) return;
+    const int NJ = B.NJ, T = B.T, rows = B.img_rows();
+    const size_t chunk = size_t(p) * (T / TB) + tb;
+    unsigned char* img = B.img + chunk * B.img_chunk();
+    double* imgd = reinterpret_cast<double*>(img);
+    const unsigned char* cnt = B.hp_cnt + chunk * rows;
+    __shared__ unsigned s_off[PK_TILE + 1];
+    __shared__ unsigned s_part[PK_THREADS];
+    __shared__ unsigned s_carry;
+    __shared__ int s_loff[TB * MAXJ + 1], s_uoff[TB * NF + 1];
+    if (tid == 0) {
+        s_carry = 0;
+        int a = 0;
+        for (int i = 0; i < TB * NJ; i++) {
+            s_loff[i] = a;
+            a += min(B.link_n[(size_t(p) * T + tb * TB) * NJ + i], B.capL);
+        }
+        s_loff[TB * NJ] = a;
+        a = 0;
+        for (int i = 0; i < TB * NF; i++) {
+            s_uoff[i] = a;
+            a += min(B.u_n[(size_t(p) * T + tb * TB) * NF + i], B.capU);
+        }
+        s_uoff[TB * NF] = a;
+    }
+    double4* rec = reinterpret_cast<double4*>(img + B.img_hdr());
+    unsigned* grp = reinterpret_cast<unsigned*>(img + B.img_grp());
+    for (int t0 = 0; t0 < rows; t0 += PK_TILE) {
+        const int n = min(PK_TILE, rows - t0);
+        const int r0 = min(tid * PK_ROWS_PER_THREAD, n), r1 = min(r0 + PK_ROWS_PER_THREAD, n);
+        unsigned sum = 0;
+        for (int x = r0; x < r1; x++) sum += cnt[t0 + x] == HP_OVERFLOW ? 0u : cnt[t0 + x];
+        s_part[tid] = sum;
+        __syncthreads();
+        if (tid == 0) {
+            unsigned run = s_carry;
+            for (int i = 0; i < PK_THREADS; i++) {
+                const unsigned v = s_part[i];
+                s_part[i] = run;
+                run += v;
+            }
+            s_off[n] = run;
+        }
+        __syncthreads();
+        sum = s_part[tid];
+        for (int x = r0; x < r1; x++) {
+            s_off[x] = sum;
+            if (((t0 + x) & 31) == 0) grp[(t0 + x) >> 5] = sum;
+            sum += cnt[t0 + x] == HP_OVERFLOW ? 0u : cnt[t0 + x];
+        }
+        __syncthreads();
+        const unsigned first = s_off[0], end = s_off[n];
+        for (unsigned c0 = first; c0 < end; c0 += PK_THREADS) {
+            const unsigned c = c0 + tid;
+            double4 v;
+            if (c < end) {
+                int lo = 0, hi = n - 1;
+                while (lo < hi) {
+                    const int mid = (lo + hi + 1) >> 1;
+                    if (s_off[mid] <= c) lo = mid; else hi = mid - 1;
+                }
+                v = rec[size_t(t0 + lo) * HP_CAP + (c - s_off[lo])];
+            }
+            __syncthreads();
+            if (c < end) rec[c] = v;
+            __syncthreads();
+        }
+        if (tid == 0) s_carry = end;
+        __syncthreads();
+    }
+    __syncthreads();
+    const unsigned total = s_carry;
+    const int nlink = s_loff[TB * NJ], ntorque = s_uoff[TB * NF];
+    const size_t l0 = B.img_hdr() / 8 + size_t(total) * 4;
+    const size_t u0 = l0 + size_t(nlink) * 4;
+    const size_t k0 = (u0 + ntorque) * 4;
+    const size_t lidx = (size_t(p) * T + tb * TB) * NJ, uidx = (size_t(p) * T + tb * TB) * NF;
+    for (int i = tid; i < TB * NJ; i += PK_THREADS)
+        reinterpret_cast<int2*>(img)[i] = make_int2(int(l0) + 4 * s_loff[i], s_loff[i + 1] - s_loff[i]);
+    for (int i = tid; i < TB * NF; i += PK_THREADS)
+        reinterpret_cast<int4*>(img + B.img_ut())[i] = make_int4(int(u0) + s_uoff[i], int(k0) + s_uoff[i], s_uoff[i + 1] - s_uoff[i], 0);
+    for (int i = tid; i < TB * NJ * 3; i += PK_THREADS) {
+        reinterpret_cast<double*>(img + B.img_lc())[i] = B.link_c[lidx * 3 + i];
+        reinterpret_cast<double*>(img + B.img_lr())[i] = B.link_r[lidx * 3 + i];
+    }
+    for (int i = tid; i < TB * NF; i += PK_THREADS) {
+        reinterpret_cast<double*>(img + B.img_uc())[i] = B.u_c[uidx + i];
+        reinterpret_cast<double*>(img + B.img_ur())[i] = B.u_r[uidx + i];
+    }
+    for (int x = tid; x < rows; x += PK_THREADS) img[B.img_cnt() + x] = cnt[x];
+    for (int q = tid; q < TB * NJ * B.capL; q += PK_THREADS) {
+        const int i = q / B.capL, mI = q - i * B.capL;
+        if (mI >= s_loff[i + 1] - s_loff[i]) continue;
+        const size_t src = (lidx + i) * B.capL + mI;
+        double* dst = imgd + l0 + size_t(s_loff[i] + mI) * 4;
+        dst[0] = B.link_g[src * 3 + 0];
+        dst[1] = B.link_g[src * 3 + 1];
+        dst[2] = B.link_g[src * 3 + 2];
+        dst[3] = __longlong_as_double((long long)B.link_key[src]);
+    }
+    for (int q = tid; q < TB * NF * B.capU; q += PK_THREADS) {
+        const int i = q / B.capU, mI = q - i * B.capU;
+        if (mI >= s_uoff[i + 1] - s_uoff[i]) continue;
+        const size_t src = (uidx + i) * B.capU + mI;
+        imgd[u0 + s_uoff[i] + mI] = B.u_g[src];
+        reinterpret_cast<uint16_t*>(img)[k0 + s_uoff[i] + mI] = B.u_key[src];
+    }
+}
+cudaError_t launch_pack_image(const Batch& B, cudaStream_t st) {
+    if (B.nprob == 0) return cudaSuccess;
+    k_pack_image<<<dim3(B.T / TB, B.nprob), PK_THREADS, 0, st>>>(B);
+    return cudaGetLastError();
 }
 
 __device__ __noinline__ void row_from_generators(const double* __restrict__ ob, const double* __restrict__ LG,
@@ -357,44 +476,9 @@
     }
 }
 
-__device__ __forceinline__ unsigned smem_u32(const void* p) { return (unsigned)__cvta_generic_to_shared(p); }
-__device__ __forceinline__ void mbar_init(unsigned long long* bar, unsigned count) {
-    asm volatile("mbarrier.init.shared::cta.b64 [%0], %1;" ::"r"(smem_u32(bar)), "r"(count) : "memory");
-}
-__device__ __forceinline__ void mbar_arrive_expect_tx(unsigned long long* bar, unsigned bytes) {
-    asm volatile("mbarrier.arrive.expect_tx.shared::cta.b64 _, [%0], %1;" ::"r"(smem_u32(bar)), "r"(bytes) : "memory");
-}
-__device__ __forceinline__ void bulk_g2s(void* dst, const void* src, unsigned bytes, unsigned long long* bar) {
-    asm volatile("cp.async.bulk.shared::cluster.global.mbarrier::complete_tx::bytes [%0], [%1], %2, [%3];" ::"r"(smem_u32(dst)),
-                 "l"(src), "r"(bytes), "r"(smem_u32(bar))
-                 : "memory");
-}
-__device__ __forceinline__ void mbar_wait(unsigned long long* bar, unsigned parity) {
-    unsigned ok;
-    do {
-        asm volatile("{\n\t.reg .pred p;\n\tmbarrier.try_wait.parity.shared::cta.b64 p, [%1], %2;\n\tselp.u32 %0, 1, 0, p;\n\t}"
-                     : "=r"(ok)
-                     : "r"(smem_u32(bar)), "r"(parity)
-                     : "memory");
-    } while (!ok);
-}
-#ifndef K3_STAGE_CAND
-#define K3_STAGE_CAND 0
-#endif
-constexpr int K3_CAND_ARENA = 36864;
-#ifndef K3_STAGE_TABLES
-#define K3_STAGE_TABLES 0
-#endif
 #ifndef K3_DIRECT_J
 #define K3_DIRECT_J 1
 #endif
-constexpr int K3_LSLOT = 12;
-constexpr int K3_USLOT = 32;
-constexpr int K3_LTAB_BYTES = 32 + K3_LSLOT * 24;
-constexpr int K3_UTAB_BYTES = K3_USLOT * 2 + K3_USLOT * 8;
-__device__ __forceinline__ void cp_async16(void* dst, const void* src) {
-    asm volatile("cp.async.ca.shared.global [%0], [%1], 16;" ::"r"((unsigned)__cvta_generic_to_shared(dst)), "l"(src) : "memory");
-}
 #ifndef K3_SKIP_ZERO_DK
 #define K3_SKIP_ZERO_DK 0
 #endif
@@ -509,8 +593,6 @@
     __shared__ double s_stage[K3_WARPS][32 * NF];
 #endif
     __shared__ double s_tj[TB * NF * NF];
-    extern __shared__ __align__(16) unsigned char k3_tab[];
-    __shared__ unsigned long long s_bar;
     __shared__ int s_in_domain;
     __shared__ int s_next;
 
@@ -537,32 +619,6 @@
         }
         return;
     }
-#if K3_STAGE_CAND
-    const int rows_all = NJ * TB * O;
-    const int rows_staged = rows_all < K3_CAND_ARENA / 64 ? rows_all : K3_CAND_ARENA / 64;
-    double* const s_rec = reinterpret_cast<double*>(k3_tab + (K3_STAGE_TABLES ? TB * (NJ * K3_LTAB_BYTES + NF * K3_UTAB_BYTES) : 0));
-    if (tid == 0) {
-        mbar_init(&s_bar, 1);
-        asm volatile("fence.mbarrier_init.release.cluster;" ::: "memory");
-        const double* src = B.hp_cand + (size_t(p) * (T / TB) + tb) * B.hp_chunk();
-        const unsigned bytes = unsigned(rows_staged) * 32u;
-        mbar_arrive_expect_tx(&s_bar, rows_staged > 0 ? 2 * bytes : 0);
-        if (rows_staged > 0) {
-            bulk_g2s(s_rec, src, bytes, &s_bar);
-            bulk_g2s(s_rec + size_t(rows_staged) * 4, src + size_t(rows_all) * 4, bytes, &s_bar);
-        }
-    }
-#endif
-#ifndef K3_PREFETCH_L2
-#define K3_PREFETCH_L2 0
-#endif
-#if K3_PREFETCH_L2
-    {
-        const char* c0p = reinterpret_cast<const char*>(B.hp_cand + (size_t(p) * (T / TB) + tb) * B.hp_chunk());
-        const int lines = (NJ * TB * O * 32 * 2 + 127) / 128;
-        for (int i = tid; i < lines; i += K3_THREADS) asm volatile("prefetch.global.L2 [%0];" ::"l"(c0p + size_t(i) * 128));
-    }
-#endif
     if (tid == 32) {
         bool in = true;
         for (int j = 0; j < NF; j++) in = in && (fabs(kin[size_t(p) * NF + j]) <= K_DOMAIN);
@@ -589,6 +645,8 @@
 #endif
     const int per_pair = NJ * TB * O;
     const size_t chunk = size_t(p) * (T / TB) + tb;
+    const unsigned char* __restrict__ img = B.img + chunk * B.img_chunk();
+    const double* __restrict__ imgd = reinterpret_cast<const double*>(img);
     const bool cnt_in_smem = per_pair <= K3_CNT_SMEM;
     __syncthreads();
 
@@ -599,7 +657,7 @@
         constexpr int CW = (K3_CNT_SMEM / 4 + K3_LINK_THREADS - 1) / K3_LINK_THREADS;
         unsigned cw[CW];
         if (cnt_in_smem) {
-            const unsigned* src = reinterpret_cast<const unsigned*>(B.hp_cnt + chunk * per_pair);
+            const unsigned* src = reinterpret_cast<const unsigned*>(img + B.img_cnt());
 #pragma unroll
             for (int q = 0; q < CW; q++) cw[q] = (tid + q * K3_LINK_THREADS < per_pair / 4) ? __ldg(src + tid + q * K3_LINK_THREADS) : 0u;
         }
@@ -607,36 +665,13 @@
         const int e = tid % 3;
         const int l = (tid / 3) % NJ;
         const int tt = slicer ? tid / (3 * NJ) : 0;
-        const size_t idx = (size_t(p) * T + tb * TB + tt) * NJ + l;
-        const int n = slicer ? B.link_n[idx] : 0;
-#if K3_STAGE_TABLES
-        unsigned char* slot = k3_tab + (tt * NJ + l) * K3_LTAB_BYTES;
-        const int ns = n < K3_LSLOT ? n : K3_LSLOT;
+        const int li = tt * NJ + l;
+        const int2 lt = slicer ? reinterpret_cast<const int2*>(img)[li] : make_int2(0, 0);
         if (slicer) {
-            const char* ksrc = reinterpret_cast<const char*>(B.link_key + idx * B.capL);
-            const char* csrc = reinterpret_cast<const char*>(B.link_g + idx * B.capL * 3);
-            const int kc = (ns * 2 + 15) >> 4, cc = (ns * 24 + 15) >> 4;
-            if (e == 0)
-                for (int c = 0; c < kc; c++) cp_async16(slot + 16 * c, ksrc + 16 * c);
-            for (int c = e; c < cc; c += 3) cp_async16(slot + 32 + 16 * c, csrc + 16 * c);
-        }
-        asm volatile("cp.async.commit_group;" ::: "memory");
-        asm volatile("cp.async.wait_group 0;" ::: "memory");
-        __syncwarp();
-        asm volatile("bar.sync 4, %0;" ::"n"(K3_LINK_THREADS) : "memory");
-#endif
-        if (slicer) {
-            double value = B.link_c[idx * 3 + e];
+            double value = reinterpret_cast<const double*>(img + B.img_lc())[li * 3 + e];
             double grad[NF] = {0, 0, 0, 0, 0, 0, 0};
-#if K3_STAGE_TABLES
-            K3_SLICE(reinterpret_cast<const uint16_t*>(slot), reinterpret_cast<const double*>(slot + 32) + e, ns, 1, 3, K3_SLICE_TABLES,
-                            value, grad);
-            if (n > ns)
-                K3_SLICE(B.link_key + idx * B.capL + ns, B.link_g + (idx * B.capL + ns) * 3 + e, n - ns, 1, 3, K3_SLICE_TABLES, value, grad);
-#else
-            K3_SLICE(B.link_key + idx * B.capL, B.link_g + idx * B.capL * 3 + e, n, 1, 3, K3_SLICE_TABLES, value, grad);
-#endif
-            const double r = B.link_r[idx * 3 + e];
+            K3_SLICE(reinterpret_cast<const uint16_t*>(imgd + lt.x) + 12, imgd + lt.x + e, lt.y, 16, 4, K3_SLICE_TABLES, value, grad);
+            const double r = reinterpret_cast<const double*>(img + B.img_lr())[li * 3 + e];
             const double c = ((value - r) + (value + r)) * 0.5;
             s_lc[tt][l][e] = c;
             if (p == 0) B.link_sliced[((size_t(tb) * TB + tt) * NJ + l) * 3 + e] = c;
@@ -656,41 +691,12 @@
         double value = 0.0;
         double grad[NF] = {0, 0, 0, 0, 0, 0, 0};
         const bool on = i < TB * NF;
-        const size_t idx = (size_t(p) * T + tb * TB) * NF + (on ? i : 0);
+        const int4 ut = on ? reinterpret_cast<const int4*>(img + B.img_ut())[i] : make_int4(0, 0, 0, 0);
         if (on) {
-            const int n = B.u_n[idx];
-#if K3_STAGE_TABLES
-            unsigned char* slot = k3_tab + TB * NJ * K3_LTAB_BYTES + i * K3_UTAB_BYTES;
-            const int ns = n < K3_USLOT ? n : K3_USLOT;
-            {
-                const char* ksrc = reinterpret_cast<const char*>(B.u_key + idx * B.capU);
-                const char* csrc = reinterpret_cast<const char*>(B.u_g + idx * B.capU);
-                const int kc = (ns * 2 + 15) >> 4, cc = (ns * 8 + 15) >> 4;
-                for (int c = part; c < kc; c += K3_TORQUE_LANES) cp_async16(slot + 16 * c, ksrc + 16 * c);
-                for (int c = part; c < cc; c += K3_TORQUE_LANES) cp_async16(slot + K3_USLOT * 2 + 16 * c, csrc + 16 * c);
-            }
-        }
-        asm volatile("cp.async.commit_group;" ::: "memory");
-        asm volatile("cp.async.wait_group 0;" ::: "memory");
-        __syncwarp();
-        asm volatile("bar.sync 5, %0;" ::"n"(K3_THREADS - K3_LINK_THREADS) : "memory");
-        if (on) {
-            const int n = B.u_n[idx];
-            unsigned char* slot = k3_tab + TB * NJ * K3_LTAB_BYTES + i * K3_UTAB_BYTES;
-            const int ns = n < K3_USLOT ? n : K3_USLOT;
-            const int mine_s = (ns - part + K3_TORQUE_LANES - 1) / K3_TORQUE_LANES;
-            K3_SLICE(reinterpret_cast<const uint16_t*>(slot) + part, reinterpret_cast<const double*>(slot + K3_USLOT * 2) + part,
-                            mine_s > 0 ? mine_s : 0, K3_TORQUE_LANES, K3_TORQUE_LANES, K3_SLICE_TABLES, value, grad);
-            if (n > ns) {
-                const int rest = (n - ns - part + K3_TORQUE_LANES - 1) / K3_TORQUE_LANES;
-                K3_SLICE(B.u_key + idx * B.capU + ns + part, B.u_g + idx * B.capU + ns + part, rest > 0 ? rest : 0,
-                                K3_TORQUE_LANES, K3_TORQUE_LANES, K3_SLICE_TABLES, value, grad);
-            }
-#else
+            const int n = ut.z;
             const int mine = (n - part + K3_TORQUE_LANES - 1) / K3_TORQUE_LANES;
-            K3_SLICE(B.u_key + idx * B.capU + part, B.u_g + idx * B.capU + part, mine > 0 ? mine : 0,
+            K3_SLICE(reinterpret_cast<const uint16_t*>(img) + ut.y + part, imgd + ut.x + part, mine > 0 ? mine : 0,
                             K3_TORQUE_LANES, K3_TORQUE_LANES, K3_SLICE_TABLES, value, grad);
-#endif
         }
 #pragma unroll
         for (int d = 1; d < K3_TORQUE_LANES; d <<= 1) {
@@ -700,8 +706,8 @@
         }
         double* st = s_tj;
         if (on && part == 0) {
-            value = B.u_c[idx] + value;
-            const double r = B.u_r[idx];
+            value = reinterpret_cast<const double*>(img + B.img_uc())[i] + value;
+            const double r = reinterpret_cast<const double*>(img + B.img_ur())[i];
             if (gp) gp[tb * TB * NF + i] = ((value - r) + (value + r)) * 0.5;
 #pragma unroll
             for (int v = 0; v < NF; v++) st[i * NF + v] = grad[v];
@@ -715,16 +721,13 @@
         asm volatile("bar.sync 2, %0;" ::"n"(K3_THREADS) : "memory");
     }
 
-    const double* cand = B.hp_cand + chunk * B.hp_chunk();
-    const unsigned char* cnt = B.hp_cnt + chunk * per_pair;
-    const size_t cstride2 = size_t(per_pair) * 2;
+    const double2* __restrict__ cand = reinterpret_cast<const double2*>(img + B.img_hdr());
+    const unsigned* __restrict__ grp = reinterpret_cast<const unsigned*>(img + B.img_grp());
+    const unsigned char* cnt = img + B.img_cnt();
     const bool in_domain = s_in_domain != 0;
     const float inv_O = O > 0 ? 1.0f / float(O) : 0.0f;
 #if !K3_DIRECT_J
     double* stage = &s_stage[warp][0];
-#endif
-#if K3_STAGE_CAND
-    mbar_wait(&s_bar, 0);
 #endif
     for (;;) {
         int x0 = 0;
@@ -733,32 +736,29 @@
         if (x0 >= per_pair) break;
         const int x = x0 + lane;
         bool active = x < per_pair;
+        const unsigned base = grp[x0 >> 5];
         double max_elt = -100000000;
         double A0 = 0, A1 = 0, A2 = 0;
         int l = 0, tt = 0, o = 0;
+        const int n = active ? (cnt_in_smem ? s_cnt[x] : cnt[x]) : 0;
+        const int stored = n == HP_OVERFLOW ? 0 : n;
+        int before = stored;
+#pragma unroll
+        for (int d = 1; d < 32; d <<= 1) {
+            const int t = __shfl_up_sync(0xffffffffu, before, d);
+            if (lane >= d) before += t;
+        }
+        before -= stored;
         if (active) {
             const int ltt = __float2int_rz((float(x) + 0.5f) * inv_O);
             o = x - ltt * O;
             tt = ltt % TB;
             l = ltt / TB;
             const double c0 = s_lc[tt][l][0], c1 = s_lc[tt][l][1], c2 = s_lc[tt][l][2];
-            const int n = cnt_in_smem ? s_cnt[x] : cnt[x];
             if (n != HP_OVERFLOW && in_domain) {
-                const double2* row = reinterpret_cast<const double2*>(cand) + size_t(x) * 2;
+                const double2* row = cand + size_t(base + unsigned(before)) * 2;
                 for (int q0 = 0; q0 < n; q0 += K3_CQ) {
                     double2 u[K3_CQ], w[K3_CQ];
-#if K3_STAGE_CAND
-                    static_assert(K3_CQ == 2, "the staged levels are the first pass of the scan");
-                    if (q0 == 0 && x < rows_staged) {
-                        const double2* sr = reinterpret_cast<const double2*>(s_rec) + size_t(x) * 2;
-                        u[0] = sr[0];
-                        w[0] = sr[1];
-                        if (n > 1) {
-                            u[1] = sr[size_t(rows_staged) * 2];
-                            w[1] = sr[size_t(rows_staged) * 2 + 1];
-                        }
-                    } else
-#endif
 #pragma unroll
                     for (int i = 0; i < K3_CQ; i++) {
                         if (q0 + i < n) {
@@ -769,10 +769,10 @@
                             asm volatile("ld.global.nc.v4.f64 {%0, %1, %2, %3}, [%4];"
 #endif
                                          : "=d"(u[i].x), "=d"(u[i].y), "=d"(w[i].x), "=d"(w[i].y)
-                                         : "l"(row + (q0 + i) * cstride2));
+                                         : "l"(row + (q0 + i) * 2));
 #else
-                            u[i] = __ldg(row + (q0 + i) * cstride2);
-                            w[i] = __ldg(row + (q0 + i) * cstride2 + 1);
+                            u[i] = __ldg(row + (q0 + i) * 2);
+                            w[i] = __ldg(row + (q0 + i) * 2 + 1);
 #endif
                         }
                     }
@@ -1073,11 +1073,8 @@
     }
 #endif
     dim3 grid(B.T / TB, B.nprob);
-    const int rows_all = B.NJ * TB * B.O;
-    const size_t dyn = (K3_STAGE_TABLES ? size_t(TB) * (B.NJ * K3_LTAB_BYTES + NF * K3_UTAB_BYTES) : 0) +
-                       (K3_STAGE_CAND ? size_t(rows_all < K3_CAND_ARENA / 64 ? rows_all : K3_CAND_ARENA / 64) * 64 : 0);
     if (B.O == 0) {
-        k_constraints<<<grid, K3_THREADS, dyn, st>>>(B, d_k, d_g, d_jac);
+        k_constraints<<<grid, K3_THREADS, 0, st>>>(B, d_k, d_g, d_jac);
         return cudaGetLastError();
     }
     k_constraints_slow<<<(B.nprob + K3S_PROBLEMS - 1) / K3S_PROBLEMS, 128, 0, st>>>(B, d_k, d_g, d_jac);
@@ -1086,7 +1083,7 @@
     cudaLaunchConfig_t cfg = {};
     cfg.gridDim = grid;
     cfg.blockDim = dim3(K3_THREADS);
-    cfg.dynamicSmemBytes = dyn;
+    cfg.dynamicSmemBytes = 0;
     cfg.stream = st;
     cudaLaunchAttribute attr[1];
     attr[0].id = cudaLaunchAttributeProgrammaticStreamSerialization;
diff --git a/armour_b200/csrc/layout.h b/armour_b200/csrc/layout.h
--- a/armour_b200/csrc/layout.h
+++ b/armour_b200/csrc/layout.h
@@ -39,14 +39,26 @@
     double* torque_radius;
     double* link_gens;
     double* link_r;
-    double* hp_cand;
     unsigned char* hp_cnt;
     int* hp_slow;
+    unsigned char* img;
     double* link_sliced;
     int* status;
     const int* plist;
 
-    __host__ __device__ size_t hp_chunk() const { return size_t(HP_CAP) * 4 * NJ * TB * O; }
+    __host__ __device__ int img_rows() const { return NJ * TB * O; }
+    __host__ __device__ size_t img_ut() const { return size_t(TB) * NJ * 8; }
+    __host__ __device__ size_t img_lc() const { return img_ut() + size_t(TB) * NF * 16; }
+    __host__ __device__ size_t img_lr() const { return img_lc() + size_t(TB) * NJ * 24; }
+    __host__ __device__ size_t img_uc() const { return img_lr() + size_t(TB) * NJ * 24; }
+    __host__ __device__ size_t img_ur() const { return img_uc() + size_t(TB) * NF * 8; }
+    __host__ __device__ size_t img_grp() const { return img_ur() + size_t(TB) * NF * 8; }
+    __host__ __device__ size_t img_cnt() const { return img_grp() + size_t(img_rows() + 31) / 32 * 4; }
+    __host__ __device__ size_t img_hdr() const { return (img_cnt() + img_rows() + 127) / 128 * 128; }
+    __host__ __device__ size_t img_chunk() const {
+        const size_t tables = size_t(TB) * NJ * capL * 32 + size_t(TB) * NF * capU * 10;
+        return (img_hdr() + size_t(img_rows()) * HP_CAP * 32 + tables + 127) / 128 * 128;
+    }
     __host__ __device__ int m() const { return NF * T + NJ * T * O + 4 * NF; }
     __device__ int failed(int p) const { return (status[p] >> 3) == epoch ? (status[p] & 7) : 0; }
 };
diff --git a/armour_b200/planner.py b/armour_b200/planner.py
--- a/armour_b200/planner.py
+++ b/armour_b200/planner.py
@@ -112,6 +112,19 @@
             self._check(self.lib.armour_batch_get_candidate_counts(self._h, self.nprob, out.ctypes.data_as(C.c_void_p)))
         return out
 
+    def eval_image_layout(self):
+        lay = (C.c_longlong * 10)()
+        self._check(self.lib.armour_eval_image_layout(self._h, lay))
+        names = ("chunk", "link_tables", "torque_tables", "link_c", "link_r", "u_c", "u_r", "groups", "counts", "records")
+        return dict(zip(names, (int(v) for v in lay)))
+
+    def eval_images(self):
+        layout = self.eval_image_layout()
+        C_ = self.lib.armour_chunk_intervals()
+        out = np.zeros((self.nprob, self.T // C_, layout["chunk"]), np.uint8)
+        self._check(self.lib.armour_batch_get_eval_images(self._h, self.nprob, out.ctypes.data_as(C.c_void_p)))
+        return out, layout
+
     def solve(self, q_des, max_iter=None, tol=None, qp_sweeps=None, qp_update_budget=None):
         q_des = np.ascontiguousarray(np.asarray(q_des, dtype=np.float64).reshape(self.nprob, NF))
         opt = _lib.SolverOptions()
diff --git a/include/armour_b200.h b/include/armour_b200.h
--- a/include/armour_b200.h
+++ b/include/armour_b200.h
@@ -98,6 +98,8 @@
 int armour_batch_get_monomial_counts(armour_ctx* ctx, int nprob, int* link_n, int* u_n);
 int armour_batch_get_candidate_counts(armour_ctx* ctx, int nprob, unsigned char* out);
 int armour_chunk_intervals(void);
+int armour_eval_image_layout(armour_ctx* ctx, long long* layout);
+int armour_batch_get_eval_images(armour_ctx* ctx, int nprob, void* out);
 int armour_measure_fp64_peak(armour_ctx* ctx, double* tflops);
 
 enum { ARMOUR_ROLLOUT_BUDGET = 0, ARMOUR_ROLLOUT_ARRIVED = 1, ARMOUR_ROLLOUT_COLLISION = 2, ARMOUR_ROLLOUT_LIMIT = 3 };
```

Measured after the change: 2.062 million, median of 6. 3.4% higher.
